# voutcn/megahit

Hardware: AMD Instinct MI355X
Metric: M (k+1)-mer edges sorted+counted/sec, sdbg_build k=21 (higher is better)
Workload: dtype u32; 1 GPU; read2sdbg (S1+S2) k=21 m=2 no mercy, 10000000 synthetic 150 bp PE reads per GPU (BASELINE configs[1]), inputs resident in HBM, outputs left in HBM; reads_per_gpu=10000000, edges_per_gpu=1290000000, k=21, min_count=2, parallelism=1 GPU, s1_items=1330000000, s2_items=117381042, sdbg_records=59857080

## Files before the change

megahit_amd/csrc/mhx_internal.h:

```cpp
#pragma once
#include <hip/hip_runtime.h>

#include <cstdint>
#include <cstdio>
#include <cstring>
#include <functional>
#include <map>
#include <stdexcept>
#include <string>
#include <vector>

#include "../../include/mhx.h"
#include "mhx_options.h"
#include "s1_handoff.h"

using mhx::Opt;

namespace mhx {

struct OnesweepLaunch;
void set_error(const char *fmt, ...);

struct Error : std::runtime_error {
  explicit Error(const std::string &s) : std::runtime_error(s) {}
// ... 56 lines not shown
  mhx::S1Handoff s1;
  uint64_t n_route = 0;
  uint32_t filter_kept = 0;
  double s1_density = 0;
  bool s1_agg_wide_agreed = false;
  std::string last_s1_plan;
  bool filter_on = false, accumulate = false;
  uint64_t filter_expected = 0, filter_batch_bytes = 0;
  bool global_marks_inverted = false;
  uint64_t s1_acc_bits = 0, mercy_acc_n = 0;
  uint32_t s1_acc_k = 0, s1_acc_m = 0;
  uint32_t count_acc_k = 0, count_acc_m = 0;
  uint64_t n_marks = 0;
  uint64_t dist_local_solid = 0;
  bool dist_s2_agg = false;
  bool ut_ready = false, ut_owner = false;
  uint64_t ut_edges = 0, ut_nv = 0;
  bool ut_text_fresh = false;
  uint64_t ub_stats[4] = {0, 0, 0, 0};
  bool lm_ready = false, lm_mapped = false;
  uint64_t lm_n_ctg = 0, lm_cap = 0, lm_n_reads = 0;
  uint32_t lm_seed = 0;
  std::map<std::string, long long> options;
  std::map<std::string, long long> tuned;
  template <mhx::Opt O>
  long long opt() const { return mhx::resolve_option<O>(options, tuned); }
  template <mhx::Opt O>
  long long opt(long long fallback) const { return mhx::resolve_option<O>(options, tuned, fallback); }
  long long opt(const char *name, long long dflt) const { return mhx::resolve_option(options, tuned, name, dflt); }
  void *pinned[2] = {nullptr, nullptr};
  hipEvent_t pinned_free[2] = {nullptr, nullptr};
  bool profiling = false;
  std::vector<mhx::PendingEvent> pending;
  std::vector<hipEvent_t> event_pool;
  std::vector<hipStream_t> side_streams;
  std::vector<hipEvent_t> side_events;
  std::map<std::string, mhx::KernelStat> stats;

  mhx::DevBuf &ws(const char *name, size_t bytes) {
    mhx::DevBuf &b = work[name];
    b.reserve(bytes);
    return b;
  }
  mhx::DevBuf &result(int which, size_t bytes) {
    mhx::DevBuf &b = results[which];
    b.reserve(bytes);
    b.used = bytes;
    return b;
  }
  void prof_begin(const char *name, double bytes);
  void prof_end();
  void prof_collect();
};

#define MHX_LAUNCH(ctx, name, bytes, ...) \
  do {                                    \
    (ctx)->prof_begin(name, bytes);       \
    __VA_ARGS__;                          \
    MHX_HIP(hipGetLastError());           \
    (ctx)->prof_end();                    \
  } while (0)

namespace mhx {

struct SortPass {
  int shift;
  int bits;
  int shift2 = 0;
  int bits2 = 0;
  int prev_lo = -1;
};
struct SortPrep {
  const void *buf = nullptr;
  uint64_t n = 0;
  int hist_passes = 0;
  uint64_t hist_sig = 0;
  const unsigned long long *hist = nullptr;
  std::function<void(const OnesweepLaunch &)> gen;
  uint64_t gen_slots = 0;
  bool gen_var = false;
  const unsigned long long *split_fill = nullptr, *split_ubase = nullptr;
  uint64_t split_range_cap = 0, split_units = 0;
  int hist_first = 0;
};
uint32_t *radix_sort(mhx_ctx *c, uint32_t *buf_a, uint32_t *buf_b, uint64_t n, int stride, int key_words,
                     const std::vector<SortPass> &passes, SortPrep *prep = nullptr);
uint32_t *sort_whole_key(mhx_ctx *c, uint32_t *buf_a, uint32_t *buf_b, uint64_t n, int stride, int key_words,
                         const std::vector<SortPass> &passes, SortPrep *prep = nullptr);
std::vector<SortPass> make_passes(int key_words, int lo_bit, int hi_bit);
bool sort_takes_generated_first_pass(const mhx_ctx *c, uint64_t n, int stride, const std::vector<SortPass> &passes);
bool sort_takes_split_first_pass(const mhx_ctx *c, const std::vector<SortPass> &passes);
constexpr uint64_t kSortSplitUnit = 4096;
uint64_t passes_signature(const std::vector<SortPass> &ps);
uint32_t *kmsort_exact(mhx_ctx *c, uint32_t *buf_a, uint32_t *buf_b, uint64_t n, int S, int key_words, SortPrep *prep = nullptr);

void exclusive_scan_u32_u64(mhx_ctx *c, const uint32_t *in, uint64_t *out, uint64_t n, uint64_t *d_total);
void exclusive_scan_u64(mhx_ctx *c, const uint64_t *in, uint64_t *out, uint64_t n, uint64_t *d_total);
void find_group_heads(mhx_ctx *c, const uint32_t *items, uint64_t n, int stride, int cmp_bits,
                      uint64_t *heads, uint64_t *d_count);
uint64_t count_group_heads(mhx_ctx *c, const uint32_t *items, uint64_t n, int stride, int cmp_bits);

struct DigitSpec;
DigitSpec spec_of_pass(const SortPass &ps, int key_words);
std::vector<SortPass> make_passes_ranges(int key_words, const std::vector<std::pair<int, int>> &ranges);
void emit_sdbg(mhx_ctx *c, const uint32_t *sorted, uint64_t n_items, int S, int kw, uint32_t k, int is_seq, mhx_sdbg_result *out, int compact_bits = 0);

void partition_by_owner(mhx_ctx *c, const uint32_t *a, uint32_t *b, uint64_t n, int stride, const uint8_t *lut, int n_parts,
                        uint64_t *counts);
uint64_t s1_extract(mhx_ctx *c, uint32_t k, bool compact, SortPrep *prep, bool defer_items = false, bool filter_in_gen = false);
bool s1_compact(const mhx_ctx *c, uint32_t k, int want_mercy);
bool s1_rank_tagged(const mhx_ctx *c, uint32_t k);
int s1_stride(uint32_t k, bool compact);
struct S1Sources {
  int n = 0;
  std::vector<const uint32_t *> ptr;
  std::vector<uint64_t> count;
  uint32_t *spare = nullptr;
  int pbits = 16;
};
constexpr int kSkmBatch = 8;
constexpr int kSkmSrcMax = 8;
struct SkmFront {
  int n_src;
  const uint4 *src[kSkmSrcMax];
  const uint64_t *src_bounds[kSkmSrcMax];
  uint32_t *spare;
  uint64_t spare_bytes;
  uint64_t n_records, n_windows;
  uint64_t n_items;
  uint32_t n_bins, max_bin;
  uint32_t bin_lo, bin_hi;
  int bin_bits;
  unsigned long long *hp;
  bool rep;
  const uint2 *giants;
  uint32_t n_giant_items, giant_limit;
  uint32_t giant_bins, giant_largest;
  const char *why;
};
bool s1_skm_applies(const mhx_ctx *c, uint32_t k, uint32_t m, int want_mercy);
bool s1_skm_dist_applies(const mhx_ctx *c, uint32_t k, uint32_t m);
int s1_skm_passes(const mhx_ctx *c, uint32_t k);
bool s1_skm_front(mhx_ctx *c, uint32_t k, SkmFront *f, int pass, int n_passes, int bin_bits_agreed = 0, bool for_count = false, bool bins_whole = false);
uint32_t s1_skm_max_m(const mhx_ctx *c);
uint64_t s1_skm_beside_below(mhx_ctx *c, const SkmFront &f, uint32_t k, uint32_t m);
void s1_skm_bounds_of(mhx_ctx *c, const uint4 *recs, uint64_t n, uint32_t n_bins, uint64_t *bounds);
void s1_skm_groups_launch(mhx_ctx *c, bool agg, unsigned grid, const SkmFront &f, uint32_t k, uint32_t m, uint8_t *solid_bytes, unsigned long long *hist,
                          uint2 *agg_raw, uint32_t agg_cap, uint32_t *agg_counts, uint32_t *err, unsigned long long *marks_raw, uint32_t marks_cap,
                          uint32_t *marks_counts);
struct DigitSpecs;
void s1_skm_hp_publish(mhx_ctx *c, const SkmFront &f, uint32_t k, uint32_t m, uint8_t *solid_bytes, unsigned long long *hist, uint2 *agg_items,
                       uint64_t *agg_cursor, bool agg, const DigitSpecs *agg_specs = nullptr, unsigned long long *agg_hist = nullptr);
uint64_t s1_skm_rep_publish(mhx_ctx *c, const SkmFront &f, uint32_t k, uint32_t m, uint8_t *solid_bytes, unsigned long long *hist, uint2 *agg_items,
                            uint64_t *agg_cursor, bool agg, const DigitSpecs *agg_specs = nullptr, unsigned long long *agg_hist = nullptr);
bool s1_skm_owner(mhx_ctx *c, uint32_t k, uint32_t m, const SkmFront &f, mhx_s1_result *out);

bool s1_presort_applies(const mhx_ctx *c, uint32_t k, uint64_t n_local_items);
uint32_t *s1_presort(mhx_ctx *c, uint32_t k, uint32_t *buf_a, uint32_t *buf_b, uint64_t n_items, int *pbits, SortPrep *prep);
bool s1_filter_in_gen_applies(const mhx_ctx *c, uint32_t k);
bool s1_bucket_histogram_fast(mhx_ctx *c, uint32_t k, unsigned long long *hist);
uint32_t s1_pos_bits(const mhx_ctx *c);
uint64_t s1_pos_stride(const mhx_ctx *c, uint32_t k);
std::string s1_plan_text(const mhx_ctx *c, uint32_t k, uint64_t n_items);
int s1_process(mhx_ctx *c, uint32_t k, uint32_t m, int want_mercy, uint32_t *buf_a, uint32_t *buf_b, uint64_t n_items, mhx_s1_result *out,
               const S1Sources *pre = nullptr, SortPrep *prep = nullptr, bool var_gen = false);
__global__ void k_add_u64(unsigned long long *__restrict__ a, const unsigned long long *__restrict__ b, int n);
void sdbg_accumulate(mhx_ctx *c, bool first);
void sdbg_publish_accumulated(mhx_ctx *c);
uint64_t s2_extract(mhx_ctx *c, uint32_t k, uint32_t m, bool filter_in_extract = false);
int s2_process(mhx_ctx *c, uint32_t k, uint32_t *buf_a, uint32_t *buf_b, uint64_t n_items, mhx_sdbg_result *out);
bool s2_use_aggregated(const mhx_ctx *c, uint32_t k, uint32_t m);
uint64_t s2_agg_extract(mhx_ctx *c, uint32_t k);
int s2_agg_process(mhx_ctx *c, uint32_t k, uint32_t *buf_a, uint32_t *buf_b, uint64_t n_items, mhx_sdbg_result *out, SortPrep *prep = nullptr);
std::vector<SortPass> s2_agg_sort_passes(uint32_t k, int count_bits);
struct StageItems {
  uint64_t n;
  int S;
  bool agg;
  bool batchable;
  SortPrep prep;
};
StageItems extract_stage(mhx_ctx *c, int stage, uint32_t k, uint32_t m, bool s1_defer_items = false);
void bucket_histogram(mhx_ctx *c, int stage, uint32_t k, uint32_t m, uint64_t *h_out);
int s2_stride(uint32_t k);
constexpr int MHX_BUF_IS_SOLID_LOCAL = 100;
constexpr int MHX_BUF_MERCY_CAND_LOCAL = 101;
uint64_t count_extract(mhx_ctx *c, uint32_t k, uint32_t m, SortPrep *prep);
int count_stride(uint32_t k);
int count_process(mhx_ctx *c, uint32_t k, uint32_t m, uint32_t *buf_a, uint32_t *buf_b, uint64_t n_items, mhx_count_result *out, SortPrep *prep = nullptr);
void count_apply_events(mhx_ctx *c, const unsigned long long *ev, uint64_t n);
uint64_t seq2sdbg_extract(mhx_ctx *c, uint32_t k);
int seq2sdbg_stride(uint32_t k);
int seq2sdbg_process(mhx_ctx *c, uint32_t k, uint32_t *buf_a, uint32_t *buf_b, uint64_t n_items, mhx_sdbg_result *out);
const uint64_t *sort_u64(mhx_ctx *c, const void *src, uint64_t n, int hi_bit);
void invert_local_marks(mhx_ctx *c, unsigned long long *words, uint64_t n_words);
DevBuf &grow_preserving(mhx_ctx *c, DevBuf &b, size_t bytes, size_t keep);
void stash_route_records(mhx_ctx *c, const void *src, uint64_t n, int hi_bit);
void mercy_adopt_routed(mhx_ctx *c, const long long *recv, uint64_t n);
void s1_apply_marks(mhx_ctx *c, const unsigned long long *recv, uint64_t n);
int sdbg_build_index(mhx_ctx *c, uint32_t k, mhx_sdbg_index_info *out);
int sdbg_remove_tips(mhx_ctx *c, const mhx_sdbg_index_info *info, int max_tip_len, uint64_t *n_removed);
int sdbg_mul_histogram(mhx_ctx *c, const mhx_sdbg_index_info *info, uint64_t *n_valid, std::vector<uint64_t> *host = nullptr);
int infer_min_depth(const uint64_t *hist, double *min_depth, int *converged);
int sdbg_unitigs(mhx_ctx *c, const mhx_sdbg_index_info *info, mhx_unitig_result *out);
int sdbg_unitig_text(mhx_ctx *c, const mhx_sdbg_index_info *info, uint64_t nv, uint64_t n_loop, mhx_unitig_result *out);
int unitig_disconnect_weak_links(mhx_ctx *c, const mhx_sdbg_index_info *info, double ratio, uint64_t *n_flagged);
int unitig_remove_tips(mhx_ctx *c, const mhx_sdbg_index_info *info, uint32_t max_tip_len, uint64_t *n_removed);
int unitig_remove_local_low_depth(mhx_ctx *c, const mhx_sdbg_index_info *info, double min_depth, uint32_t max_len, uint32_t local_width,
                                  double local_ratio, int mark_changed, uint64_t *n_removed, int *is_changed);
int unitig_iterate_local_low_depth(mhx_ctx *c, const mhx_sdbg_index_info *info, double min_depth, uint32_t max_len, uint32_t local_width,
                                   double local_ratio, int mark_changed, uint64_t *n_removed);
int unitig_finish(mhx_ctx *c, const mhx_sdbg_index_info *info, mhx_unitig_result *out);
int unitig_remove_low_depth(mhx_ctx *c, const mhx_sdbg_index_info *info, double min_depth, uint64_t *n_removed);
int unitig_pop_bubbles(mhx_ctx *c, const mhx_sdbg_index_info *info, uint32_t max_len, double similarity, double careful_threshold, int mark_changed,
                       uint64_t *n_removed, uint64_t *n_records);
int unitig_similarity(mhx_ctx *c, const char *a, uint32_t n, const char *b, uint32_t m, double sim, double *out);
int iterate_edges(mhx_ctx *c, uint32_t k, uint32_t step, const uint32_t *ctg_words, uint64_t ctg_n_words, uint64_t n_ctg, const uint64_t *ctg_start,
                  mhx_iterate_result *out);
int local_index(mhx_ctx *c, const uint32_t *ctg_words, uint64_t ctg_n_words, uint64_t n_ctg, const uint64_t *ctg_start, uint32_t seed,
                uint32_t sparsity, uint64_t *index_size);
int local_map(mhx_ctx *c, int32_t min_mapping_len, double similarity, uint64_t *n_valid);
int local_collect(mhx_ctx *c, uint32_t n_libs, const uint64_t *lib_begin, const uint64_t *lib_end, const int32_t *lib_paired,
// ... 85 lines not shown
```

megahit_amd/csrc/mhx_options.h:

```cpp
#pragma once
#include <cstddef>
#include <cstdlib>
#include <cstring>
#include <map>
#include <string>
#include <vector>

#define MHX_OPTIONS(X, D)          \
                     \
  X(edges_reserve_permille, 1000)  \
  X(fetch_pinned, 1)               \
  X(dist_marks_one_pass, 1)        \
                     \
  X(sort_unit_runs, 1)             \
  X(sort_xcd_units, 1)             \
  X(sort_loaded_ut2, 0)            \
  X(sort_rank_uniform, 1)          \
  X(sort_hybrid, 1)                \
  X(sort_hybrid_min, 1 << 16)      \
  X(sort_hybrid_margin_ps, 6)      \
  X(sort_hybrid_bits, 0)           \
                  \
  X(iterate_prefix_filter, 1)      \
                \
  X(tips_candidate_list, 1)        \
               \
  D(sdbg_hist_flush_tiles)         \
               \
  X(kmsort_emu_legacy, 0)          \
                   \
  X(s2_filter_in_extract, 1)       \
                     \
  X(dist_presort, 1)               \
  X(dist_max_items, 0)             \
  X(count_skm_dist, 0)             \
                    \
  X(count_seg, 1)                  \
  X(count_seg_bits, 0)             \
  X(count_extract_fixed, 1)        \
  X(count_seg_la, 3)               \
                       \
  X(s1_seg_bits, 0)                \
  X(s1_seg, 1)                     \
  X(s1_stream, 1)                  \
  X(s1_stream_wide, 1)             \
  X(s1_stream_max, 40000)          \
  X(s1_stream_sub_max, 1)          \
  D(s1_stream_max3)                \
  X(s1_stream_bits, 0)             \
  X(s1_stream_sub0, -1)            \
  X(s1_pos_bits, 0)                \
  X(dist_sparse_marks, 0)          \
  X(s1_seg_per, 8)                 \
  X(s1_seg_la, 3)                  \
  X(s1_stream_direct, 1)           \
  X(s1_stream_probes, 1024)        \
  D(s1_stream_fill)                \
  X(s1_giant, 1)                   \
  X(s1_giant_min, 262144)          \
  X(s1_pack_fixed, 1)              \
  X(s1_agg_wide, 0)                \
  X(count_stream, 1)               \
  X(count_event_share, 4)          \
  X(count_giant, 1)                \
                 \
  X(s1_bucket_hist_fast, 1)        \
  X(s1_digit_hist_roll, 1)         \
  X(count_stream_wide, 1)          \
  X(s1_var_fast, 1)                \
  X(s1_var_min_fill, 50)           \
  X(s1_extract_fast, 1)            \
  X(s1_filter_in_gen, 1)           \
  X(s1_fused_first_pass, 1)        \
  X(s1_digit_hist_blocked, 1)      \
  X(s1_digit_hist_plain, 1)        \
  X(s1_gen_any_order, 1)           \
  X(s1_gen_blocked, 0)             \
  X(s1_gen_roll, 1)                \
  X(s1_extract_items, 4)           \
  X(s1_digit_hist_preload, 0)      \
                  \
  X(s1_mercy_regions, 1)           \
                   \
  X(s1_skm, 1)                     \
  X(s1_skm_min_windows, 1 << 22)   \
  X(s1_skm_bin_bits, 0)            \
  X(count_skm, 1)                  \
  X(s1_skm_max_m, 2)               \
  X(dist_skm, 1)                   \
  X(s1_skm_passes, 0)              \
  X(s1_skm_cap_pct, 36)            \
  X(s1_skm_pass_gb, 48)            \
  X(s1_skm_split, 1)               \
  D(s1_skm_split_stage)            \
  X(s1_skm_make_grid, 0)           \
  X(s1_skm_hp, 1)                  \
  X(s1_skm_rep, 0)                 \
  X(s1_skm_rep_slots, 64)          \
  X(s1_skm_giant, 0)               \
  X(s1_skm_giant_max, 1 << 21)     \
  X(s1_skm_giant_keys, 4096)       \
  X(s1_skm_giant_work_pct, 25)     \
  X(s1_skm_giant_slices, 0)        \
  X(s1_skm_max_bin, 1 << 16)       \
  X(s1_skm_tags, 0)                \
  X(s1_skm_deal, 2)                \
  X(count_skm_group, 2)            \
  X(count_skm_ev_cap, 0)           \
                       \
  X(sdbg_fast, 1)                  \
  D(sdbg_fast_halo)                \
  X(sdbg_fast_tile, 2048)          \
  X(sdbg_fast_keep, 1)             \
  X(sdbg_fast_keep_max_mb, 4096)   \
  X(s2_bound_from_s1, 1)           \
  X(s2_dummy_list, 1)              \
  X(s2_dummy_list_cap, 0)          \
  X(s2_agg_from_count, 1)          \
  X(s2_count_budget_mb, 0)         \
  X(s2_count_pass_items, 0)        \
  X(s2_pre_hist, 1)                \
  X(s2_agg_in_place, 1)

namespace mhx {

#define MHX_OPT_PLAIN(name, dflt) name,
#define MHX_OPT_DERIVED(name) name,
enum class Opt : int { MHX_OPTIONS(MHX_OPT_PLAIN, MHX_OPT_DERIVED) };
#undef MHX_OPT_PLAIN
#undef MHX_OPT_DERIVED

struct OptInfo {
  const char *name;
  char env_name[48];
  long long dflt;
  bool derived;
};

constexpr void opt_env_name(const char *name, char *out, size_t cap) {
  const char pre[] = "MHX_";
  size_t n = 0;
  for (const char *p = pre; *p && n + 1 < cap; ++p) out[n++] = *p;
  for (const char *p = name; *p && n + 1 < cap; ++p) out[n++] = *p >= 'a' && *p <= 'z' ? (char)(*p - 'a' + 'A') : *p;
  out[n] = 0;
}
constexpr OptInfo make_opt_info(const char *name, long long dflt, bool derived) {
  OptInfo o{name, {}, dflt, derived};
  opt_env_name(name, o.env_name, sizeof o.env_name);
  return o;
}

#define MHX_OPT_PLAIN(name, dflt) make_opt_info(#name, dflt, false),
#define MHX_OPT_DERIVED(name) make_opt_info(#name, 0, true),
inline constexpr OptInfo kOptions[] = {MHX_OPTIONS(MHX_OPT_PLAIN, MHX_OPT_DERIVED)};
#undef MHX_OPT_PLAIN
#undef MHX_OPT_DERIVED
inline constexpr size_t kNumOptions = sizeof kOptions / sizeof kOptions[0];
constexpr const OptInfo &opt_info(Opt o) { return kOptions[(size_t)o]; }

using OptMap = std::map<std::string, long long>;

inline long long resolve_option(const OptMap &options, const OptMap &tuned, const char *name, const char *env_name, long long dflt) {
  auto it = options.find(name);
  if (it != options.end()) return it->second;
  const char *e = getenv(env_name);
  if (e && *e) return atoll(e);
  auto tu = tuned.find(name);
  return tu != tuned.end() ? tu->second : dflt;
}
inline long long resolve_option(const OptMap &options, const OptMap &tuned, const char *name, long long dflt) {
  std::string env(strlen(name) + 5, '\0');
  opt_env_name(name, &env[0], env.size());
  return resolve_option(options, tuned, name, env.c_str(), dflt);
}
template <Opt O>
long long resolve_option(const OptMap &options, const OptMap &tuned) {
  static_assert(!opt_info(O).derived, "a derived knob has no default of its own: read it as opt<Opt::name>(fallback)");
  return resolve_option(options, tuned, opt_info(O).name, opt_info(O).env_name, opt_info(O).dflt);
}
template <Opt O>
long long resolve_option(const OptMap &options, const OptMap &tuned, long long fallback) {
  static_assert(opt_info(O).derived, "this knob has its default in the table: read it as opt<Opt::name>()");
  return resolve_option(options, tuned, opt_info(O).name, opt_info(O).env_name, fallback);
}

inline void set_option(OptMap &options, Opt o, long long v) { options[opt_info(o).name] = v; }

class OptScope {
 public:
// ... 19 lines not shown
```

megahit_amd/csrc/s1.hip:

```cpp
#include "s1_shared.h"

namespace mhx {

template <bool HIST>
__global__ __launch_bounds__(256) void k_agg_compact(const uint2 *__restrict__ raw, uint32_t cap, const uint32_t *__restrict__ counts,
                                                    uint2 *__restrict__ dense, int from_back, DigitSpecs specs, unsigned long long *__restrict__ hist) {
  __shared__ uint64_t sm[256 / kWave + 1];
  __shared__ uint32_t s_hist[HIST ? kItemHistRows : 1][256];
  if (HIST)
    for (int i = threadIdx.x; i < kItemHistRows * 256; i += 256) (&s_hist[0][0])[i] = 0;
  const ItemDigits digits(specs);
  const uint32_t r = blockIdx.x;
  uint64_t part = 0;
  for (uint32_t i = threadIdx.x; i < r; i += 256) part += counts[i];
  uint64_t off;
  block_exclusive_sum<uint64_t, 256>(part, sm, &off);
  const uint32_t n = counts[r];
  const uint2 *src = raw + (size_t)r * cap;
  for (uint32_t i = blockIdx.y * 256 + threadIdx.x; i < n; i += gridDim.y * 256) {
    const uint2 v = from_back ? src[cap - 1 - i] : src[i];
    dense[off + i] = v;
    if (HIST) item_hist_add(s_hist, digits, ((uint64_t)v.x << 32) | v.y);
  }
  if (HIST) {
// ... 306 lines not shown
  const double n_eff = per_bucket * (double)MHX_NUM_BUCKETS;
  int bits = 8;
  while (bits < 32 && n_eff / 96.0 > (double)(1ull << bits)) bits += 8;
  if (force_bits) bits = force_bits;
  bits = std::max(1, std::min(bits, std::min(32, kmer_bits)));
  p.seg_bits = bits;
  p.passes = make_passes(2, 64 - bits, 64);
  return p;
}
std::string s1_plan_text(const mhx_ctx *c, uint32_t k, uint64_t n_items) {
  const S1Plan p = s1_plan(c, k, n_items, s1_compact(c, k, 0), 0);
  char buf[128];
  if (p.stream) snprintf(buf, sizeof buf, "stream p%d sub%d %zu passes (%.0f records per lv1 bucket)", p.seg_bits, p.sub0, p.passes.size(), p.per_bucket);
  else if (p.seg_bits) snprintf(buf, sizeof buf, "seg p%d %zu passes", p.seg_bits, p.passes.size());
  else snprintf(buf, sizeof buf, "full sort %zu passes", p.passes.size());
  return buf;
}
uint32_t s1_pos_bits(const mhx_ctx *c) {
  const bool force = getenv("MHX_S1_FORCE_TAGGED") != nullptr;
  const long long f = c->opt<Opt::s1_pos_bits>();
  if (f > 0) return (uint32_t)std::min<long long>(std::max<long long>(f, 4), 32);
  if (force) {
    const uint64_t n_bits = c->global_bases ? c->global_bases : c->seqs.n_bases;
    uint32_t b = 4;
    while (b < 32 && (n_bits >> b) >= 128) ++b;
    return b;
  }
  return 32;
}
bool s1_rank_tagged(const mhx_ctx *c, uint32_t k) {
  const uint64_t n_bits = c->global_bases ? c->global_bases : c->seqs.n_bases;
  const uint32_t pb = s1_pos_bits(c);
  if ((n_bits >> pb) == 0) return false;
  const int spare = 32 * s1_kw(k) - (int)(k - 1) * 2 - 6;
  return spare >= 8 && (n_bits >> pb) < 256;
}
uint64_t s1_pos_stride(const mhx_ctx *c, uint32_t k) { return s1_rank_tagged(c, k) ? 1ull << s1_pos_bits(c) : 0ull; }
bool s1_compact(const mhx_ctx *c, uint32_t k, int want_mercy) {
  if (want_mercy) return false;
  if (s1_kw(k) < 2) return false;
  const uint64_t n_bits = c->global_bases ? c->global_bases : c->seqs.n_bases;
  return (n_bits >> s1_pos_bits(c)) == 0 || s1_rank_tagged(c, k);
}
int s1_stride(uint32_t k, bool compact) {
  const int kw = s1_kw(k);
  if (!compact) return round_up2(kw + 2);
  return kw + 1 == 3 ? 3 : round_up2(kw + 1);
}


bool s1_presort_applies(const mhx_ctx *c, uint32_t k, uint64_t n_local_items) {
  return c->n_parts <= kStreamSrcMax && s1_plan(c, k, n_local_items, s1_compact(c, k, 0), 0).stream;
}
uint32_t *s1_presort(mhx_ctx *c, uint32_t k, uint32_t *buf_a, uint32_t *buf_b, uint64_t n_items, int *pbits, SortPrep *prep) {
  const S1Plan plan = s1_plan(c, k, std::max<uint64_t>(n_items, 1), true, 0);
  if (!plan.stream) throw Error("s1_presort: the bucket-streaming plan does not apply");
  *pbits = plan.seg_bits;
  return n_items ? radix_sort(c, buf_a, buf_b, n_items, 3, s1_kw(k), plan.passes, prep) : buf_a;
}

namespace {
struct S1Stage {
  mhx_ctx *c;
  uint32_t k, m;
  int want_mercy;
  uint32_t *buf_a, *buf_b;
  uint64_t n_items;
  const S1Sources *pre;
  SeqSet &s;
  hipStream_t st;
  bool compact, global, tagged_keys;
  int KWv, S, kmer_bits;
  size_t item_bytes;
  uint64_t pos_stride;
  S1Plan plan;
  uint32_t *sorted = nullptr, *spare = nullptr;
  uint64_t n_bits = 0, n_words64 = 0;
  int mark_atomic = 0;
  const char *mark_env = nullptr;
  bool sparse = false, acc = false;
  bool list_local = false;
  unsigned long long *is_solid = nullptr, *hist = nullptr, *ctr = nullptr;
  uint8_t *solid_bytes = nullptr;
  uint64_t marks_prev = 0, seg_marks = 0;
  const uint32_t *giant_ctr = nullptr;
  bool classic_ran = false;
  long long *mercy = nullptr;
  bool agg = false;
  bool agg_wide = false;
  uint2 *agg_items = nullptr;
  uint64_t *agg_cursor = nullptr;
  uint64_t agg_prev = 0, agg_bound = 0;
  unsigned long long *agg_hist = nullptr;
  DigitSpecs agg_specs = no_digits();
  uint64_t agg_sig = 0;
  uint32_t seg_grid = 0, seg_cap = 0, seg_mcap = 0;
  uint32_t *seg_err = nullptr;
  uint64_t skm_rounds = 0, skm_looks = 0;
  int mark_mode = 0, mark_mode_used = 0;

  S1Stage(mhx_ctx *c_, uint32_t k_, uint32_t m_, int wm, uint32_t *a, uint32_t *b, uint64_t n, const S1Sources *pre_)
      : c(c_), k(k_), m(m_), want_mercy(wm), buf_a(a), buf_b(b), n_items(n), pre(pre_), s(c_->seqs), st(c_->stream) {
    compact = s1_compact(c, k, want_mercy);
    KWv = s1_kw(k);
    S = s1_stride(k, compact);
    item_bytes = (size_t)S * 4;
    global = c->global_bases != 0;
    kmer_bits = (int)(k - 1) * 2;
    tagged_keys = compact && s1_rank_tagged(c, k);
    pos_stride = compact ? s1_pos_stride(c, k) : 0;
    plan = s1_plan(c, k, pre ? std::max<uint64_t>(n_items, 1) : n_items, compact, want_mercy);
    if (pre && (!plan.stream || want_mercy || !compact)) throw Error("s1_process: pre-sorted sources need the bucket-streaming plan");
    if (pre && pre->pbits != plan.seg_bits) throw Error("s1_process: the sources were sorted for another plan than the one this rank makes");
  }

  void sort_records(SortPrep *prep) {
    sorted = pre ? nullptr
             : want_mercy == 2
                 ? kmsort_exact(c, buf_a, buf_b, n_items, S, KWv, prep)
                 : (plan.seg_bits || tagged_keys ? radix_sort(c, buf_a, buf_b, n_items, S, KWv, plan.passes, prep)
                                                 : sort_whole_key(c, buf_a, buf_b, n_items, S, KWv, plan.passes, prep));
    set_spare(pre ? pre->spare : (sorted == buf_a ? buf_b : buf_a));
  }
  void set_spare(uint32_t *sp) {
    spare = sp;
    mercy = reinterpret_cast<long long *>(spare);
  }
  void ensure_byte_map() {
    if (solid_bytes) return;
    const uint64_t nw = div_ceil(n_bits, 64);
    solid_bytes = c->ws("solid_bytes", (nw + 1) * 64).as<uint8_t>();
    if (!acc || sparse) MHX_HIP(hipMemsetAsync(solid_bytes, 0, (nw + 1) * 64, st));
  }
  void open_outputs() {
    n_bits = global ? c->global_bases : s.n_bases;
    mark_env = getenv("MHX_S1_MARK");
    mark_atomic = mark_env && !strcmp(mark_env, "atomic") ? 1 : 0;
    sparse = global && !mark_atomic && c->opt<Opt::dist_sparse_marks>() != 0;
    n_words64 = sparse ? 0 : div_ceil(n_bits, 64);
    is_solid = c->result(MHX_BUF_IS_SOLID, (n_words64 + 1) * 8).as<unsigned long long>();
    c->results[MHX_BUF_IS_SOLID].used = n_words64 * 8;
    hist = c->result(MHX_BUF_MUL_HIST, (MHX_MAX_MUL + 1) * 8).as<unsigned long long>();
    acc = c->accumulate && c->s1_acc_bits == n_bits && c->s1_acc_k == k && c->s1_acc_m == m;
    marks_prev = sparse && acc ? c->n_marks : 0;
    if (!sparse || !acc) c->n_marks = 0;
    if (mark_atomic) {
      if (!acc) MHX_HIP(hipMemsetAsync(is_solid, 0, (n_words64 + 1) * 8, st));
    } else {
      if (!sparse) ensure_byte_map();
      MHX_HIP(hipMemsetAsync(is_solid + n_words64, 0, 8, st));
    }
    if (!acc) MHX_HIP(hipMemsetAsync(hist, 0, (MHX_MAX_MUL + 1) * 8, st));
    c->s1_acc_bits = n_bits;
    c->s1_acc_k = k;
    c->s1_acc_m = m;
    ctr = c->ws("s1_counters", 64).as<unsigned long long>();
    MHX_HIP(hipMemsetAsync(ctr, 0, 64, st));
    const bool agg_off = getenv("MHX_S2_PER_OCCURRENCE") != nullptr;
    agg = !agg_off && k <= 22 && m >= 2 && KWv == 2;
    agg_wide = !agg_off && k >= 23 && k <= 27 && m >= 2 && KWv == 2 && !want_mercy && plan.stream && c->opt<Opt::s1_agg_wide>() != 0;
    if (global && !c->s1_agg_wide_agreed) agg_wide = false;
    const S1Handoff::Opened opened = c->s1.open_items(k, m, acc);
    if (agg_wide && acc && !opened.continues) agg_wide = false;
    agg = agg || agg_wide;
    agg_cursor = c->ws("s2_agg_cursor", 64).as<uint64_t>();
    if (!opened.in_flight.empty()) MHX_HIP(hipStreamSynchronize(st));
    agg_prev = opened.continues ? c->s1.agg_n : 0;
    agg_bound = (n_items / m + 16) * 2;
    if (agg_wide) agg_bound += n_items / ((1ull << s2_agg_compact_bits(k)) - 1) * 2;
    agg_hist = nullptr;
    if (agg && !global && !c->filter_on && !c->accumulate && agg_prev == 0 && c->opt<Opt::s2_pre_hist>() != 0) {
      const std::vector<SortPass> ps = s2_agg_sort_passes(k, s2_agg_count_bits(k));
      if (!ps.empty() && ps.size() <= (size_t)kItemHistRows) {
        agg_specs.n = (int)ps.size();
        for (size_t p = 0; p < ps.size(); ++p) agg_specs.d[p] = spec_of_pass(ps[p], 2);
        agg_sig = passes_signature(ps);
        agg_hist = c->ws("s2_pre_hist", (size_t)kItemHistRows * 256 * 8).as<unsigned long long>();
        MHX_HIP(hipMemsetAsync(agg_hist, 0, (size_t)kItemHistRows * 256 * 8, st));
      }
    }
    seg_err = c->ws("s1_seg_err", 64).as<uint32_t>();
  }
  void agg_wide_off() {
    if (!agg_wide) return;
    agg = agg_wide = false;
    agg_hist = nullptr;
  }
  void agg_prepare_classic() {
    agg_wide_off();
    agg_hist = nullptr;
    if (!agg) return;
    agg_items = grow_preserving(c, c->work["s2_agg_items"], (agg_prev + agg_bound) * 8, agg_prev * 8).as<uint2>();
    MHX_HIP(hipMemsetAsync(agg_cursor, 0, 24, st));
    if (agg_prev) MHX_HIP(hipMemcpyAsync(agg_cursor, &agg_prev, 8, hipMemcpyHostToDevice, st));
  }

  void launch_partial(int mode) {
    const int per = (int)c->opt<Opt::s1_seg_per>();
    const int la = (int)std::min<long long>(std::max<long long>(c->opt<Opt::s1_seg_la>(), 0), 200);
    const int T = 256 * (per == 4 ? 4 : 8);
    const uint64_t n_tiles = div_ceil(n_items, (uint64_t)T);
    const uint32_t stride = mode == 2 ? 64u : 1u;
    const uint64_t n_buckets = plan.stream ? 1ull << plan.seg_bits : 0;
    const uint64_t n_work = plan.stream ? div_ceil(n_buckets, stride) : div_ceil(n_tiles, stride);
    const uint32_t pfx_mask = plan.seg_bits >= 32 ? 0xFFFFFFFFu : ~(0xFFFFFFFFu >> plan.seg_bits);
    const uint32_t eq_mask1 = (kmer_bits > 32 ? ~(0xFFFFFFFFu >> (kmer_bits - 32)) : 0u) | 63u;
    const bool agg_on = agg && mode != 2;
    const bool half = false;
    const uint64_t cus = c->n_cus > 0 ? (uint64_t)c->n_cus : 256;
    unsigned grid = (unsigned)std::min<uint64_t>(n_work, plan.stream ? (half ? 2 * cus : cus) : (per == 4 ? 256 * 6 : 256 * 3));
    if (agg_on && agg_wide) {
      const uint64_t min_region = 16 * ((uint64_t)MHX_MAX_MUL / ((1ull << s2_agg_compact_bits(k)) - 1) + 1);
      grid = (unsigned)std::min<uint64_t>(grid, std::max<uint64_t>(1, n_items * (uint64_t)S * 4 / 8 / min_region));
    }
    const uint32_t region = (uint32_t)std::min<uint64_t>(n_items * (uint64_t)S * 4 / 8 / grid, 0xFFFFFFF0u);
// ... 538 lines not shown
    g.fl_cap = kGiantFlagged;
    g.fl_cnt = c->ws("cs_giant_fl_cnt", (size_t)g.gcap * 4 + 64).as<uint32_t>();
    g.fl_key = c->ws("cs_giant_fl_key", (size_t)g.gcap * g.fl_cap * 8 + 64).as<unsigned long long>();
    MHX_HIP(hipMemsetAsync(g.fl_cnt, 0, (size_t)g.gcap * 4 + 64, st));
    if (global) {
      g.ev_cap = (uint32_t)std::min<uint64_t>(std::max<uint64_t>(n_items / 8, 1u << 20), 0xFFFFFFF0u);
      g.ev = c->ws("cs_giant_events", (size_t)g.ev_cap * 8 + 64).as<unsigned long long>();
      g.ev_cur = g.fl_cnt + g.gcap;
    }
    MHX_HIP(hipMemsetAsync(g.flag, 0, n_buckets, st));
    MHX_HIP(hipMemsetAsync(lists, 0, 64, st));
    s1_giant_launch(c, items0, srcs, bounds, n_src, n_buckets, plan.seg_bits, (int)k, g, key64, true);
  }
  S1StreamLaunch sl{true, false, pos_stride != 0, false, true, grid, items0, bounds, a, geo, 1u, ticket, srcs, n_src};
  sl.key64 = key64;
  s1_stream_launch(c, "count_groups", bytes, sl);
  if (giant_on) {
    S1StreamLaunch gl{true, false, pos_stride != 0, true, true, grid, items0, bounds, a, geo, 1u, ticket2, srcs, n_src};
    gl.key64 = key64;
    s1_stream_launch(c, "count_giant_groups", 0.0, gl);
    count_giant_look_launch(c, items0, srcs, bounds, n_src, n_buckets, plan.seg_bits, a);
  }
  uint32_t e = 0;
  unsigned long long h_ctr[8] = {0};
  std::vector<uint32_t> h_ec(global ? grid : 0);
  MHX_HIP(hipMemcpyAsync(&e, seg_err, 4, hipMemcpyDeviceToHost, st));
  MHX_HIP(hipMemcpyAsync(h_ctr, ctr, 64, hipMemcpyDeviceToHost, st));
  if (global) MHX_HIP(hipMemcpyAsync(h_ec.data(), ecounts, (size_t)grid * 4, hipMemcpyDeviceToHost, st));
  MHX_HIP(hipStreamSynchronize(st));
  o->grid = grid;
  o->cap = region;
  o->counts = counts;
  o->spare = spare;
  o->sorted = sorted;
  o->n_items = n_items;
  o->n_distinct = h_ctr[4];
  o->plan = s1_plan_text(c, k, std::max<uint64_t>(count_plan_items(c, k), 1));
  if (giant_ctr) {
    uint32_t h_giant[4] = {0, 0, 0, 0};
    MHX_HIP(hipMemcpy(h_giant, giant_ctr, 16, hipMemcpyDeviceToHost));
    if (h_giant[0]) o->plan += " [" + std::to_string(h_giant[0]) + " giant buckets in slices]";
  }
  o->events = nullptr;
  o->n_events = 0;
  if (e == 0 && global) {
    for (uint32_t v : h_ec) o->n_events += v;
    uint32_t n_look = 0;
    if (giant_on) {
      MHX_HIP(hipMemcpy(&n_look, a.giant.ev_cur, 4, hipMemcpyDeviceToHost));
      n_look = std::min(n_look, a.giant.ev_cap);
    }
    unsigned long long *dense = c->ws("cs_events_dense", (o->n_events + n_look) * 8 + 64).as<unsigned long long>();
    if (o->n_events)
      MHX_LAUNCH(c, "events_compact", (double)o->n_events * 16,
                 agg_compact_launch(st, dim3(grid, 8), reinterpret_cast<const uint2 *>(a.marks_raw), ecap, ecounts,
                                    reinterpret_cast<uint2 *>(dense), 0, no_digits(), nullptr));
    if (n_look) MHX_HIP(hipMemcpyAsync(dense + o->n_events, a.giant.ev, (size_t)n_look * 8, hipMemcpyDeviceToDevice, st));
    o->n_events += n_look;
    o->events = dense;
  }
  return e == 0;
}

static bool s1_skm_try(mhx_ctx *c, uint32_t k, uint32_t m, mhx_s1_result *out, std::string *why) {
  const int n_passes = s1_skm_passes(c, k);
  SkmFront f{};
  S1Stage stage(c, k, m, 0, nullptr, nullptr, 0, nullptr);
  stage.sorted = nullptr;
  uint64_t n_records = 0;
  uint32_t max_bin = 0, giant_bins = 0, giant_slices = 0, giant_largest = 0;
  for (int p = 0; p < n_passes; ++p) {
    if (!s1_skm_front(c, k, &f, p, n_passes, 0, false, m >= 3)) {
      *why = f.n_records ? "a bin of " + std::to_string(f.max_bin) + " records" : "more records than the array holds";
      if (f.why) *why += std::string(", ") + f.why;
      return false;
    }
    if (p == 0 && m >= 3) {
      if (const uint64_t n_below = s1_skm_beside_below(c, f, k, m)) {
        *why = "a key beside the records has " + std::to_string(n_below) + " windows, below the min count";
        return false;
      }
    }
    stage.set_spare(f.spare);
    if (p == 0) stage.open_outputs();
    if (!stage.run_skm(f)) {
      *why = "an output region overflowed";
      return false;
    }
    n_records += f.n_records;
    max_bin = std::max(max_bin, f.max_bin);
    giant_bins += f.giant_bins;
    giant_slices += f.n_giant_items;
    giant_largest = std::max(giant_largest, f.giant_largest);
  }
  stage.publish_skm_hp(f);
  const uint64_t n_rep = stage.publish_skm_rep(f);
  stage.n_items = f.n_items;
  stage.mark_mode_used = 1;
  char txt[320];
  snprintf(txt, sizeof txt, "super-k-mers m%u, 2^%d bins (%llu records for %llu windows: %.2f per record; largest bin %u)%s", k + 1 - 9, f.bin_bits,
           (unsigned long long)n_records, (unsigned long long)f.n_windows, n_records ? (double)f.n_windows / (double)n_records : 0.0, max_bin,
           c->seqs.fixed_len ? "" : " [reads of several lengths]");
  c->last_s1_plan = txt;
  if (n_passes > 1) c->last_s1_plan += " [" + std::to_string(n_passes) + " passes over ranges of bins]";
  if (f.rep) c->last_s1_plan += " [" + std::to_string(n_rep) + " windows of period <= 4 beside the records]";
  if (giant_bins)
    c->last_s1_plan += " [" + std::to_string(giant_bins) + " giant bins in " + std::to_string(giant_slices) + " slices, largest " + std::to_string(giant_largest) + " records]";
  if (m >= 3) c->last_s1_plan += " [a second look in " + std::to_string(stage.skm_looks) + " of " + std::to_string(stage.skm_rounds) + " rounds]";
  stage.publish(out);
  return true;
}

bool s1_skm_owner(mhx_ctx *c, uint32_t k, uint32_t m, const SkmFront &f, mhx_s1_result *out) {
  S1Stage stage(c, k, m, 0, nullptr, nullptr, f.n_items, nullptr);
  stage.sorted = nullptr;
  stage.set_spare(f.spare);
  stage.open_outputs();
  if (!stage.sparse) throw Error("s1_skm_owner: the marks of a global layout leave as a list (dist_sparse_marks)");
  if (!stage.run_skm(f)) return false;
  stage.mark_mode_used = 1;
  char txt[320];
  snprintf(txt, sizeof txt, "super-k-mers m%u, 2^%d bins (%llu records at this owner, bins %u..%u) [records exchanged by bin]", k + 1 - 9, f.bin_bits,
           (unsigned long long)f.n_records, f.bin_lo, f.bin_hi);
  c->last_s1_plan = txt;
  stage.publish(out);
  return true;
}

int run_s1(mhx_ctx *c, uint32_t k, uint32_t m, int want_mercy, mhx_s1_result *out) {
  if (c->global_bases) throw Error("read2sdbg_s1: a global layout is set; use the mhx_dist_* entry points");
  std::string skm_why;
  if (s1_skm_applies(c, k, m, want_mercy)) {
    if (s1_skm_try(c, k, m, out, &skm_why)) return 0;
    if (c->opt<Opt::s1_skm>() == 3) throw Error("read2sdbg_s1: super-k-mer records given up (" + skm_why + ")");
  }
  StageItems it = extract_stage(c, want_mercy ? MHX_STAGE_S1_MERCY : MHX_STAGE_S1, k, m, !want_mercy);
  uint32_t *buf_a = c->work["items_a"].as<uint32_t>();
  uint32_t *buf_b = c->ws("items_b", it.n * (size_t)it.S * 4 + 64).as<uint32_t>();
  const int rc = s1_process(c, k, m, want_mercy, buf_a, buf_b, it.n, out, nullptr, &it.prep, it.prep.gen_var);
  if (!skm_why.empty()) c->last_s1_plan += " [super-k-mer records given up: " + skm_why + "]";
  return rc;
}

}
```

megahit_amd/csrc/s1_skm.hip:

```cpp
#include <cstring>

#include "s1_shared.h"
#include "skm_deal.h"
#include "skm_giant.h"

namespace mhx {

constexpr int kSkmC = 8;
constexpr int kSkmW = 10;
constexpr int kSkmNM = kSkmC + kSkmW - 1;
constexpr int kSkmMinBinBits = 16, kSkmMaxBinBits = 20;

__device__ __forceinline__ uint32_t skm_mix(uint32_t c) {
  uint32_t h = c * 0x9E3779B1u;
  return h ^ (h >> 15);
}
__device__ __forceinline__ uint32_t skm_mix2(uint32_t c) {
  uint32_t h = c * 0x9E3779B1u;
  h ^= h >> 15;
  return h * 0x85EBCA6Bu;
}
__device__ __forceinline__ uint32_t skm_bin_of(uint32_t minh) {
  return (minh ^ (minh >> 16)) * 0x7FEB352Du;
}

constexpr int kSkmStage = 2560;
constexpr int kSkmRepN = 320, kSkmRepAt = 64;
constexpr int kSkmRepSlotsS1 = 48, kSkmRepSlotsCount = 16, kSkmRepProbes = 8;
template <int NT, int J, bool VAR, bool COUNT = false, bool SPLIT = false, bool REP = false>
__global__ __launch_bounds__(NT) void k_skm_make(const uint32_t *__restrict__ seq, const uint64_t *__restrict__ start, uint32_t L, uint32_t bpr, uint64_t n_blocks,
                                                 int k, int bin_bits, uint32_t bin_lo, uint32_t bin_hi, int count_items, uint64_t pos_base,
                                                 unsigned long long *__restrict__ hp, uint4 *__restrict__ out, unsigned long long cap,
                                                 unsigned long long *__restrict__ cursor, uint32_t *__restrict__ err, unsigned long long *__restrict__ digit_hist,
                                                 unsigned long long range_cap, unsigned long long *__restrict__ split_cur, uint32_t stage_n) {
  constexpr long long kNoRoom = -0x7FFFFFFFFFFFFFFFll - 1;
  __shared__ uint32_t sm_scan[NT / kWave + 1];
  __shared__ uint4 stage[SPLIT ? kSkmStage : 1];
  __shared__ uint32_t dcnt[SPLIT ? 256 : 1], dpos[SPLIT ? 256 : 1];
  __shared__ long long goff[SPLIT ? 256 : 1];
  __shared__ unsigned long long s_base;
  __shared__ uint32_t dh[3][256];
  __shared__ uint32_t lbin[J * kSkmC][NT];
  __shared__ uint32_t hpl[2][12];
  constexpr int kSkmRepSlots = COUNT ? kSkmRepSlotsCount : kSkmRepSlotsS1;
  __shared__ uint32_t rid[REP ? kSkmRepSlots : 1];
  __shared__ uint32_t rtl[REP ? kSkmRepSlots : 1][COUNT ? 9 : 1];
  __shared__ unsigned long long rps[REP && !COUNT ? kSkmRepSlots : 1];
  const int tid = threadIdx.x;
  if constexpr (REP) {
    if (tid < kSkmRepSlots) {
      rid[tid] = (uint32_t)kSkmRepN;
      if constexpr (!COUNT) rps[tid] = ~0ull;
    }
    if (tid < kSkmRepSlots * (COUNT ? 9 : 1)) rtl[tid / (COUNT ? 9 : 1)][tid % (COUNT ? 9 : 1)] = 0;
  }
  if (tid < 24) hpl[tid / 12][tid % 12] = 0;
  for (int i = tid; i < 768; i += NT) dh[i >> 8][i & 255] = 0;
  if (SPLIT && tid < 256) dcnt[tid] = 0;
  __syncthreads();
  const bool third_digit = bin_bits > 16;
  const int M = k + 1 - (kSkmW - 1);
  const uint32_t mmask = (1u << (2 * M)) - 1u;
  const int K1 = k + 1;
  const unsigned bin_sh = 32u - (unsigned)bin_bits;
  unsigned long long items = 0;
  uint32_t hp_n[2] = {0, 0};
  unsigned long long hp_p[2] = {~0ull, ~0ull};
  const uint64_t step_trip = (uint64_t)gridDim.x * (uint64_t)(NT * J);
  const uint64_t trip_r = step_trip / bpr;
  const uint32_t trip_q = (uint32_t)(step_trip - trip_r * bpr), next_r = (uint32_t)NT / bpr, next_q = (uint32_t)NT % bpr;
  uint64_t blk_r = ((uint64_t)blockIdx.x * (uint64_t)(NT * J) + tid) / bpr;
  uint32_t blk_q = (uint32_t)((uint64_t)blockIdx.x * (uint64_t)(NT * J) + tid - blk_r * bpr);
  uint64_t fa[J];
  uint32_t fq0[J], fnwin[J], fc[J][COUNT ? 4 : 3];
  [[maybe_unused]] auto rep_tally = [&](uint32_t e, unsigned pv, unsigned nx, uint64_t p) {
    if constexpr (REP) {
      unsigned long long *const tab = hp + kSkmRepAt;
      const uint32_t n_slots = min((uint32_t)hp[kSkmRepAt - 1], (uint32_t)kSkmRepSlots);
      uint32_t h = n_slots ? (e ^ (e >> 4) ^ (e >> 6)) % n_slots : 0u;
      int slot = -1;
      for (int n = 0; n < kSkmRepProbes && n_slots; ++n) {
        const uint32_t old = atomicCAS(&rid[h], (uint32_t)kSkmRepN, e);
        if (old == (uint32_t)kSkmRepN || old == e) {
          slot = (int)h;
          break;
        }
        h = h + 1 == n_slots ? 0u : h + 1;
      }
      if (slot >= 0) {
        atomicAdd(&rtl[slot][0], 1u);
        if constexpr (COUNT) {
          if (pv < 4) atomicAdd(&rtl[slot][1 + pv], 1u);
          if (nx < 4) atomicAdd(&rtl[slot][5 + nx], 1u);
        } else {
          atomicMin(&rps[slot], (unsigned long long)p);
        }
      } else {
        const uint32_t sig = COUNT ? e | ((uint32_t)pv << 9) | ((uint32_t)nx << 12) : e;
        for (;;) {
          const uint32_t s0 = (uint32_t)__builtin_amdgcn_readfirstlane((int)sig);
          const unsigned long long together = __ballot(sig == s0);
          if (sig == s0) {
            if ((tid & (kWave - 1)) == __builtin_ctzll(together)) {
              const unsigned long long n = (unsigned long long)__builtin_popcountll(together);
              if constexpr (COUNT) {
                atomicAdd(tab + 9 * e, n);
                if (pv < 4) atomicAdd(tab + 9 * e + 1 + pv, n);
                if (nx < 4) atomicAdd(tab + 9 * e + 5 + nx, n);
              } else {
                atomicAdd(tab + e, n);
              }
            }
            break;
          }
        }
        if constexpr (!COUNT) {
          unsigned long long *const at = tab + kSkmRepN + e;
          if ((unsigned long long)p < __hip_atomic_load(at, __ATOMIC_RELAXED, __HIP_MEMORY_SCOPE_AGENT)) atomicMin(at, (unsigned long long)p);
        }
      }
    }
  };
  auto fetch = [&](uint64_t it2) {
    uint64_t r = blk_r;
    uint32_t q = blk_q;
#pragma unroll
    for (int j = 0; j < J; ++j) {
      const uint64_t b = it2 * (uint64_t)(NT * J) + (uint64_t)j * NT + tid;
      fa[j] = 0;
      fq0[j] = 0;
      fnwin[j] = 0;
      if (j > 0) {
        r += next_r;
        q += next_q;
        if (q >= bpr) {
          q -= bpr;
          ++r;
        }
      }
      if (b < n_blocks) {
        const uint32_t q0 = q * kSkmC;
        uint64_t base;
        uint32_t nwin;
        if constexpr (VAR) {
          base = start[r];
          const uint64_t len_r = start[r + 1] - base;
          nwin = len_r >= (uint64_t)K1 ? (uint32_t)(len_r - k) : 0u;
          if (q0 == 0 && nwin && count_items) items += nwin + (COUNT ? 0 : 4);
        } else {
          base = r * L;
          nwin = L - k;
        }
        if (q0 < nwin) {
          fa[j] = base + q0;
          fq0[j] = q0;
          fnwin[j] = nwin;
        }
      }
      const uint64_t wi = fa[j] >> 4;
      fc[j][0] = seq[wi];
      fc[j][1] = seq[wi + 1];
      fc[j][2] = seq[wi + 2];
      if constexpr (COUNT) fc[j][3] = seq[(fa[j] > 0 ? fa[j] - 1 : 0) >> 4];
    }
    blk_r += trip_r;
    blk_q += trip_q;
    if (blk_q >= bpr) {
      blk_q -= bpr;
      ++blk_r;
    }
  };
  for (uint64_t it = blockIdx.x; it * (uint64_t)(NT * J) < n_blocks; it += gridDim.x) {
    uint64_t Wv[J], pos0[J];
    uint32_t smask[J], emask[J];
    uint32_t bflag[J];
    fetch(it);
#pragma unroll
    for (int j = 0; j < J; ++j) {
      smask[j] = 0;
      emask[j] = 0;
      bflag[j] = 0;
      Wv[j] = 0;
      pos0[j] = 0;
      {
        const uint32_t q0 = fq0[j], nwin = fnwin[j];
        if (q0 < nwin) {
          const uint64_t a = fa[j];
          const unsigned sh = (unsigned)(a & 15) * 2;
          const uint32_t c0 = fc[j][0], c1 = fc[j][1], c2 = fc[j][2];
          const uint64_t W = ((uint64_t)funnel_l(c0, c1, sh) << 32) | funnel_l(c1, c2, sh);
          const uint64_t R = rc64(W, 32);
          uint32_t h[kSkmNM];
#pragma unroll
          for (int i = 0; i < kSkmNM; ++i) {
            const uint32_t f = (uint32_t)(W >> (64 - 2 * (i + M))) & mmask;
            const uint32_t rv = (uint32_t)(R >> (2 * i)) & mmask;
            h[i] = skm_mix(min(f, rv));
          }
          uint32_t sfx[kSkmW];
          sfx[kSkmW - 1] = h[kSkmW - 1];
#pragma unroll
          for (int i = kSkmW - 2; i >= 0; --i) sfx[i] = min(h[i], sfx[i + 1]);
          uint32_t pfx = 0xFFFFFFFFu;
          uint32_t bins[kSkmC];
          bins[0] = skm_bin_of(sfx[0]) >> bin_sh;
#pragma unroll
          for (int w = 1; w < kSkmC; ++w) {
            pfx = min(pfx, h[kSkmW - 1 + w]);
            bins[w] = skm_bin_of(min(sfx[w], pfx)) >> bin_sh;
          }
#pragma unroll
          for (int w = 0; w < kSkmC; ++w) lbin[j * kSkmC + w][tid] = bins[w];
          const uint32_t n_here = min((uint32_t)kSkmC, nwin - q0);
          uint32_t km = 0, sm = 0, hm = 0;
          if constexpr (REP) {
            const uint64_t d4 = W ^ (W << 8), d3 = W ^ (W << 6);
            uint32_t m4 = 0, m3 = 0;
            if ((d4 & ((~0ull >> (2 * (kSkmC - 1))) & (~0ull << (64 - 2 * (K1 - 4))))) == 0) {
#pragma unroll
              for (int w = 0; w < kSkmC; ++w)
                if ((uint32_t)w < n_here && ((d4 << (2 * w)) >> (64 - 2 * (K1 - 4))) == 0) m4 |= 1u << w;
            }
            if ((d3 & ((~0ull >> (2 * (kSkmC - 1))) & (~0ull << (64 - 2 * (K1 - 3))))) == 0) {
#pragma unroll
              for (int w = 0; w < kSkmC; ++w)
                if ((uint32_t)w < n_here && ((d3 << (2 * w)) >> (64 - 2 * (K1 - 3))) == 0) m3 |= 1u << w;
            }
            hm = m4 | m3;
            if (hm && count_items) {
#pragma unroll
              for (int w = 0; w < kSkmC; ++w)
                if ((hm >> w) & 1u) {
                  const uint32_t e = (m4 >> w) & 1u ? (uint32_t)(W >> (56 - 2 * w)) & 255u : 256u + ((uint32_t)(W >> (58 - 2 * w)) & 63u);
                  unsigned prev_raw = 4, next_raw = 4;
                  if constexpr (COUNT) {
                    prev_raw = q0 + w == 0 ? kSentinel
                                           : (w == 0 ? (unsigned)((fc[j][COUNT ? 3 : 0] >> (30 - 2 * (unsigned)((a - 1) & 15))) & 3u) : (unsigned)(W >> (64 - 2 * w)) & 3u);
                    next_raw = q0 + w + 1 == nwin ? kSentinel : (unsigned)(W >> (62 - 2 * (w + K1))) & 3u;
                  }
                  rep_tally(e, prev_raw, next_raw, pos_base + a + (uint64_t)w);
                }
            }
          } else if (hp) {
            const uint64_t dx = W ^ (W << 2);
            if ((dx & ((~0ull >> (2 * (kSkmC - 1))) & (~0ull << (64 - 2 * (K1 - 1))))) == 0) {
#pragma unroll
              for (int w = 0; w < kSkmC; ++w)
                if ((uint32_t)w < n_here && ((dx << (2 * w)) >> (64 - 2 * (K1 - 1))) == 0) hm |= 1u << w;
            }
            if (hm && count_items) {
#pragma unroll
              for (int w = 0; w < kSkmC; ++w)
                if ((hm >> w) & 1u) {
                  const unsigned b = (unsigned)(W >> (62 - 2 * w)) & 3u;
                  const unsigned cls = b == 0 || b == 3 ? 0u : 1u;
                  if constexpr (COUNT) {
                    const bool strand = b >= 2;
                    const unsigned prev_raw = q0 + w == 0 ? kSentinel
                                              : (w == 0 ? (unsigned)((fc[j][COUNT ? 3 : 0] >> (30 - 2 * (unsigned)((a - 1) & 15))) & 3u) : (unsigned)(W >> (64 - 2 * w)) & 3u);
                    const unsigned next_raw = q0 + w + 1 == nwin ? kSentinel : (unsigned)(W >> (62 - 2 * (w + K1))) & 3u;
                    const unsigned pv = strand ? comp_or_sentinel(next_raw) : prev_raw, nx = strand ? comp_or_sentinel(prev_raw) : next_raw;
                    atomicAdd(&hpl[cls][0], 1u);
                    if (pv < 4) atomicAdd(&hpl[cls][1 + pv], 1u);
                    if (nx < 4) atomicAdd(&hpl[cls][5 + nx], 1u);
                  } else {
                    ++hp_n[cls];
                    hp_p[cls] = min(hp_p[cls], pos_base + a + (uint64_t)w);
                  }
                }
            }
          }
#pragma unroll
          for (int w = 0; w < kSkmC; ++w)
            if ((uint32_t)w < n_here && !((hm >> w) & 1u) && bins[w] >= bin_lo && bins[w] < bin_hi) km |= 1u << w;
#pragma unroll
          for (int w = 0; w < kSkmC; ++w)
            if (((km >> w) & 1u) && (w == 0 || !((km >> (w - 1)) & 1u) || bins[w] != bins[w > 0 ? w - 1 : 0])) sm |= 1u << w;
          smask[j] = sm;
          emask[j] = km & ((sm >> 1) | ~(km >> 1));
          if constexpr (COUNT) {
            const uint64_t pb = a > 0 ? (uint64_t)((fc[j][COUNT ? 3 : 0] >> (30 - 2 * (unsigned)((a - 1) & 15))) & 3u) : 0ull;
            Wv[j] = (W >> 2) | (pb << 62);
            bflag[j] = (q0 == 0 ? 1u : 0u) | (q0 + n_here == nwin ? 2u : 0u) | (n_here << 2);
          } else {
            Wv[j] = W;
          }
          pos0[j] = pos_base + a;
        }
      }
    }
    auto rec_of = [&](int j, int rs, int re, uint32_t run_bin) -> uint4 {
      const int len = re - rs + 1;
      const uint64_t p = pos0[j] + (uint64_t)rs;
// ... 228 lines not shown
  for (int o = 0; o < kSkmRepN; ++o)
    if (s_t[o][0] && s_key[o] == s_key[e]) {
      if (o < e) lead = false;
      for (int c = 0; c < 9; ++c) t[c] += s_t[o][c];
    }
  if (lead && t[0]) {
    atomicAdd(&s_res[1], 1ull);
    atomicAdd(&s_res[3], t[0]);
    const unsigned long long hb = t[0] > MHX_MAX_MUL ? (unsigned long long)MHX_MAX_MUL : t[0];
    atomicAdd(&hist[hb], 1ull);
    if (t[0] >= m) {
      bool has_in = false, has_out = false;
      for (int c = 0; c < 4; ++c) {
        has_in = has_in || t[1 + c] >= m;
        has_out = has_out || t[5 + c] >= m;
      }
      if (!has_in || !has_out) s_res[2] = 1;
      edges_at[atomicAdd(&s_res[0], 1ull)] = s_key[e] | hb;
    }
  }
  __syncthreads();
  if (e < 4) res[e] = s_res[e];
}

__global__ void k_skm_hp_publish(const unsigned long long *__restrict__ hp, int k, uint32_t m, uint8_t *__restrict__ solid_bytes,
                                 unsigned long long *__restrict__ hist, uint2 *__restrict__ agg_items, uint64_t *__restrict__ agg_cursor, int agg,
                                 DigitSpecs agg_specs, unsigned long long *__restrict__ agg_hist) {
  if (threadIdx.x || blockIdx.x) return;
  for (int x = 0; x < 2; ++x) {
    const unsigned long long cnt = hp[x];
    if (!cnt) continue;
    const unsigned long long hb = cnt > MHX_MAX_MUL ? (unsigned long long)MHX_MAX_MUL : cnt;
    hist[hb] += 1;
    if (cnt < m) {
      solid_bytes[hp[2 + x]] = 1;
    } else if (agg) {
      const uint64_t e0 = x == 0 ? 0ull : 0x5555555555555555ull;
      const uint64_t keep = ~0ull << (64 - 2 * (k + 1));
      const uint64_t xs[2] = {e0 & keep, ~e0 & keep};
      const uint64_t mask_k = ~0ull << (64 - 2 * k);
      uint64_t at = *agg_cursor;
      for (int y = 0; y < 2; ++y) {
        const uint64_t v = xs[y];
        const uint64_t f = ((v << 2) & mask_k) | (1ull << 19) | ((v >> 62) << 16) | hb;
        agg_items[at++] = make_uint2((uint32_t)(f >> 32), (uint32_t)f);
        if (agg_hist) {
          const uint32_t w[2] = {(uint32_t)(f >> 32), (uint32_t)f};
          for (int p = 0; p < agg_specs.n; ++p) atomicAdd(&agg_hist[p * 256 + words_digit2<2>(w, agg_specs.d[p])], 1ull);
        }
      }
      *agg_cursor = at;
    }
  }
}

__global__ __launch_bounds__(kSkmRepN) void k_skm_beside_check(const unsigned long long *__restrict__ hp, int rep, int k, uint32_t m, unsigned long long *__restrict__ res) {
  __shared__ unsigned long long s_key[kSkmRepN], s_cnt[kSkmRepN];
  __shared__ unsigned long long s_worst;
  const int e = threadIdx.x, K1 = k + 1;
  const uint64_t kmask = ~0ull << (64 - 2 * (k - 1));
  if (e == 0) s_worst = 0;
  {
    const uint64_t win = skm_rep_window((uint32_t)e, K1);
    const uint64_t f = (win << 2) & kmask, rc = (rc64(win, 32) << (2 * (32 - k))) & kmask;
    const unsigned head = (unsigned)(win >> 62), tail = (unsigned)(win >> (62 - 2 * k)) & 3u;
    s_key[e] = skm_s1_key(f, rc, head, tail);
    s_cnt[e] = rep ? hp[kSkmRepAt + e] : 0ull;
  }
  __syncthreads();
  unsigned long long cnt = 0;
  bool lead = s_cnt[e] != 0;
  for (int o = 0; o < kSkmRepN; ++o)
    if (s_cnt[o] && s_key[o] == s_key[e]) {
      if (o < e) lead = false;
      cnt += s_cnt[o];
    }
  if (!lead) cnt = 0;
  if (e < 2 && !rep) cnt = hp[e];
  if (cnt > 1 && cnt < m) atomicMax(&s_worst, cnt);
  __syncthreads();
  if (e == 0) *res = s_worst;
}

__global__ __launch_bounds__(256) void k_skm_bounds(const uint4 *__restrict__ recs, uint64_t n, uint32_t n_bins, uint64_t *__restrict__ bounds,
                                                    uint32_t *__restrict__ max_bin) {
  const uint32_t b = blockIdx.x * 256 + threadIdx.x;
  if (b > n_bins) return;
  auto lower = [&](uint32_t v) -> uint64_t {
    uint64_t lo = 0, hi = n;
    while (lo < hi) {
      const uint64_t mid = (lo + hi) >> 1;
      const uint32_t bin = (reinterpret_cast<const uint32_t *>(recs + mid)[0] >> 8) & 0xFFFFFu;
      if (bin < v) lo = mid + 1;
      else hi = mid;
    }
    return lo;
  };
  const uint64_t at = b == n_bins ? n : lower(b);
  bounds[b] = at;
  if (b < n_bins) {
    const uint64_t nx = b + 1 == n_bins ? n : lower(b + 1);
    const uint64_t d = nx - at;
    atomicMax(max_bin, d > 0xFFFFFFFFull ? 0xFFFFFFFFu : (uint32_t)d);
  }
}

__global__ __launch_bounds__(256) void k_skm_giants(const uint64_t *__restrict__ bounds, uint32_t bin_lo, uint32_t bin_hi, uint64_t limit, uint2 *__restrict__ out,
                                                    uint32_t list_cap) {
  const uint64_t b = (uint64_t)bin_lo + (uint64_t)blockIdx.x * 256 + threadIdx.x;
  if (b >= bin_hi) return;
  const uint64_t d = bounds[b + 1] - bounds[b];
  if (d > limit) {
    const uint32_t at = atomicAdd(reinterpret_cast<uint32_t *>(out), 1u);
    if (at < list_cap) out[1 + at] = make_uint2((uint32_t)b, d > 0xFFFFFFFFull ? 0xFFFFFFFFu : (uint32_t)d);
  }
}

struct SkmArgs {
  int k;
  uint32_t m;
  uint8_t *solid_bytes;
  unsigned long long *hist;
  uint2 *agg_raw;
  uint32_t agg_cap;
  uint32_t *agg_counts;
  uint32_t *err;
  uint32_t max_fill;
  int probe_limit;
  uint32_t bin_lo, bin_hi;
  unsigned long long *marks_raw;
  uint32_t marks_cap;
  uint32_t *marks_counts;
  const uint2 *giants;
  uint32_t n_giant, giant_limit;
};
struct SkmSrcs {
  const uint4 *ptr[kSkmSrcMax];
  const uint64_t *bounds[kSkmSrcMax];
  int n;
};

constexpr int kSkmThreads = 1024, kSkmLogSlots = 13;

__device__ __forceinline__ uint32_t wave_exclusive_sum_4bit(uint32_t v, uint32_t *total) {
  uint32_t ex = 0, tot = 0;
#pragma unroll
  for (int b = 0; b < 4; ++b) {
    const unsigned long long has = __ballot((v >> b) & 1u);
    ex += __builtin_amdgcn_mbcnt_hi((uint32_t)(has >> 32), __builtin_amdgcn_mbcnt_lo((uint32_t)has, 0u)) << b;
    tot += (uint32_t)__builtin_popcountll(has) << b;
  }
  *total = tot;
  return ex;
}

template <bool AGG, bool TAGS, int DEAL, bool GIANT = false, bool LOOK = false>
__global__ __launch_bounds__(kSkmThreads) void k_s1_skm(SkmSrcs srcs, SkmArgs a, uint32_t *__restrict__ ticket) {
  static_assert(!LOOK || (DEAL == 2 && !GIANT), "the second look is built on the three-shuffle deal, bins whole");
  constexpr int NT = kSkmThreads, NSLOT = 1 << kSkmLogSlots, W = NSLOT / NT;
  constexpr unsigned long long kEmpty = ~0ull;
  constexpr int NLIST = 1024;
  __shared__ unsigned long long keys[NSLOT];
  __shared__ uint32_t cnts[NSLOT];
  __shared__ uint32_t fpos[NSLOT];
  __shared__ uint8_t ftag[TAGS ? NSLOT : 4];
  __shared__ uint32_t lhist[kSegHist];
  __shared__ unsigned long long slist_k[AGG ? NLIST : 1];
  __shared__ uint32_t slist_c[AGG ? NLIST : 1];
  __shared__ unsigned long long heads[DEAL ? kSkmThreads / kWave : 1][8];
  __shared__ uint32_t s_bad2[2], s_nclaimed2[2], s_list_n2[2];
  __shared__ uint32_t s_agg_cur, s_mark_cur, s_tk;
  __shared__ uint32_t s_look;
  __shared__ uint64_t s_lo[kSkmSrcMax][kSkmBatch + 1];
  const int tid = threadIdx.x, lane = tid & (kWave - 1), wv = DEAL ? tid / kWave : 0;
  const uint32_t le_lo = lane >= 31 ? 0xFFFFFFFFu : (2u << lane) - 1u, le_hi = lane < 32 ? 0u : (lane == 63 ? 0xFFFFFFFFu : (2u << (lane - 32)) - 1u);
  const int k = a.k, K1 = k + 1;
  const uint32_t m = a.m;
  const uint64_t kmask = ~0ull << (64 - 2 * (k - 1));
  uint2 *const agg_end = AGG ? a.agg_raw + (size_t)(blockIdx.x + 1) * a.agg_cap : nullptr;
  for (int i = tid; i < NSLOT; i += NT) {
    keys[i] = kEmpty;
    cnts[i] = 0;
  }
  for (int i = tid; i < kSegHist; i += NT) lhist[i] = 0;
  if (tid == 0) {
    s_bad2[0] = s_bad2[1] = 0;
    s_nclaimed2[0] = s_nclaimed2[1] = 0;
    s_list_n2[0] = s_list_n2[1] = 0;
    s_agg_cur = 0;
    s_mark_cur = 0;
    if constexpr (LOOK) s_look = 0;
  }
  const int n_src = srcs.n;
  unsigned long long *const marks_out = a.marks_raw ? a.marks_raw + (size_t)blockIdx.x * a.marks_cap : nullptr;
  int rp = 0;
  __syncthreads();

  auto emit_items = [&](unsigned long long key, uint32_t cnt, bool dense, bool valid) {
    uint64_t x = 0, xr = 0;
    uint32_t n_out = 0;
    if (valid) {
      x = skm_s1_key_kmer(key, k, kmask);
      xr = rc64(x, K1);
      n_out = x == xr ? 1u : 2u;
    }
    uint32_t at;
    bool ok;
    if (dense) {
      const uint32_t incl = wave_inclusive_sum(n_out);
      const uint32_t tot = __shfl(incl, kWave - 1, kWave);
      if (!tot) return;
      uint32_t wbase = 0;
      if (lane == 0) wbase = atomicAdd(&s_agg_cur, tot);
      wbase = __shfl(wbase, 0, kWave);
      ok = wbase + tot <= a.agg_cap;
      at = wbase + incl - n_out;
    } else {
      at = atomicAdd(&s_agg_cur, n_out);
      ok = at + n_out <= a.agg_cap;
    }
    if (!ok) {
      atomicOr(a.err, 1u);
      return;
    }
    if (n_out) {
      const uint64_t mul = cnt > MHX_MAX_MUL ? (uint64_t)MHX_MAX_MUL : cnt;
      const uint64_t f = skm_s2_item(x, k, mul);
      agg_end[-1 - (long)at] = make_uint2((uint32_t)(f >> 32), (uint32_t)f);
      if (n_out == 2) {
        const uint64_t b = skm_s2_item(xr, k, mul);
        agg_end[-2 - (long)at] = make_uint2((uint32_t)(b >> 32), (uint32_t)b);
      }
    }
  };

  uint4 pre = make_uint4(0u, 0u, 0u, 0u);
  uint64_t pre_at = 0;
  bool pre_ok = false;
  for (;;) {
    if (tid == 0) s_tk = atomicAdd(ticket, 1u);
    __syncthreads();
    uint32_t sub0 = 0, rj0 = 0;
    bool slice = false;
    if constexpr (GIANT) slice = s_tk < a.n_giant;
    if (slice) {
      const uint2 item = a.giants[(uint32_t)__builtin_amdgcn_readfirstlane((int)s_tk)];
      const uint32_t depth_at = (uint32_t)__builtin_amdgcn_readfirstlane((int)item.y);
      sub0 = depth_at >> 16;
      rj0 = depth_at & 0xFFFFu;
      if (tid <= kSkmBatch) s_lo[0][tid] = srcs.bounds[0][item.x + (tid ? 1u : 0u)];
    } else {
      const uint64_t bin0 = (uint64_t)a.bin_lo + (uint64_t)(s_tk - (GIANT ? a.n_giant : 0u)) * kSkmBatch;
      if (bin0 >= a.bin_hi) break;
      if (tid < n_src * (kSkmBatch + 1)) {
        const int q = tid / (kSkmBatch + 1), x = tid - q * (kSkmBatch + 1);
        s_lo[q][x] = srcs.bounds[q][min(bin0 + x, (uint64_t)a.bin_hi)];
      }
    }
    __syncthreads();
    for (int bb = 0; bb < kSkmBatch; ++bb) {
      bool any = false;
      for (int q = 0; q < n_src; ++q) any = any || s_lo[q][bb] != s_lo[q][bb + 1];
      if (!any) continue;
      const uint64_t lo0 = s_lo[0][bb], hi0 = s_lo[0][bb + 1];
      if constexpr (GIANT)
        if (!slice && hi0 - lo0 > (uint64_t)a.giant_limit) continue;
      uint32_t sub = sub0, rj = rj0;
      for (;;) {
        uint32_t seen = 0;
        for (int q = 0; q < n_src; ++q) {
        const uint64_t lo = s_lo[q][bb], hi = s_lo[q][bb + 1];
        if (lo == hi) continue;
        const uint4 *__restrict__ recs = srcs.ptr[q];
        uint4 nxt = q == 0 && pre_ok && pre_at == lo ? pre : (lo + tid < hi ? recs[lo + tid] : make_uint4(0u, 0u, 0u, 0u));
        if (q == 0) pre_ok = false;
        for (uint64_t base = lo; base < hi; base += NT) {
          const uint4 r = nxt;
          const bool in = base + tid < hi;
          if (base + NT + tid < hi) nxt = recs[base + NT + tid];
          if (seen > a.max_fill) continue;
          const uint32_t len = in ? (r.z & 7u) + 1u : 0u;
          const uint8_t tag = TAGS ? (uint8_t)(r.x >> 28) : (uint8_t)0;
          uint32_t claims = 0;
          auto settle = [&](unsigned long long old, unsigned long long key, uint32_t hh, uint32_t pos, uint8_t tg) -> bool {
            if (old != kEmpty && old != key) return false;
            atomicAdd(&cnts[hh], 1u);
            if (old == kEmpty) {
              fpos[hh] = pos;
              if constexpr (TAGS) ftag[hh] = tg;
              ++claims;
            }
            return true;
          };
          const uint64_t rec_b = ((uint64_t)r.y << 32) | r.z;
          if constexpr (DEAL != 0) {
            uint32_t start, T;
            if constexpr (DEAL == 2) {
              start = wave_exclusive_sum_4bit(len, &T);
            } else {
              const uint32_t incl = wave_inclusive_sum(len);
              T = (uint32_t)__builtin_amdgcn_readlane((int)incl, kWave - 1);
              start = incl - len;
            }
            if (lane < 8) heads[wv][lane] = 0ull;
            __builtin_amdgcn_fence(__ATOMIC_RELEASE, "wavefront");
            __builtin_amdgcn_wave_barrier();
            if (len) atomicOr(&heads[wv][start >> 6], 1ull << (start & 63u));
            __builtin_amdgcn_fence(__ATOMIC_ACQ_REL, "wavefront");
            __builtin_amdgcn_wave_barrier();
            const unsigned long long hv = __hip_atomic_load(&heads[wv][lane & 7], __ATOMIC_RELAXED, __HIP_MEMORY_SCOPE_WORKGROUP);
            const uint32_t hv_lo = (uint32_t)hv, hv_hi = (uint32_t)(hv >> 32);
            const uint32_t bh = r.y, bl = r.z;
            [[maybe_unused]] uint32_t qh = 0, ql = 0, pd = 0, cbase_m1 = 0xFFFFFFFFu;
            [[maybe_unused]] SkmDealCarry dc;
            if constexpr (DEAL == 1) {
              const uint64_t rec_r = rc64(rec_b, 32);
              qh = (uint32_t)(rec_r >> 32), ql = (uint32_t)rec_r;
              pd = r.w - start;
            }
#pragma unroll
            for (int grp = 0; grp < 2; ++grp) {
              if ((uint32_t)(grp * 4 * kWave) >= T) break;
              unsigned long long key[4], old1[4];
              uint32_t h1[4], pos[4], mine = 0;
              uint8_t tg[4];
#pragma unroll
              for (int u = 0; u < 4; ++u) {
                const int c = grp * 4 + u;
                const uint32_t w_lo = (uint32_t)__builtin_amdgcn_readlane((int)hv_lo, c), w_hi = (uint32_t)__builtin_amdgcn_readlane((int)hv_hi, c);
                uint32_t o, j, xbh, xbl, p0;
                uint64_t win, rc;
                bool mn;
                if constexpr (DEAL == 2) {
                  const SkmDealAt d = skm_deal_at(((uint64_t)w_hi << 32) | w_lo, (uint32_t)lane, dc);
                  o = d.o;
                  j = d.j & 7u;
                  xbh = __shfl(bh, (int)o, kWave), xbl = __shfl(bl, (int)o, kWave);
                  p0 = __shfl(r.w, (int)o, kWave);
                  win = (((uint64_t)xbh << 32) | xbl) << (2 * j);
                  rc = skm_win_rc(win, k, kmask);
                  pos[u] = p0 + j;
                  mn = lane < (int)T - c * kWave;
                } else {
                  const uint32_t g = (uint32_t)(c * kWave) + (uint32_t)lane;
                  o = cbase_m1 + (uint32_t)__builtin_popcount(w_lo & le_lo) + (uint32_t)__builtin_popcount(w_hi & le_hi);
                  cbase_m1 += (uint32_t)__builtin_popcount(w_lo) + (uint32_t)__builtin_popcount(w_hi);
                  xbh = __shfl(bh, (int)o, kWave), xbl = __shfl(bl, (int)o, kWave);
                  const uint32_t xqh = __shfl(qh, (int)o, kWave), xql = __shfl(ql, (int)o, kWave);
                  const uint32_t so = __shfl(start, (int)o, kWave), pdo = __shfl(pd, (int)o, kWave);
                  j = g - so;
                  win = (((uint64_t)xbh << 32) | xbl) << (2 * j);
                  rc = ((((uint64_t)xqh << 32) | xql) << (2 * (32 - k - j))) & kmask;
                  pos[u] = pdo + g;
                  p0 = pdo + so;
                  mn = g < T;
                }
                const uint64_t f = (win << 2) & kmask;
                const unsigned head = (unsigned)(win >> 62), tail = ((uint32_t)win >> (62 - 2 * k)) & 3u;
                key[u] = skm_s1_key(f, rc, head, tail);
                const uint32_t klo = (uint32_t)key[u], khi = (uint32_t)(key[u] >> 32);
                if (sub) mn = mn && skm_in_round(skm_mix2((klo * 0xC2B2AE35u) ^ (khi * 0x27D4EB2Fu)), sub, rj);
                mine |= mn ? 1u << u : 0u;
// ... 73 lines not shown
              }
              if (a.probe_limit <= 0) {
                if (mine) s_bad2[rp] = 1;
                mine = 0;
              }
  #pragma unroll
              for (int u = 0; u < 4; ++u) {
                old1[u] = kEmpty;
                if ((mine >> u) & 1u) old1[u] = atomicCAS(&keys[h1[u]], kEmpty, key[u]);
              }
              bool has = false;
              unsigned long long pk = 0;
              uint32_t ph = 0, pp = 0;
              uint8_t pt = 0;
  #pragma unroll
              for (int u = 0; u < 4; ++u) {
                if ((mine >> u) & 1u) {
                  const uint32_t pos = r.w + (uint32_t)(half * 4 + u);
                  const uint8_t ptag = TAGS ? (uint8_t)(tag + (pos < r.w ? 1 : 0)) : (uint8_t)0;
                  if (!settle(old1[u], key[u], h1[u], pos, ptag)) {
                    uint32_t hh = (h1[u] + 1) & (NSLOT - 1);
                    if (!has) {
                      has = true;
                      pk = key[u], ph = hh, pp = pos, pt = ptag;
                    } else {
                      int n = 0;
                      while (!settle(atomicCAS(&keys[hh], kEmpty, key[u]), key[u], hh, pos, ptag)) {
                        hh = (hh + 1) & (NSLOT - 1);
                        if (++n >= a.probe_limit) {
                          s_bad2[rp] = 1;
                          break;
                        }
                      }
                    }
                  }
                }
              }
              int turns = 0;
              while (__ballot(has)) {
                if (has) {
                  if (settle(atomicCAS(&keys[ph], kEmpty, pk), pk, ph, pp, pt)) has = false;
                  else ph = (ph + 1) & (NSLOT - 1);
                }
                if (++turns > a.probe_limit) {
                  if (has) s_bad2[rp] = 1;
                  break;
                }
              }
            }
          }
          {
            uint32_t c;
            if constexpr (DEAL == 2) wave_exclusive_sum_4bit(claims, &c);
            else c = wave_sum(claims);
            if (lane == 0 && c) atomicAdd(&s_nclaimed2[rp], c);
            seen = __hip_atomic_load(&s_nclaimed2[rp], __ATOMIC_RELAXED, __HIP_MEMORY_SCOPE_WORKGROUP);
            seen = (uint32_t)__builtin_amdgcn_readfirstlane((int)seen);
          }
        }
        }
        __syncthreads();
        const bool bad = s_bad2[rp] != 0 || s_nclaimed2[rp] > a.max_fill;
        if (tid == 0) {
          s_bad2[rp ^ 1] = 0;
          s_nclaimed2[rp ^ 1] = 0;
          s_list_n2[rp ^ 1] = 0;
        }
        uint32_t nsub, nrj;
        bool done, give_up;
        skm_next_round(sub, rj, bad, sub0, rj0, &nsub, &nrj, &done, &give_up);
        if (give_up && tid == 0) atomicOr(a.err, 1u);
        {
          uint64_t nlo = lo0, nhi = hi0;
          if (done) {
            nlo = nhi = 0;
            for (int nb = bb + 1; nb < kSkmBatch; ++nb)
              if (s_lo[0][nb] != s_lo[0][nb + 1] && !(GIANT && !slice && s_lo[0][nb + 1] - s_lo[0][nb] > (uint64_t)a.giant_limit)) {
                nlo = s_lo[0][nb];
                nhi = s_lo[0][nb + 1];
                break;
              }
          }
          if (nlo != nhi) {
            pre = nlo + tid < nhi ? srcs.ptr[0][nlo + tid] : make_uint4(0u, 0u, 0u, 0u);
            pre_at = nlo;
            pre_ok = true;
          }
        }
        unsigned long long wk[W];
        uint32_t wc[W], wp[W];
        uint8_t wt[W];
#pragma unroll
        for (int it = 0; it < W; ++it) {
          const int sl = it * NT + tid;
          wk[it] = keys[sl];
          wc[it] = cnts[sl];
          wp[it] = fpos[sl];
          wt[it] = TAGS ? ftag[sl] : (uint8_t)0;
        }
        if constexpr (!LOOK) {
#pragma unroll
        for (int it = 0; it < W; ++it) {
          const int sl = it * NT + tid;
          keys[sl] = kEmpty;
          cnts[sl] = 0;
        }
        }
        uint32_t want_bits = 0, mark_bits = 0;
        [[maybe_unused]] bool look_mine = false;
#pragma unroll
        for (int it = 0; it < W; ++it) {
          if (wk[it] != kEmpty && !bad) {
            const uint32_t cnt = wc[it];
            const uint32_t hb = cnt > MHX_MAX_MUL ? (uint32_t)MHX_MAX_MUL : cnt;
            if (hb < kSegHist) atomicAdd(&lhist[hb], 1u);
            else atomicAdd(&a.hist[hb], 1ull);
            if (cnt < m) mark_bits |= 1u << it;
            else if (AGG) want_bits |= 1u << it;
            if constexpr (LOOK) look_mine = look_mine || (cnt > 1u && cnt < m);
          }
        }
        if constexpr (LOOK) {
          if (__ballot(look_mine) && lane == 0) s_look = 1;
        }
        if (!marks_out) {
#pragma unroll
          for (int it = 0; it < W; ++it)
            if ((mark_bits >> it) & 1u) a.solid_bytes[((uint64_t)wt[it] << 32) | wp[it]] = 1;
        } else {
          const uint32_t n_mk = (uint32_t)__builtin_popcount(mark_bits);
          const uint32_t incl = wave_inclusive_sum(n_mk);
          const uint32_t tot = __shfl(incl, kWave - 1, kWave);
          if (tot) {
            uint32_t mbase = 0;
            if (lane == 0) mbase = atomicAdd(&s_mark_cur, tot);
            mbase = __shfl(mbase, 0, kWave);
            uint32_t at = mbase + incl - n_mk;
#pragma unroll
            for (int it = 0; it < W; ++it)
              if ((mark_bits >> it) & 1u) {
                if (at < a.marks_cap) marks_out[at] = ((unsigned long long)wt[it] << 32) | wp[it];
                else atomicOr(a.err, 2u);
                ++at;
              }
          }
        }
        if constexpr (AGG) {
          const uint32_t n_w = (uint32_t)__builtin_popcount(want_bits);
          const uint32_t incl = wave_inclusive_sum(n_w);
          const uint32_t tot = __shfl(incl, kWave - 1, kWave);
          if (tot) {
            uint32_t lbase = 0;
            if (lane == 0) lbase = atomicAdd(&s_list_n2[rp], tot);
            lbase = __shfl(lbase, 0, kWave);
            uint32_t at = lbase + incl - n_w;
#pragma unroll
            for (int it = 0; it < W; ++it)
              if ((want_bits >> it) & 1u) {
                if (at < (uint32_t)NLIST) {
                  slist_k[at] = wk[it];
                  slist_c[at] = wc[it];
                } else {
                  emit_items(wk[it], wc[it], false, true);
                }
                ++at;
              }
          }
        }
        __syncthreads();
        if constexpr (AGG) {
          const uint32_t n_list = min(s_list_n2[rp], (uint32_t)NLIST);
          for (uint32_t base = 0; base < n_list; base += NT) {
            const uint32_t i = base + tid;
            const bool v = i < n_list;
            emit_items(v ? slist_k[i] : 0ull, v ? slist_c[i] : 0u, true, v);
          }
        }
        if constexpr (LOOK) {
          if (tid == 0 && !bad) {
            atomicAdd(a.err + 1, 1u);
            if (s_look) atomicAdd(a.err + 2, 1u);
          }
          if (s_look && !bad) {
            for (int q = 0; q < n_src; ++q) {
              const uint64_t lo = s_lo[q][bb], hi = s_lo[q][bb + 1];
              const uint4 *__restrict__ recs = srcs.ptr[q];
              for (uint64_t base = lo; base < hi; base += NT) {
                const bool in = base + tid < hi;
                const uint4 r = in ? recs[base + tid] : make_uint4(0u, 0u, 0u, 0u);
                const uint32_t len = in ? (r.z & 7u) + 1u : 0u;
                const uint8_t tag = TAGS ? (uint8_t)(r.x >> 28) : (uint8_t)0;
                uint32_t T;
                const uint32_t start = wave_exclusive_sum_4bit(len, &T);
                if (lane < 8) heads[wv][lane] = 0ull;
                __builtin_amdgcn_fence(__ATOMIC_RELEASE, "wavefront");
                __builtin_amdgcn_wave_barrier();
                if (len) atomicOr(&heads[wv][start >> 6], 1ull << (start & 63u));
                __builtin_amdgcn_fence(__ATOMIC_ACQ_REL, "wavefront");
                __builtin_amdgcn_wave_barrier();
                const unsigned long long hv = __hip_atomic_load(&heads[wv][lane & 7], __ATOMIC_RELAXED, __HIP_MEMORY_SCOPE_WORKGROUP);
                const uint32_t hv_lo = (uint32_t)hv, hv_hi = (uint32_t)(hv >> 32);
                SkmDealCarry dc;
                for (uint32_t c = 0; c * kWave < T; ++c) {
                  const uint32_t w_lo = (uint32_t)__builtin_amdgcn_readlane((int)hv_lo, (int)c), w_hi = (uint32_t)__builtin_amdgcn_readlane((int)hv_hi, (int)c);
                  const SkmDealAt d = skm_deal_at(((uint64_t)w_hi << 32) | w_lo, (uint32_t)lane, dc);
                  const uint32_t o = d.o, j = d.j & 7u;
                  const uint32_t xbh = __shfl(r.y, (int)o, kWave), xbl = __shfl(r.z, (int)o, kWave), p0 = __shfl(r.w, (int)o, kWave);
                  const uint64_t win = (((uint64_t)xbh << 32) | xbl) << (2 * j);
                  const uint64_t rc = skm_win_rc(win, k, kmask), f = (win << 2) & kmask;
                  const unsigned head = (unsigned)(win >> 62), tail = ((uint32_t)win >> (62 - 2 * k)) & 3u;
                  const unsigned long long key = skm_s1_key(f, rc, head, tail);
                  const uint32_t klo = (uint32_t)key, khi = (uint32_t)(key >> 32), pos = p0 + j;
                  [[maybe_unused]] uint32_t tg = 0;
                  if constexpr (TAGS) tg = (uint8_t)(__shfl((uint32_t)tag, (int)o, kWave) + (pos < p0 ? 1u : 0u));
                  bool mn = c * kWave + (uint32_t)lane < T;
                  if (sub) mn = mn && skm_in_round(skm_mix2((klo * 0xC2B2AE35u) ^ (khi * 0x27D4EB2Fu)), sub, rj);
                  if (mn) {
                    uint32_t h = ((klo * 0x9E3779B1u) ^ (khi * 0x85EBCA6Bu)) >> (32 - kSkmLogSlots);
                    int n = 0;
                    while (keys[h] != key && n < NSLOT) {
                      h = (h + 1) & (NSLOT - 1);
                      ++n;
                    }
                    if (n >= NSLOT) atomicOr(a.err, 4u);
                    else if (cnts[h] < m) a.solid_bytes[((uint64_t)tg << 32) | pos] = 1;
                  }
                }
              }
            }
          }
          __syncthreads();
#pragma unroll
          for (int it = 0; it < W; ++it) {
            const int sl = it * NT + tid;
            keys[sl] = kEmpty;
            cnts[sl] = 0;
          }
          if (tid == 0) s_look = 0;
          __syncthreads();
        }
        rp ^= 1;
        sub = nsub;
        rj = nrj;
        if (done) break;
      }
    }
  }
  __syncthreads();
  for (int i = tid; i < kSegHist; i += NT)
    if (lhist[i]) atomicAdd(&a.hist[i], (unsigned long long)lhist[i]);
  if (AGG && tid == 0) a.agg_counts[blockIdx.x] = s_agg_cur < a.agg_cap ? s_agg_cur : a.agg_cap;
  if (marks_out && tid == 0) a.marks_counts[blockIdx.x] = s_mark_cur < a.marks_cap ? s_mark_cur : a.marks_cap;
}

__global__ void k_count_hp_publish(const unsigned long long *__restrict__ hp, int k, uint32_t m, unsigned long long *__restrict__ hist,
                                   unsigned long long *__restrict__ edges_at, unsigned long long *__restrict__ res) {
  if (threadIdx.x || blockIdx.x) return;
  unsigned long long n_edges = 0, n_keys = 0, flagged = 0;
  for (int x = 0; x < 2; ++x) {
    const unsigned long long *t = hp + 8 + x * 16;
    const unsigned long long cnt = t[0];
    if (!cnt) continue;
    ++n_keys;
    const unsigned long long hb = cnt > MHX_MAX_MUL ? (unsigned long long)MHX_MAX_MUL : cnt;
    hist[hb] += 1;
    if (cnt >= m) {
      bool has_in = false, has_out = false;
      for (int c = 0; c < 4; ++c) {
        has_in = has_in || t[1 + c] >= m;
        has_out = has_out || t[5 + c] >= m;
      }
      if (!has_in || !has_out) flagged = 1;
// ... 399 lines not shown
      }
    }
  }
  n_dist_all = wave_sum(n_dist_all);
  if (lane == 0 && n_dist_all) atomicAdd(a.ctr + 4, n_dist_all);
  __syncthreads();
  for (int i = tid; i < kSegHist; i += NT)
    if (lhist[i]) atomicAdd(&a.hist[i], (unsigned long long)lhist[i]);
  if (tid == 0) a.edges_counts[blockIdx.x] = s_edge_cur < a.edges_cap ? s_edge_cur : a.edges_cap;
}

uint32_t s1_skm_max_m(const mhx_ctx *c) { return (uint32_t)std::min<long long>(std::max<long long>(c->opt<Opt::s1_skm_max_m>(), 2), 4); }

bool s1_skm_applies(const mhx_ctx *c, uint32_t k, uint32_t m, int want_mercy) {
  const SeqSet &s = c->seqs;
  const long long knob = c->opt<Opt::s1_skm>();
  if (!knob || want_mercy || c->global_bases || c->n_parts > 1 || c->filter_on || c->accumulate || c->pos_base) return false;
  if (k < 19 || k > 22 || m < 1 || m > s1_skm_max_m(c)) return false;
  if (!s.n_seqs || s.max_len < k + 1 || (s.n_bases >> 36)) return false;
  if (!s.fixed_len && (double)s.n_bases * 100.0 < (double)c->opt<Opt::s1_var_min_fill>() * (double)s.n_seqs * s.max_len) return false;
  const char *e = getenv("MHX_S1_MARK");
  if (e && strcmp(e, "nonsolid")) return false;
  const uint64_t n_win = s.n_bases > s.n_seqs * (uint64_t)k ? s.n_bases - s.n_seqs * (uint64_t)k : 0;
  return knob >= 2 || n_win >= (uint64_t)c->opt<Opt::s1_skm_min_windows>();
}

bool s1_skm_dist_applies(const mhx_ctx *c, uint32_t k, uint32_t m) {
  const SeqSet &s = c->seqs;
  if (!c->opt<Opt::s1_skm>() || !c->opt<Opt::dist_skm>() || !c->global_bases || c->n_parts > kSkmSrcMax || c->filter_on || c->accumulate) return false;
  if (k < 19 || k > 22 || m < 1 || m > 2 || (c->global_bases >> 36)) return false;
  if (!s.n_seqs || s.max_len < k + 1) return false;
  if (!s.fixed_len && (double)s.n_bases * 100.0 < (double)c->opt<Opt::s1_var_min_fill>() * (double)s.n_seqs * s.max_len) return false;
  if (getenv("MHX_S1_MARK") || !c->opt<Opt::dist_sparse_marks>()) return false;
  return s1_skm_passes(c, k) == 1;
}

int s1_skm_passes(const mhx_ctx *c, uint32_t k) {
  const SeqSet &s = c->seqs;
  if (const long long f = c->opt<Opt::s1_skm_passes>()) return (int)std::min<long long>(64, std::max<long long>(1, f));
  const uint64_t n_win = s.n_bases > s.n_seqs * (uint64_t)k ? s.n_bases - s.n_seqs * (uint64_t)k : 0;
  const double need = (double)n_win * (double)std::max<long long>(c->opt<Opt::s1_skm_cap_pct>(), 1) / 100.0 * 32.0;
  const double budget = (double)std::max<long long>(c->opt<Opt::s1_skm_pass_gb>(), 1) * 1e9;
  return (int)std::min(64.0, std::max(1.0, std::ceil(need / budget)));
}

bool s1_skm_front(mhx_ctx *c, uint32_t k, SkmFront *f, int pass, int n_passes, int bin_bits_agreed, bool for_count, bool bins_whole) {
  SeqSet &s = c->seqs;
  hipStream_t st = c->stream;
  const bool var = s.fixed_len == 0;
  const uint32_t L = var ? s.max_len : s.fixed_len, bpr = (L - k + kSkmC - 1) / kSkmC;
  const uint64_t n_blocks = s.n_seqs * (uint64_t)bpr;
  const uint64_t n_win = var ? (s.n_bases > s.n_seqs * (uint64_t)k ? s.n_bases - s.n_seqs * (uint64_t)k : 0) : s.n_seqs * (uint64_t)(L - k);
  const uint64_t cap_all = n_win * (uint64_t)std::max<long long>(c->opt<Opt::s1_skm_cap_pct>(), 1) / 100;
  const uint64_t cap = std::max<uint64_t>(n_passes > 1 ? cap_all / n_passes + cap_all / n_passes * 15 / 100 : cap_all, 1u << 16);
  int bin_bits = kSkmMinBinBits;
  while (bin_bits < kSkmMaxBinBits && (double)n_win * 0.29 / (double)(1ull << bin_bits) > 8192.0) ++bin_bits;
  if (const long long fb = c->opt<Opt::s1_skm_bin_bits>()) bin_bits = (int)std::min<long long>(kSkmMaxBinBits, std::max<long long>(8, fb));
  if (bin_bits_agreed > 0) bin_bits = bin_bits_agreed;
  std::vector<SortPass> passes;
  for (int lo = 0; lo < bin_bits; lo += 8) passes.push_back(SortPass{8 + lo, std::min(8, bin_bits - lo), 0, 0, 0});
  const std::vector<SortPass> passes_rest(passes.begin() + (passes.empty() ? 0 : 1), passes.end());
  bool split = c->opt<Opt::s1_skm_split>() != 0 && passes.size() >= 2 && sort_takes_split_first_pass(c, passes_rest);
  const uint64_t cap_split = std::max<uint64_t>(cap, 1u << 20), range_cap = cap_split / 256 / kSortSplitUnit * kSortSplitUnit;
  const uint64_t cap_alloc = split ? cap_split : cap;
  uint4 *buf_a = c->ws("items_a", cap_alloc * 16 + 64).as<uint4>();
  uint4 *buf_b = c->ws("items_b", cap_alloc * 16 + 64).as<uint4>();
  unsigned long long *cursor = c->ws("skm_cursor", 64).as<unsigned long long>();
  uint32_t *err = reinterpret_cast<uint32_t *>(cursor + 1);
  uint32_t *max_bin = err + 1;
  unsigned long long *split_cur = split ? c->ws("skm_split_cursors", (256 + 257) * 8).as<unsigned long long>() : nullptr;
  const uint32_t stage_n = (uint32_t)std::min<long long>(std::max<long long>(c->opt<Opt::s1_skm_split_stage>(kSkmStage), 0), kSkmStage);
  unsigned long long *pre_hist = c->ws("sort_pre_hist", (size_t)kMaxFusedPasses * 256 * 8).as<unsigned long long>();
  constexpr int NT = 512, J = 2;
  const uint64_t cus = c->n_cus > 0 ? (uint64_t)c->n_cus : 256;
  const long long grid_knob = c->opt<Opt::s1_skm_make_grid>();
  const unsigned grid = (unsigned)std::min<uint64_t>(div_ceil(n_blocks, (uint64_t)NT * J), grid_knob > 0 ? (uint64_t)grid_knob : cus * 8);
  const uint32_t n_bins = 1u << bin_bits;
  const uint32_t bin_lo = (uint32_t)((uint64_t)n_bins * pass / n_passes), bin_hi = (uint32_t)((uint64_t)n_bins * (pass + 1) / n_passes);
  unsigned long long *hp = nullptr;
  if ((!c->global_bases || for_count) && c->opt<Opt::s1_skm_hp>()) hp = c->ws("skm_hp", 512).as<unsigned long long>();
  const bool rep = hp && !c->global_bases && c->n_parts <= 1 && c->opt<Opt::s1_skm_rep>() != 0;
  if (rep) hp = c->ws("skm_hp", (size_t)(kSkmRepAt + kSkmRepN * 9) * 8).as<unsigned long long>();
  const unsigned long long rep_slots = (unsigned long long)std::min<long long>(std::max<long long>(c->opt<Opt::s1_skm_rep_slots>(), 0), 64);
  unsigned long long hp_init[48] = {0};
  hp_init[2] = hp_init[3] = ~0ull;
  unsigned long long h[4] = {0, 0, 0, 0};
  std::vector<unsigned long long> h_dh(passes.size() * 256), h_fill(256);
#define MHX_MAKE(VARV, COUNTV, SPLITV) MHX_MAKE_R(VARV, COUNTV, SPLITV, false)
#define MHX_MAKE_R(VARV, COUNTV, SPLITV, REPV)                                                                                                                           \
  hipLaunchKernelGGL((k_skm_make<NT, J, VARV, COUNTV, SPLITV, REPV>), dim3(grid), dim3(NT), 0, st, s.words.as<uint32_t>(), s.start.as<uint64_t>(), L, bpr, n_blocks, (int)k, \
                     bin_bits, bin_lo, bin_hi, pass == 0 ? 1 : 0, c->pos_base, hp, buf_a, (unsigned long long)cap, cursor, err, pre_hist,                            \
                     (unsigned long long)range_cap, split_cur, stage_n)
  auto make = [&](bool split_now) {
    MHX_HIP(hipMemsetAsync(cursor, 0, 64, st));
    MHX_HIP(hipMemsetAsync(pre_hist, 0, (size_t)3 * 256 * 8, st));
    if (split_now) MHX_HIP(hipMemsetAsync(split_cur, 0, 256 * 8, st));
    if (hp && pass == 0) MHX_HIP(hipMemcpyAsync(hp, hp_init, sizeof hp_init, hipMemcpyHostToDevice, st));
    if (rep && pass == 0) {
      MHX_HIP(hipMemsetAsync(hp + kSkmRepAt, 0, (size_t)kSkmRepN * 9 * 8, st));
      MHX_HIP(hipMemcpyAsync(hp + kSkmRepAt - 1, &rep_slots, 8, hipMemcpyHostToDevice, st));
      if (!for_count) MHX_HIP(hipMemsetAsync(hp + kSkmRepAt + kSkmRepN, 0xFF, (size_t)kSkmRepN * 8, st));
    }
    MHX_LAUNCH(c, for_count ? "count_skm_make" : "s1_skm_make", (double)s.n_bases / 4 + (double)n_win * 16 / 3.5, {
      if (rep && split_now) {
        if (var && for_count) MHX_MAKE_R(true, true, true, true);
        else if (var) MHX_MAKE_R(true, false, true, true);
        else if (for_count) MHX_MAKE_R(false, true, true, true);
        else MHX_MAKE_R(false, false, true, true);
      } else if (rep) {
        if (var && for_count) MHX_MAKE_R(true, true, false, true);
        else if (var) MHX_MAKE_R(true, false, false, true);
        else if (for_count) MHX_MAKE_R(false, true, false, true);
        else MHX_MAKE_R(false, false, false, true);
      } else if (split_now) {
        if (var && for_count) MHX_MAKE(true, true, true);
        else if (var) MHX_MAKE(true, false, true);
        else if (for_count) MHX_MAKE(false, true, true);
        else MHX_MAKE(false, false, true);
      } else {
        if (var && for_count) MHX_MAKE(true, true, false);
        else if (var) MHX_MAKE(true, false, false);
        else if (for_count) MHX_MAKE(false, true, false);
        else MHX_MAKE(false, false, false);
      }
    });
    MHX_HIP(hipMemcpyAsync(h, cursor, 32, hipMemcpyDeviceToHost, st));
    MHX_HIP(hipMemcpyAsync(h_dh.data(), pre_hist, h_dh.size() * 8, hipMemcpyDeviceToHost, st));
    if (split_now) MHX_HIP(hipMemcpyAsync(h_fill.data(), split_cur, 256 * 8, hipMemcpyDeviceToHost, st));
    MHX_HIP(hipStreamSynchronize(st));
  };
  make(split);
  if (split && ((uint32_t)h[1] & 2u)) {
    split = false;
    make(false);
  }
#undef MHX_MAKE
#undef MHX_MAKE_R
  if (split) {
    h[0] = 0;
    for (int d = 0; d < 256; ++d) h[0] += h_fill[d];
  }
  f->n_records = 0;
  f->hp = hp;
  f->rep = rep;
  f->giants = nullptr;
  f->n_giant_items = f->giant_limit = f->giant_bins = f->giant_largest = 0;
  f->why = nullptr;
  if ((uint32_t)h[1] != 0 || h[0] > cap) return false;
  const uint64_t n = h[0];
  const bool giant = !bins_whole && !c->global_bases && c->n_parts <= 1 && c->opt<Opt::s1_skm_giant>() != 0;
  SkmGiantKnobs gk;
  gk.max_records = (uint64_t)std::max<long long>(c->opt<Opt::s1_skm_giant_max>(), 1);
  gk.keys = (uint64_t)std::max<long long>(c->opt<Opt::s1_skm_giant_keys>(), 1);
  gk.work_pct = (uint64_t)std::max<long long>(c->opt<Opt::s1_skm_giant_work_pct>(), 0);
  gk.slices = (uint64_t)std::min<long long>(std::max<long long>(c->opt<Opt::s1_skm_giant_slices>(), 0), 1 << kSkmGiantMaxDepth);
  {
    const uint64_t n_bins_pass = std::max<uint64_t>(1, ((1ull << bin_bits) + n_passes - 1) / n_passes);
    const uint64_t limit = giant ? gk.max_records : std::max<uint64_t>((uint64_t)c->opt<Opt::s1_skm_max_bin>(), 16 * (n / n_bins_pass + 1));
    bool all = n > 0;
    uint64_t smallest_excess = ~0ull;
    for (size_t p = 0; p < passes.size() && all; ++p) {
      const uint64_t vals = 1ull << passes[p].bits;
      uint64_t mx = 0;
      for (uint64_t d = 0; d < vals; ++d) mx = std::max<uint64_t>(mx, h_dh[p * 256 + d]);
      const uint64_t mean = n / std::max<uint64_t>(1, (p + 1 == passes.size() && n_passes > 1) ? std::max<uint64_t>(1, vals / n_passes) : vals);
      const uint64_t excess = mx > mean ? mx - mean : 0;
      smallest_excess = std::min(smallest_excess, excess);
      all = excess >= limit + limit / 2;
    }
    if (all) {
      f->n_records = n;
      f->max_bin = (uint32_t)std::min<uint64_t>(smallest_excess, 0xFFFFFFFFu);
      if (giant) f->why = "beyond s1_skm_giant_max";
      return false;
    }
  }
  const std::vector<SortPass> &sort_passes = split ? passes_rest : passes;
  SortPrep prep;
  prep.buf = buf_a;
  prep.n = n;
  prep.hist_passes = (int)sort_passes.size();
  prep.hist_sig = passes_signature(sort_passes);
  std::vector<unsigned long long> h_ubase(257, 0);
  if (split) {
    for (int d = 0; d < 256; ++d) h_ubase[d + 1] = h_ubase[d] + div_ceil((uint64_t)h_fill[d], kSortSplitUnit);
    unsigned long long *ubase = split_cur + 256;
    MHX_HIP(hipMemcpyAsync(ubase, h_ubase.data(), 257 * 8, hipMemcpyHostToDevice, st));
    prep.split_fill = split_cur;
    prep.split_ubase = ubase;
    prep.split_units = h_ubase[256];
    prep.split_range_cap = range_cap;
    prep.hist_first = 1;
  }
  uint32_t *sorted = radix_sort(c, reinterpret_cast<uint32_t *>(buf_a), reinterpret_cast<uint32_t *>(buf_b), n, 4, 1, sort_passes, &prep);
  uint64_t *bounds = c->ws("s1_bucket_bounds", ((size_t)n_bins + 1) * 8 + 64).as<uint64_t>();
  MHX_LAUNCH(c, "s1_skm_bounds", (double)n_bins * 8 * 30,
             hipLaunchKernelGGL(k_skm_bounds, dim3((n_bins + 1 + 255) / 256), dim3(256), 0, st, reinterpret_cast<const uint4 *>(sorted), n, n_bins, bounds, max_bin));
  const uint64_t limit = std::max<uint64_t>((uint64_t)c->opt<Opt::s1_skm_max_bin>(), 16 * (n / (bin_hi - bin_lo) + 1));
  constexpr uint32_t kListCap = (uint32_t)kSkmGiantMaxBins + 1;
  uint2 *giant_list = nullptr;
  if (giant && bin_hi > bin_lo) {
    giant_list = c->ws("skm_giant_list", (size_t)(1 + kListCap) * 8).as<uint2>();
    MHX_HIP(hipMemsetAsync(giant_list, 0, 8, st));
    MHX_LAUNCH(c, "s1_skm_giants", (double)(bin_hi - bin_lo) * 8,
               hipLaunchKernelGGL(k_skm_giants, dim3((bin_hi - bin_lo + 255) / 256), dim3(256), 0, st, bounds, bin_lo, bin_hi, limit, giant_list, kListCap));
  }
  uint32_t h_max = 0;
  MHX_HIP(hipMemcpyAsync(&h_max, max_bin, 4, hipMemcpyDeviceToHost, st));
  MHX_HIP(hipStreamSynchronize(st));
  f->n_src = 1;
  f->src[0] = reinterpret_cast<const uint4 *>(sorted);
  f->src_bounds[0] = bounds;
  f->spare = sorted == reinterpret_cast<uint32_t *>(buf_a) ? reinterpret_cast<uint32_t *>(buf_b) : reinterpret_cast<uint32_t *>(buf_a);
  f->spare_bytes = cap_alloc * 16;
  f->n_records = n;
  f->n_windows = n_win;
  if (pass == 0) f->n_items = var ? h[3] : s.n_seqs * (uint64_t)(L - k + (for_count ? 0 : 4));
  f->n_bins = n_bins;
  f->bin_lo = bin_lo;
  f->bin_hi = bin_hi;
  f->bin_bits = bin_bits;
  f->max_bin = h_max;
  if (h_max <= limit) return true;
  if (!giant_list) return false;
  std::vector<uint2> h_list(1 + kListCap);
  MHX_HIP(hipMemcpyAsync(h_list.data(), giant_list, h_list.size() * 8, hipMemcpyDeviceToHost, st));
  MHX_HIP(hipStreamSynchronize(st));
  const uint32_t n_listed = h_list[0].x;
  std::vector<uint2> bins(h_list.begin() + 1, h_list.begin() + 1 + std::min(n_listed, kListCap));
  std::sort(bins.begin(), bins.end(), [](const uint2 &x, const uint2 &y) { return x.y != y.y ? x.y > y.y : x.x < y.x; });
  std::vector<uint64_t> recs(bins.size());
  for (size_t g = 0; g < bins.size(); ++g) recs[g] = bins[g].y;
  std::vector<uint8_t> depth(bins.size() + 1, 0);
  const double win_per_rec = n ? (double)n_win / (double)n_passes / (double)n : 1.0;
  switch (skm_giant_plan(recs.data(), (int)recs.size(), n, win_per_rec, gk, depth.data())) {
    case kSkmGiantServed: break;
    case kSkmGiantCap: f->why = "beyond s1_skm_giant_max"; return false;
    case kSkmGiantBudget: f->why = "its slices beyond s1_skm_giant_work_pct"; return false;
    default: f->why = "more than 1024 such bins"; return false;
  }
  std::vector<uint2> items;
  for (size_t g = 0; g < bins.size(); ++g)
    for (uint32_t rj0 = 0; rj0 < (1u << depth[g]); ++rj0) items.push_back(make_uint2(bins[g].x, ((uint32_t)depth[g] << 16) | rj0));
  uint2 *d_items = c->ws("skm_giant_items", items.size() * 8 + 64).as<uint2>();
  MHX_HIP(hipMemcpyAsync(d_items, items.data(), items.size() * 8, hipMemcpyHostToDevice, st));
  MHX_HIP(hipStreamSynchronize(st));
  f->giants = d_items;
  f->n_giant_items = (uint32_t)items.size();
  f->giant_limit = (uint32_t)std::min<uint64_t>(limit, 0xFFFFFFFFu);
  f->giant_bins = (uint32_t)bins.size();
  f->giant_largest = bins.empty() ? 0u : bins[0].y;
  return true;
}

void s1_skm_groups_launch(mhx_ctx *c, bool agg, unsigned grid, const SkmFront &f, uint32_t k, uint32_t m, uint8_t *solid_bytes, unsigned long long *hist,
                          uint2 *agg_raw, uint32_t agg_cap, uint32_t *agg_counts, uint32_t *err, unsigned long long *marks_raw, uint32_t marks_cap,
                          uint32_t *marks_counts) {
  hipStream_t st = c->stream;
  uint32_t *ticket = c->ws("s1_stream_ticket", 64).as<uint32_t>();
  MHX_HIP(hipMemsetAsync(ticket, 0, 4, st));
  const uint32_t nslot = 1u << kSkmLogSlots;
  SkmArgs a{(int)k, m, solid_bytes, hist, agg_raw, agg_cap, agg_counts, err,
            (uint32_t)std::min<long long>(std::max<long long>(c->opt<Opt::s1_stream_fill>(nslot * 7 / 8), 1), nslot), (int)std::min<long long>(c->opt<Opt::s1_stream_probes>(), 1024),
            f.bin_lo, f.bin_hi, marks_raw, marks_cap, marks_counts, f.giants, f.n_giant_items, f.giant_limit};
  const bool giant = f.n_giant_items != 0 && f.n_src == 1;
  SkmSrcs srcs{};
  srcs.n = f.n_src;
  for (int q = 0; q < f.n_src; ++q) {
    srcs.ptr[q] = f.src[q];
    srcs.bounds[q] = f.src_bounds[q];
  }
  const uint64_t n_bits = c->global_bases ? c->global_bases : c->seqs.n_bases;
  const bool tags = (n_bits >> 32) != 0 || c->opt<Opt::s1_skm_tags>() != 0;
  const long long deal = std::min<long long>(std::max<long long>(c->opt<Opt::s1_skm_deal>(), 0), 2);
#define MHX_SKM_G(AGGV, TAGV, GV)                                                                                                \
  do {                                                                                                                           \
    if (deal == 2) hipLaunchKernelGGL((k_s1_skm<AGGV, TAGV, 2, GV>), dim3(grid), dim3(kSkmThreads), 0, st, srcs, a, ticket);      \
    else if (deal == 1) hipLaunchKernelGGL((k_s1_skm<AGGV, TAGV, 1, GV>), dim3(grid), dim3(kSkmThreads), 0, st, srcs, a, ticket); \
    else hipLaunchKernelGGL((k_s1_skm<AGGV, TAGV, 0, GV>), dim3(grid), dim3(kSkmThreads), 0, st, srcs, a, ticket);                \
  } while (0)
#define MHX_SKM(AGGV, TAGV)                  \
  do {                                       \
    if (giant) MHX_SKM_G(AGGV, TAGV, true);  \
    else MHX_SKM_G(AGGV, TAGV, false);       \
  } while (0)
  const bool look = m >= 3;
  if (look && (marks_raw || giant)) throw Error("s1_skm_groups: min count 3 and 4 are served on one GPU, bins whole");
#define MHX_SKM_LOOK(AGGV, TAGV) hipLaunchKernelGGL((k_s1_skm<AGGV, TAGV, 2, false, true>), dim3(grid), dim3(kSkmThreads), 0, st, srcs, a, ticket)
  MHX_LAUNCH(c, "s1_skm_groups", (double)f.n_records * 16, {
    if (look && agg && tags) MHX_SKM_LOOK(true, true);
    else if (look && agg) MHX_SKM_LOOK(true, false);
    else if (look && tags) MHX_SKM_LOOK(false, true);
    else if (look) MHX_SKM_LOOK(false, false);
    else if (agg && tags) MHX_SKM(true, true);
    else if (agg) MHX_SKM(true, false);
    else if (tags) MHX_SKM(false, true);
    else MHX_SKM(false, false);
  });
#undef MHX_SKM_LOOK
#undef MHX_SKM
#undef MHX_SKM_G
}

bool count_skm_applies(const mhx_ctx *c, uint32_t k, uint32_t m) {
  const SeqSet &s = c->seqs;
  const long long knob = c->opt<Opt::count_skm>();
  if (!knob || !c->opt<Opt::s1_skm>() || c->global_bases || c->n_parts > 1 || c->filter_on || c->accumulate || c->pos_base) return false;
  if (k < 19 || k > 21 || m < 1 || m > s1_skm_max_m(c)) return false;
  if (!s.n_seqs || s.max_len < k + 1 || (s.n_bases >> 36)) return false;
  if (!s.fixed_len && (double)s.n_bases * 100.0 < (double)c->opt<Opt::s1_var_min_fill>() * (double)s.n_seqs * s.max_len) return false;
  const uint64_t n_win = s.n_bases > s.n_seqs * (uint64_t)k ? s.n_bases - s.n_seqs * (uint64_t)k : 0;
  return knob >= 2 || c->opt<Opt::s1_skm>() >= 2 || n_win >= (uint64_t)c->opt<Opt::s1_skm_min_windows>();
}
static uint32_t count_skm_launch(mhx_ctx *c, uint32_t k, uint32_t m, const SkmFront &f, unsigned grid, unsigned long long *edges_raw, uint32_t region, uint32_t *counts,
                                 uint32_t *first_0_out, uint32_t *last_0_in_p1, unsigned long long *hist, unsigned long long *ev_raw, uint32_t ev_cap,
                                 uint32_t *ev_counts, uint64_t *n_distinct) {
  SeqSet &s = c->seqs;
  hipStream_t st = c->stream;
  unsigned long long *ctr = c->ws("s1_counters", 64).as<unsigned long long>();
  uint32_t *seg_err = c->ws("s1_seg_err", 64).as<uint32_t>();
  uint32_t *ticket = c->ws("s1_stream_ticket", 64).as<uint32_t>();
  MHX_HIP(hipMemsetAsync(ctr, 0, 64, st));
  MHX_HIP(hipMemsetAsync(seg_err, 0, 4, st));
  MHX_HIP(hipMemsetAsync(ticket, 0, 4, st));
  if (ev_raw) MHX_HIP(hipMemsetAsync(ev_counts, 0, (size_t)grid * 4, st));
  const uint32_t nslot = 1u << kSkmLogSlots;
  CountSkmArgs a{(int)k, m, hist, ctr, edges_raw, region, counts, seg_err,
                 (uint32_t)std::min<long long>(std::max<long long>(c->opt<Opt::s1_stream_fill>(nslot * 7 / 8), 1), nslot), (int)std::min<long long>(c->opt<Opt::s1_stream_probes>(), 1024),
                 f.bin_lo, f.bin_hi, s.start.as<uint64_t>(), s.n_seqs, s.fixed_len, first_0_out, last_0_in_p1, ev_raw, ev_cap, ev_counts,
                 f.giants, f.n_giant_items, f.giant_limit};
  const bool giant = f.n_giant_items != 0 && f.n_src == 1 && !ev_raw;
  SkmSrcs srcs{};
  srcs.n = f.n_src;
  for (int q = 0; q < f.n_src; ++q) {
    srcs.ptr[q] = f.src[q];
    srcs.bounds[q] = f.src_bounds[q];
  }
  const uint64_t n_bits = c->global_bases ? c->global_bases : s.n_bases;
  const bool tags = (n_bits >> 32) != 0 || c->opt<Opt::s1_skm_tags>() != 0;
  const bool g2 = c->opt<Opt::count_skm_group>() == 2;
#define MHX_CSKM(EV, GV)                                                                                                                 \
  do {                                                                                                                                   \
    if (tags && g2) hipLaunchKernelGGL((k_count_skm<true, 2, EV, GV>), dim3(grid), dim3(kSkmThreads), 0, st, srcs, a, ticket);            \
    else if (tags) hipLaunchKernelGGL((k_count_skm<true, 4, EV, GV>), dim3(grid), dim3(kSkmThreads), 0, st, srcs, a, ticket);             \
    else if (g2) hipLaunchKernelGGL((k_count_skm<false, 2, EV, GV>), dim3(grid), dim3(kSkmThreads), 0, st, srcs, a, ticket);              \
    else hipLaunchKernelGGL((k_count_skm<false, 4, EV, GV>), dim3(grid), dim3(kSkmThreads), 0, st, srcs, a, ticket);                      \
  } while (0)
  const bool lv4 = m >= 3;
  if (lv4 && (ev_raw || giant)) throw Error("count_skm_groups: min count 3 and 4 are served on one GPU, bins whole");
  MHX_LAUNCH(c, "count_skm_groups", (double)f.n_records * 16, {
    if (lv4 && tags) hipLaunchKernelGGL((k_count_skm<true, 2, false, false, 4>), dim3(grid), dim3(kSkmThreads), 0, st, srcs, a, ticket);
    else if (lv4) hipLaunchKernelGGL((k_count_skm<false, 2, false, false, 4>), dim3(grid), dim3(kSkmThreads), 0, st, srcs, a, ticket);
    else if (ev_raw) MHX_CSKM(true, false);
    else if (giant) MHX_CSKM(false, true);
    else MHX_CSKM(false, false);
  });
#undef MHX_CSKM
  uint32_t e = 0;
  unsigned long long h_ctr[8] = {0};
  MHX_HIP(hipMemcpyAsync(&e, seg_err, 4, hipMemcpyDeviceToHost, st));
  MHX_HIP(hipMemcpyAsync(h_ctr, ctr, 64, hipMemcpyDeviceToHost, st));
  MHX_HIP(hipStreamSynchronize(st));
  *n_distinct = h_ctr[4];
  return e;
}

bool count_skm_groups(mhx_ctx *c, uint32_t k, uint32_t m, uint32_t *first_0_out, uint32_t *last_0_in_p1, unsigned long long *hist, CountStreamOut *o, bool *touched,
                      int pass, int n_passes) {
  SkmFront f{};
  if (!s1_skm_front(c, k, &f, pass, n_passes, 0, true, m >= 3)) {
    if (f.why) o->skm_why = "a bin of " + std::to_string(f.max_bin) + " records, " + f.why;
    return false;
// ... 66 lines not shown
  o->grid = grid;
  o->cap = region;
  o->counts = counts;
  o->spare = reinterpret_cast<uint32_t *>(edges_raw);
  o->sorted = nullptr;
  o->n_items = 0;
  o->n_distinct = n_distinct;
  o->events = ev_raw;
  o->n_events = n_events;
  o->ev_cap = ev_cap;
  o->ev_counts = ev_counts;
  o->skm_hp = nullptr;
  o->skm_records = f.n_records;
  o->skm_windows = 0;
  o->skm_max_bin = f.max_bin;
  o->skm_bin_bits = f.bin_bits;
  return true;
}

void count_skm_hp_publish(mhx_ctx *c, const unsigned long long *hp, uint32_t k, uint32_t m, unsigned long long *hist, unsigned long long *edges_at,
                          uint64_t *n_edges, uint64_t *n_keys, bool *flagged) {
  unsigned long long *res = c->ws("skm_hp_res", 64).as<unsigned long long>();
  hipLaunchKernelGGL(k_count_hp_publish, dim3(1), dim3(64), 0, c->stream, hp, (int)k, m, hist, edges_at, res);
  unsigned long long h[3] = {0, 0, 0};
  MHX_HIP(hipMemcpyAsync(h, res, 24, hipMemcpyDeviceToHost, c->stream));
  MHX_HIP(hipStreamSynchronize(c->stream));
  *n_edges = h[0];
  *n_keys = h[1];
  *flagged = h[2] != 0;
}

void s1_skm_hp_publish(mhx_ctx *c, const SkmFront &f, uint32_t k, uint32_t m, uint8_t *solid_bytes, unsigned long long *hist, uint2 *agg_items,
                       uint64_t *agg_cursor, bool agg, const DigitSpecs *agg_specs, unsigned long long *agg_hist) {
  if (!f.hp) return;
  DigitSpecs specs;
  specs.n = 0;
  if (agg_specs && agg_hist) specs = *agg_specs;
  MHX_LAUNCH(c, "s1_skm_hp", 64.0, hipLaunchKernelGGL(k_skm_hp_publish, dim3(1), dim3(64), 0, c->stream, f.hp, (int)k, m, solid_bytes, hist, agg_items, agg_cursor,
                                                       agg ? 1 : 0, specs, agg_specs ? agg_hist : nullptr));
}

uint64_t s1_skm_beside_below(mhx_ctx *c, const SkmFront &f, uint32_t k, uint32_t m) {
  if (!f.hp || m < 3) return 0;
  unsigned long long *res = c->ws("skm_hp_res", 64).as<unsigned long long>();
  hipLaunchKernelGGL(k_skm_beside_check, dim3(1), dim3(kSkmRepN), 0, c->stream, f.hp, f.rep ? 1 : 0, (int)k, m, res);
  unsigned long long h = 0;
  MHX_HIP(hipMemcpyAsync(&h, res, 8, hipMemcpyDeviceToHost, c->stream));
  MHX_HIP(hipStreamSynchronize(c->stream));
  return h;
}

uint64_t s1_skm_rep_publish(mhx_ctx *c, const SkmFront &f, uint32_t k, uint32_t m, uint8_t *solid_bytes, unsigned long long *hist, uint2 *agg_items,
                            uint64_t *agg_cursor, bool agg, const DigitSpecs *agg_specs, unsigned long long *agg_hist) {
  if (!f.hp || !f.rep) return 0;
  DigitSpecs specs;
  specs.n = 0;
  if (agg_specs && agg_hist) specs = *agg_specs;
  unsigned long long *res = c->ws("skm_hp_res", 64).as<unsigned long long>();
  MHX_LAUNCH(c, "s1_skm_rep", (double)kSkmRepN * 16,
             hipLaunchKernelGGL(k_skm_rep_publish, dim3(1), dim3(kSkmRepN), 0, c->stream, f.hp + kSkmRepAt, (int)k, m, solid_bytes, hist, agg_items,
                                reinterpret_cast<unsigned long long *>(agg_cursor), agg ? 1 : 0, specs, agg_specs ? agg_hist : nullptr, res));
  unsigned long long h[2] = {0, 0};
  MHX_HIP(hipMemcpyAsync(h, res, 16, hipMemcpyDeviceToHost, c->stream));
  MHX_HIP(hipStreamSynchronize(c->stream));
  return h[0];
}

void count_skm_rep_publish(mhx_ctx *c, const unsigned long long *hp, uint32_t k, uint32_t m, unsigned long long *hist, unsigned long long *edges_at,
                           uint64_t *n_edges, uint64_t *n_keys, bool *flagged, uint64_t *n_windows) {
  unsigned long long *res = c->ws("skm_hp_res", 64).as<unsigned long long>();
  MHX_LAUNCH(c, "count_skm_rep", (double)kSkmRepN * 72,
             hipLaunchKernelGGL(k_count_rep_publish, dim3(1), dim3(kSkmRepN), 0, c->stream, hp + kSkmRepAt, (int)k, m, hist, edges_at, res));
  unsigned long long h[4] = {0, 0, 0, 0};
  MHX_HIP(hipMemcpyAsync(h, res, 32, hipMemcpyDeviceToHost, c->stream));
  MHX_HIP(hipStreamSynchronize(c->stream));
  *n_edges = h[0];
  *n_keys = h[1];
  *flagged = h[2] != 0;
  *n_windows = h[3];
}

void s1_skm_bounds_of(mhx_ctx *c, const uint4 *recs, uint64_t n, uint32_t n_bins, uint64_t *bounds) {
  uint32_t *scratch = c->ws("skm_cursor", 64).as<uint32_t>() + 8;
  hipLaunchKernelGGL(k_skm_bounds, dim3((n_bins + 1 + 255) / 256), dim3(256), 0, c->stream, recs, n, n_bins, bounds, scratch);
}

}
```

megahit_amd/csrc/sort.hip:

```cpp
#include "dev_prims.h"
#include <cstdlib>
#include <cstring>
#include <string>

#include "mhx_internal.h"
#include "sort_digits.h"
#include "sort_kernels.h"

namespace mhx {

template <int S, int NI>
__global__ __launch_bounds__(kSortThreads) void k_radix_hist(const uint32_t *__restrict__ items, uint64_t n, DigitSpec ds,
                                                             uint32_t *__restrict__ hist, uint64_t n_chunks,
                                                             const uint8_t *__restrict__ lut) {
  __shared__ uint32_t h[kSortWaves][256];
  for (int i = threadIdx.x; i < kSortWaves * 256; i += kSortThreads) (&h[0][0])[i] = 0;
  __syncthreads();
  const int w = threadIdx.x / kWave;
  const uint64_t base = (uint64_t)blockIdx.x * SortCfg<S, NI>::kChunk;
  for (int j = 0; j < SortCfg<S, NI>::kChunk / kSortThreads; ++j) {
    uint64_t idx = base + (uint64_t)j * kSortThreads + threadIdx.x;
    if (idx < n) {
      const uint32_t *p = items + idx * S;
      unsigned d;
// ... 197 lines not shown
}

DigitSpec spec_of_pass(const SortPass &ps, int key_words) {
  DigitSpec ds{key_words - 1 - ps.shift / 32, (unsigned)(ps.shift % 32), (1u << ps.bits) - 1, 0, 0u, 0u, 0u};
  if (ps.bits2) {
    ds.wi2 = key_words - 1 - ps.shift2 / 32;
    ds.bit2 = (unsigned)(ps.shift2 % 32);
    ds.mask2 = (1u << ps.bits2) - 1;
    ds.sh2 = (unsigned)ps.bits;
  }
  if (ps.prev_lo >= 0 && ps.prev_lo < ps.shift && !ps.bits2 && ps.prev_lo / 32 == (ps.shift + ps.bits - 1) / 32) {
    const unsigned hi = (unsigned)(ps.shift % 32), lo = (unsigned)(ps.prev_lo % 32);
    ds.prev_mask = ((1u << hi) - 1u) & ~((1u << lo) - 1u);
  }
  return ds;
}

struct SortEnv {
  bool classic;
  std::string shape;
  int items;
};
static SortEnv sort_env() {
  const char *e = getenv("MHX_SORT"), *sh = getenv("MHX_SORT_SHAPE"), *it = getenv("MHX_SORT_ITEMS");
  return SortEnv{e && !strcmp(e, "classic"), sh ? sh : "", it ? atoi(it) : 0};
}
static void refuse_unconsumed_generator(const SortPrep &prep, const char *who) {
  if (prep.gen) throw Error(std::string(who) + ": the records of this buffer are to be made by a generated first pass, which this sort path cannot run");
  if (prep.split_fill) throw Error(std::string(who) + ": the records of this buffer lie in ranges split by an earlier digit, which this sort path cannot read");
}

template <int S, int NI, int UT>
static uint32_t *radix_sort_onesweep(mhx_ctx *c, uint32_t *a, uint32_t *b, uint64_t n, int key_words, const std::vector<SortPass> &passes,
                                     const SortPrep &prep) {
  const int P = (int)passes.size();
  const bool prep_fits = prep.buf == (const void *)a && prep.n == n;
  const bool gen = prep.gen && prep_fits && S == 3 && NI == 8 && UT == 3;
  constexpr bool kCanSplit = S == 4 && NI == 8 && UT == 2;
  static_assert(!kCanSplit || (uint64_t)kSortThreads * NI * UT == kSortSplitUnit, "a unit of the split pass");
  const bool split = kCanSplit && !prep.gen && prep.split_fill && prep.split_ubase && prep_fits && c->opt<Opt::sort_unit_runs>() != 0 &&
                     prep.split_range_cap > 0 && prep.split_range_cap % kSortSplitUnit == 0;
  if (!gen && !split) refuse_unconsumed_generator(prep, "radix sort (chained scan)");
  const uint64_t gen_slots = gen ? std::max<uint64_t>(prep.gen_slots, n) : (split ? prep.split_units * kSortSplitUnit : n);
  const int xcd_units = c->opt<Opt::sort_xcd_units>() != 0 && c->n_cus >= 192;
  const uint64_t unit = (uint64_t)kSortThreads * NI * UT;
  auto units_of = [&](uint64_t items) { return xcd_units ? (div_ceil(items, unit) + 127) / 128 * 128 : div_ceil(items, unit); };
  const uint64_t n_units = units_of(n), n_units_gen = units_of(gen_slots);
  hipStream_t st = c->stream;
  constexpr bool kCanUt2 = S == 3 && NI == 8 && UT == 3;
  const bool loaded_ut2 = kCanUt2 && c->opt<Opt::sort_loaded_ut2>() != 0;
  const uint64_t unit2 = (uint64_t)kSortThreads * NI * 2;
  const uint64_t n_units2 = xcd_units ? (div_ceil(n, unit2) + 127) / 128 * 128 : div_ceil(n, unit2);
  const uint64_t n_status = std::max(n_units_gen, loaded_ut2 ? n_units2 : 0);
  unsigned long long *status = c->ws("sort_status", n_status * 256 * 8).as<unsigned long long>();
  unsigned long long *gh = c->ws("sort_ghist", (size_t)2 * kMaxChainedPasses * 256 * 8).as<unsigned long long>();
  unsigned long long *starts = gh + kMaxChainedPasses * 256;
  constexpr int kErrSlot = kMaxChainedPasses * 8;
  uint32_t *tickets = c->ws("sort_tickets", (kErrSlot + 8) * 4).as<uint32_t>();
  MHX_HIP(hipMemsetAsync(status, 0, n_status * 256 * 8, st));
  MHX_HIP(hipMemsetAsync(gh, 0, (size_t)kMaxChainedPasses * 256 * 8, st));
  MHX_HIP(hipMemsetAsync(tickets, 0, (kErrSlot + 8) * 4, st));
  const double bytes = (double)n * S * 4;
  static const std::string nm_hist = "radix_hist_all_" + std::to_string(S * 4) + "B", nm_scat = "radix_scatter_" + std::to_string(S * 4) + "B";
  const unsigned hgrid = (unsigned)std::min<uint64_t>(div_ceil(n, (uint64_t)kSortThreads * 16), 4096);
  std::vector<DigitSpec> all(P);
  for (int p = 0; p < P; ++p) all[p] = spec_of_pass(passes[p], key_words);
  const bool pre = prep_fits && prep.hist_passes == P && P > 0 && P <= kMaxFusedPasses && prep.hist_sig == passes_signature(passes);
  if (gen && !pre) throw Error("radix sort: a generated first pass needs the digit histograms of the plan (pre-hist)");
  if (split && !pre) throw Error("radix sort: a split first pass needs the digit histograms of the plan (pre-hist)");
  if (pre)
    MHX_HIP(hipMemcpyAsync(gh, (prep.hist ? prep.hist : static_cast<const unsigned long long *>(c->work["sort_pre_hist"].p)) + (size_t)prep.hist_first * 256,
                           (size_t)P * 256 * 8, hipMemcpyDeviceToDevice, st));
  for (int p0 = 0; p0 < P && !pre; p0 += kMaxFusedPasses) {
    DigitSpecs specs;
    specs.n = std::min(kMaxFusedPasses, P - p0);
    for (int p = 0; p < specs.n; ++p) specs.d[p] = all[p0 + p];
    MHX_LAUNCH(c, nm_hist.c_str(), bytes,
               hipLaunchKernelGGL((k_radix_hist_all<S>), dim3(hgrid), dim3(kSortThreads), 0, st, a, n, specs, gh + (size_t)p0 * 256));
  }
  hipLaunchKernelGGL(k_bin_starts, dim3(P), dim3(256), 0, st, gh, starts);
  constexpr bool kHasUnitRuns = (S <= 3 && NI == 8 && (UT == 3 || UT == 2)) || (S == 4 && NI == 8 && UT == 2) || (S > 4 && NI == 4 && UT == 2);
  const bool unit_runs = kHasUnitRuns && c->opt<Opt::sort_unit_runs>() != 0;
  const bool rank_uniform = unit_runs && c->opt<Opt::sort_rank_uniform>() != 0;
  for (int p = 0; p < P; ++p) {
    const int nb = passes[p].bits + passes[p].bits2;
    const int wi = digit_word_of(all[p], nb, 1);
    if (p == 0 && gen) {
      static const std::string nm_gen = nm_scat + "_gen";
      MHX_LAUNCH(c, nm_gen.c_str(), bytes,
                 prep.gen(OnesweepLaunch{(unsigned)n_units_gen, st, b, gen_slots, all[p], nb, starts + p * 256, status, tickets + p * 8,
                                    tickets + kErrSlot, (unsigned long long)(p + 1), xcd_units, unit_runs ? 1 : 0, wi}));
    } else if (p == 0 && split) {
      if constexpr (kCanSplit) {
#define MHX_US(RANKV, WIV)                                                                                                                        \
  hipLaunchKernelGGL((k_radix_onesweep_u<S, NI, UT, SrcSplit<S>, RANKV, WIV>), dim3((unsigned)n_units_gen), dim3(kSortThreads), 0, st,            \
                     SrcSplit<S>{a, prep.split_fill, prep.split_ubase, prep.split_range_cap}, b, gen_slots, all[p], nb, starts + p * 256, status, tickets + p * 8, \
                     tickets + kErrSlot, (unsigned long long)(p + 1), xcd_units)
        MHX_LAUNCH(c, nm_scat.c_str(), 2 * bytes, {
          if (wi == 0 && rank_uniform && all[p].prev_mask) MHX_US(2, 0);
          else if (wi == 0) MHX_US(0, 0);
          else MHX_US(0, -1);
        });
#undef MHX_US
      }
    } else if (unit_runs) {
      if constexpr (kHasUnitRuns) {
#define MHX_U(RANKV, WIV)                                                                                                                      \
  hipLaunchKernelGGL((k_radix_onesweep_u<S, NI, UT, SrcArray<S>, RANKV, WIV>), dim3((unsigned)n_units), dim3(kSortThreads), 0, st, SrcArray<S>{a}, b, \
                     n, all[p], nb, starts + p * 256, status, tickets + p * 8, tickets + kErrSlot, (unsigned long long)(p + 1), xcd_units)
#define MHX_U2(RANKV, WIV)                                                                                                                     \
  hipLaunchKernelGGL((k_radix_onesweep_u<S, NI, 2, SrcArray<S>, RANKV, WIV>), dim3((unsigned)n_units2), dim3(kSortThreads), 0, st, SrcArray<S>{a}, b, \
                     n, all[p], nb, starts + p * 256, status, tickets + p * 8, tickets + kErrSlot, (unsigned long long)(p + 1), xcd_units)
        if constexpr (kCanUt2) {
          if (loaded_ut2 && wi == 0) {
            MHX_LAUNCH(c, nm_scat.c_str(), 2 * bytes, {
              if (rank_uniform && all[p].prev_mask) MHX_U2(2, 0);
              else MHX_U2(0, 0);
            });
            std::swap(a, b);
            continue;
          }
        }
#undef MHX_U2
        MHX_LAUNCH(c, nm_scat.c_str(), 2 * bytes, {
          if (wi == 0 && rank_uniform && all[p].prev_mask) MHX_U(2, 0);
          else if (wi == 0) MHX_U(0, 0);
          else if (wi == 1) MHX_U(0, 1);
          else MHX_U(0, -1);
        });
#undef MHX_U
      }
    } else {
      MHX_LAUNCH(c, nm_scat.c_str(), 2 * bytes,
                 hipLaunchKernelGGL((k_radix_onesweep<S, NI, UT, SrcArray<S>>), dim3((unsigned)n_units), dim3(kSortThreads), 0, st, SrcArray<S>{a}, b, n,
                                    all[p], nb, starts + p * 256, status, tickets + p * 8, tickets + kErrSlot,
                                    (unsigned long long)(p + 1), xcd_units));
    }
    std::swap(a, b);
  }
  uint32_t e = 0;
  MHX_HIP(hipMemcpyAsync(&e, tickets + kErrSlot, 4, hipMemcpyDeviceToHost, st));
  MHX_HIP(hipStreamSynchronize(st));
  if (e) throw Error("radix sort: chained scan timed out waiting for a predecessor unit (set MHX_SORT=classic)");
  return a;
}

template <int S, int NI>
static uint32_t *radix_sort_impl2(mhx_ctx *c, uint32_t *a, uint32_t *b, uint64_t n, int key_words,
                                  const std::vector<SortPass> &passes, const SortPrep &prep) {
  if (n == 0) return a;
  const SortEnv env = sort_env();
  if constexpr (S <= 8 && NI == default_items<S>()) {
    const bool classic = env.classic;
    if (!classic && passes.size() <= (size_t)kMaxChainedPasses && div_ceil(n, (uint64_t)kSortThreads * 8) < (1ull << 31)) {
      if constexpr (S <= 4) {
        const std::string shape = !env.shape.empty() ? env.shape : (S <= 3 ? "8x3" : "8x2");
        if (shape == "8x2") return radix_sort_onesweep<S, 8, 2>(c, a, b, n, key_words, passes, prep);
        if (shape == "4x4") return radix_sort_onesweep<S, 4, 4>(c, a, b, n, key_words, passes, prep);
        if (shape == "16x1") return radix_sort_onesweep<S, 16, 1>(c, a, b, n, key_words, passes, prep);
        if (shape == "8x4" && S <= 3) return radix_sort_onesweep<S, 8, 4>(c, a, b, n, key_words, passes, prep);
        if (shape == "8x3" || S <= 3) return radix_sort_onesweep<S, 8, 3>(c, a, b, n, key_words, passes, prep);
        return radix_sort_onesweep<S, 8, 2>(c, a, b, n, key_words, passes, prep);
      } else {
        return radix_sort_onesweep<S, 4, 2>(c, a, b, n, key_words, passes, prep);
      }
    }
  }
  refuse_unconsumed_generator(prep, "radix sort (classic passes)");
  const uint64_t n_chunks = div_ceil(n, SortCfg<S, NI>::kChunk);
  uint32_t *hist = c->ws("sort_hist", n_chunks * 256 * 4).as<uint32_t>();
  uint64_t *offs = c->ws("sort_offs", n_chunks * 256 * 8).as<uint64_t>();
  const double bytes = (double)n * S * 4;
  static const std::string nm_hist = "radix_hist_" + std::to_string(S * 4) + "B", nm_scat = "radix_scatter_" + std::to_string(S * 4) + "B";
  auto spec_of = [&](const SortPass &ps) {
    DigitSpec ds{key_words - 1 - ps.shift / 32, (unsigned)(ps.shift % 32), (1u << ps.bits) - 1, 0, 0u, 0u, 0u};
    if (ps.bits2) {
      ds.wi2 = key_words - 1 - ps.shift2 / 32;
      ds.bit2 = (unsigned)(ps.shift2 % 32);
      ds.mask2 = (1u << ps.bits2) - 1;
      ds.sh2 = (unsigned)ps.bits;
    }
    return ds;
  };
#ifdef MHX_TILE_TIMING
  const bool use_side = getenv("MHX_SORT_SIDE_DIGITS") != nullptr;
#else
  constexpr bool use_side = false;
#endif
  uint8_t *dnext = use_side && passes.size() > 1 ? c->ws("sort_digits", n + 64).as<uint8_t>() : nullptr;
  static const std::string nm_histb = "radix_hist_bytes";
  for (size_t pi = 0; pi < passes.size(); ++pi) {
    const SortPass &ps = passes[pi];
    const DigitSpec ds = spec_of(ps);
    const bool last = pi + 1 == passes.size();
    const DigitSpec ds_next = last ? ds : spec_of(passes[pi + 1]);
#ifdef MHX_TILE_TIMING
    const bool dbg_identity = getenv("MHX_DEBUG_IDENTITY_SCATTER") != nullptr;
#else
    constexpr bool dbg_identity = false;
#endif
    const int nbits = dbg_identity ? -(ps.bits + ps.bits2) : ps.bits + ps.bits2;
    if (pi == 0 || !dnext)
      MHX_LAUNCH(c, nm_hist.c_str(), bytes,
                 hipLaunchKernelGGL((k_radix_hist<S, NI>), dim3((unsigned)n_chunks), dim3(kSortThreads), 0, c->stream, a, n, ds, hist,
                                    n_chunks, (const uint8_t *)nullptr));
    else
      MHX_LAUNCH(c, nm_histb.c_str(), (double)n,
                 hipLaunchKernelGGL((k_radix_hist_bytes<SortCfg<S, NI>::kChunk>), dim3((unsigned)n_chunks), dim3(kSortThreads), 0,
                                    c->stream, dnext, n, hist, n_chunks));
    exclusive_scan_u32_u64(c, hist, offs, n_chunks * 256, nullptr);
    uint8_t *dn = last ? nullptr : dnext;
#ifdef MHX_TILE_TIMING
    const unsigned lds_pad = getenv("MHX_SORT_LDS_PAD") ? (unsigned)atoi(getenv("MHX_SORT_LDS_PAD")) : 0u;
#else
    constexpr unsigned lds_pad = 0u;
#endif
    MHX_LAUNCH(c, nm_scat.c_str(), 2 * bytes + (dn ? (double)n : 0.0),
               hipLaunchKernelGGL((k_radix_scatter<S, NI>), dim3((unsigned)n_chunks), dim3(kSortThreads), lds_pad, c->stream, a, b, n, ds,
                                  nbits, offs, n_chunks, (const uint8_t *)nullptr, ds_next, dn));
    std::swap(a, b);
  }
  return a;
}

template <int S>
static uint32_t *radix_sort_impl(mhx_ctx *c, uint32_t *a, uint32_t *b, uint64_t n, int key_words,
                                 const std::vector<SortPass> &passes, const SortPrep &prep) {
  if constexpr (S <= 4) {
    const SortEnv env = sort_env();
    const int items = env.items ? env.items : default_items<S>();
    if (items == 2) return radix_sort_impl2<S, 2>(c, a, b, n, key_words, passes, prep);
    if (items == 3) return radix_sort_impl2<S, 3>(c, a, b, n, key_words, passes, prep);
    if (items == 6) return radix_sort_impl2<S, 6>(c, a, b, n, key_words, passes, prep);
    if (items == 16) return radix_sort_impl2<S, 16>(c, a, b, n, key_words, passes, prep);
    if (items == 8) return radix_sort_impl2<S, 8>(c, a, b, n, key_words, passes, prep);
    if (items == 12) return radix_sort_impl2<S, 12>(c, a, b, n, key_words, passes, prep);
  }
  return radix_sort_impl2<S, default_items<S>()>(c, a, b, n, key_words, passes, prep);
}

constexpr int kSegWalkLimit = 4096;

template <int S>
__global__ __launch_bounds__(256) void k_seg_finish(const uint32_t *__restrict__ in, uint32_t *__restrict__ out, uint64_t n, int kw,
                                                    uint32_t pfx_mask, uint32_t *__restrict__ err) {
  const uint64_t stride = (uint64_t)gridDim.x * 256;
  for (uint64_t gi = (uint64_t)blockIdx.x * 256 + threadIdx.x; gi < n; gi += stride) {
    Rec<S> me;
    load_rec<S>(in + gi * S, me);
    const uint32_t r0 = me.w[0];
    auto cmp = [&](uint64_t x) -> int {
// ... 72 lines not shown
    const double avg = pbits >= 40 ? 0.0 : (double)n / (double)(1ull << pbits);
    return (14.0 + 4.5 * stride) + std::max(0.0, avg - 1.0) * (2.0 + 0.8 * stride);
  };
  int best_bits = 0;
  double best = (double)passes.size() * pass_ps;
  for (int pbits = 8; pbits <= 32; pbits += 8) {
    const double t = (pbits / 8) * pass_ps + finish_ps(pbits) + (double)c->opt<Opt::sort_hybrid_margin_ps>();
    if ((double)n / (double)(1ull << pbits) <= 64.0 && t < best) {
      best = t;
      best_bits = pbits;
    }
  }
  if (mode == 2 && !best_bits) {
    best_bits = 8;
    while (best_bits < 32 && (double)n / 4.0 > (double)(1ull << best_bits)) best_bits += 8;
  }
  if (const long long f = c->opt<Opt::sort_hybrid_bits>()) best_bits = (int)std::min<long long>(32, std::max<long long>(1, f));
  if (!best_bits) return radix_sort(c, a, b, n, stride, key_words, passes, prep);
  uint32_t *sorted = radix_sort(c, a, b, n, stride, key_words, make_passes(key_words, key_words * 32 - best_bits, key_words * 32), prep);
  uint32_t *other = sorted == a ? b : a;
  if (seg_finish(c, sorted, other, n, stride, key_words, best_bits)) return other;
  return radix_sort(c, sorted, other, n, stride, key_words, passes);
}

template <int S>
static void partition_impl(mhx_ctx *c, const uint32_t *a, uint32_t *b, uint64_t n, const uint8_t *lut, int n_parts, uint64_t *counts) {
  for (int p = 0; p < n_parts; ++p) counts[p] = 0;
  if (n == 0) return;
  const uint64_t n_chunks = div_ceil(n, SortCfg<S, default_items<S>()>::kChunk);
  uint32_t *hist = c->ws("sort_hist", n_chunks * 256 * 4).as<uint32_t>();
  uint64_t *offs = c->ws("sort_offs", (n_chunks * 256 + 1) * 8).as<uint64_t>();
  const double bytes = (double)n * S * 4;
  int nbits = 1;
  while ((1 << nbits) < n_parts) ++nbits;
  MHX_LAUNCH(c, "owner_hist", bytes,
             hipLaunchKernelGGL((k_radix_hist<S, default_items<S>()>), dim3((unsigned)n_chunks), dim3(kSortThreads), 0, c->stream, a, n, DigitSpec{0, 0u, 0xFFu, 0, 0u, 0u, 0u}, hist,
                                n_chunks, lut));
  exclusive_scan_u32_u64(c, hist, offs, n_chunks * 256, offs + n_chunks * 256);
  MHX_LAUNCH(c, "owner_scatter", 2 * bytes,
             hipLaunchKernelGGL((k_radix_scatter<S, default_items<S>()>), dim3((unsigned)n_chunks), dim3(kSortThreads), 0, c->stream, a, b, n, DigitSpec{0, 0u, 0xFFu, 0, 0u, 0u, 0u},
                                nbits, offs, n_chunks, lut, DigitSpec{0, 0u, 0xFFu, 0, 0u, 0u, 0u}, (uint8_t *)nullptr));
  std::vector<uint64_t> starts(n_parts + 1);
  for (int p = 0; p <= n_parts; ++p)
    MHX_HIP(hipMemcpyAsync(&starts[p], offs + (uint64_t)p * n_chunks, 8, hipMemcpyDeviceToHost, c->stream));
  MHX_HIP(hipStreamSynchronize(c->stream));
  for (int p = 0; p < n_parts; ++p) counts[p] = starts[p + 1] - starts[p];
}

void partition_by_owner(mhx_ctx *c, const uint32_t *a, uint32_t *b, uint64_t n, int stride, const uint8_t *lut, int n_parts,
                        uint64_t *counts) {
  if (n_parts > 256) throw Error("partition_by_owner: at most 256 owners");
  switch (stride) {
    case 2: return partition_impl<2>(c, a, b, n, lut, n_parts, counts);
    case 3: return partition_impl<3>(c, a, b, n, lut, n_parts, counts);
    case 4: return partition_impl<4>(c, a, b, n, lut, n_parts, counts);
    case 6: return partition_impl<6>(c, a, b, n, lut, n_parts, counts);
    case 8: return partition_impl<8>(c, a, b, n, lut, n_parts, counts);
    case 10: return partition_impl<10>(c, a, b, n, lut, n_parts, counts);
    case 12: return partition_impl<12>(c, a, b, n, lut, n_parts, counts);
    case 14: return partition_impl<14>(c, a, b, n, lut, n_parts, counts);
    case 16: return partition_impl<16>(c, a, b, n, lut, n_parts, counts);
    case 18: return partition_impl<18>(c, a, b, n, lut, n_parts, counts);
    case 20: return partition_impl<20>(c, a, b, n, lut, n_parts, counts);
    default: throw Error("partition_by_owner: unsupported record stride");
  }
}

bool sort_takes_generated_first_pass(const mhx_ctx *c, uint64_t n, int stride, const std::vector<SortPass> &passes) {
  (void)c;
  const SortEnv env = sort_env();
  if (env.classic) return false;
  if ((!env.shape.empty() && env.shape != "8x3") || (env.items && env.items != default_items<3>())) return false;
  return stride == 3 && n > 0 && passes.size() <= (size_t)kMaxChainedPasses && passes.size() <= (size_t)kMaxFusedPasses &&
         div_ceil(n, (uint64_t)kSortThreads * 8) < (1ull << 31);
}

bool sort_takes_split_first_pass(const mhx_ctx *c, const std::vector<SortPass> &passes) {
  const SortEnv env = sort_env();
  if (env.classic || c->opt<Opt::sort_unit_runs>() == 0) return false;
  if ((!env.shape.empty() && env.shape != "8x2") || (env.items && env.items != default_items<4>())) return false;
  return !passes.empty() && passes.size() <= (size_t)kMaxChainedPasses && passes.size() <= (size_t)kMaxFusedPasses;
}

uint32_t *radix_sort(mhx_ctx *c, uint32_t *a, uint32_t *b, uint64_t n, int stride, int key_words,
                     const std::vector<SortPass> &passes, SortPrep *prep_io) {
  SortPrep prep;
  if (prep_io) std::swap(prep, *prep_io);
  switch (stride) {
    case 2: return radix_sort_impl<2>(c, a, b, n, key_words, passes, prep);
    case 3: return radix_sort_impl<3>(c, a, b, n, key_words, passes, prep);
    case 4: return radix_sort_impl<4>(c, a, b, n, key_words, passes, prep);
    case 6: return radix_sort_impl<6>(c, a, b, n, key_words, passes, prep);
    case 8: return radix_sort_impl<8>(c, a, b, n, key_words, passes, prep);
    case 10: return radix_sort_impl<10>(c, a, b, n, key_words, passes, prep);
    case 12: return radix_sort_impl<12>(c, a, b, n, key_words, passes, prep);
    case 14: return radix_sort_impl<14>(c, a, b, n, key_words, passes, prep);
    case 16: return radix_sort_impl<16>(c, a, b, n, key_words, passes, prep);
    case 18: return radix_sort_impl<18>(c, a, b, n, key_words, passes, prep);
    case 20: return radix_sort_impl<20>(c, a, b, n, key_words, passes, prep);
    default: throw Error("radix_sort: unsupported record stride");
  }
}

}
```

megahit_amd/csrc/sort_kernels.h:

```cpp
#pragma once
#include "dev_prims.h"
#include "sort_digits.h"

namespace mhx {

constexpr int kSortThreads = 256;
constexpr int kSortWaves = kSortThreads / kWave;

template <int S>
constexpr int default_items() {
  return (S <= 4) ? 4 : (S <= 8 ? 8 : (S <= 12 ? 5 : (S <= 16 ? 4 : 3)));
}
template <int S, int ITEMS>
struct SortCfg {
  static constexpr int kItems = ITEMS;
  static constexpr int kTile = kSortThreads * kItems;
  static constexpr int kTilesPerChunk = (16384 / kTile) > 4 ? (16384 / kTile) : 4;
  static constexpr int kChunk = kTile * kTilesPerChunk;
};

template <int S>
struct Rec {
  uint32_t w[S];
};
// ... 199 lines not shown
          const uint64_t m = __ballot(bitset);
          peers &= bitset ? m : ~m;
        }
        const uint32_t before = wave_cnt[w][d];
        rank[j] = before + __builtin_popcountll(peers & lanemask_lt);
        __builtin_amdgcn_wave_barrier();
        if (valid && (peers & lanemask_lt) == 0) wave_cnt[w][d] = before + __builtin_popcountll(peers);
        __builtin_amdgcn_wave_barrier();
      }
    }
    __syncthreads();
    {
      uint32_t c[kSortWaves], tot = 0;
#pragma unroll
      for (int i = 0; i < kSortWaves; ++i) {
        c[i] = wave_cnt[i][tid];
        tot += c[i];
      }
      const uint32_t start = block_exclusive_sum<uint32_t, kSortThreads>(tot, sm_scan, nullptr);
      uint32_t run = start;
#pragma unroll
      for (int i = 0; i < kSortWaves; ++i) {
        wave_cnt[i][tid] = run;
        run += c[i];
      }
      if (t == 0) {
        unsigned long long excl = 0;
        if (unit > 0) {
          for (uint64_t p = unit; p-- > 0;) {
            unsigned long long v;
            uint32_t polls = 0;
            for (;;) {
              v = __hip_atomic_load(status + p * 256 + tid, __ATOMIC_RELAXED, __HIP_MEMORY_SCOPE_AGENT);
              if ((v >> 58) == tag && ((v >> 56) & 3ull)) break;
              if (++polls > (1u << 27)) {
                atomicOr(err, 1u);
                v = 2ull << 56;
                break;
              }
              if (polls < 64) __builtin_amdgcn_s_sleep(1);
              else __builtin_amdgcn_s_sleep(8);
            }
            excl += v & kStValMask;
            if (((v >> 56) & 3ull) == 2ull) break;
          }
          __hip_atomic_store(st, tagbits | (2ull << 56) | (excl + unit_tot), __ATOMIC_RELAXED, __HIP_MEMORY_SCOPE_AGENT);
        }
        g_base[tid] = bin_start[tid] + excl;
      }
      g_off[tid] = (long long)g_base[tid] - (long long)start;
      g_base[tid] += tot;
    }
    __syncthreads();
#pragma unroll
    for (int j = 0; j < NI; ++j) {
      const int li = w * (kWave * NI) + j * kWave + lane;
      if (li < tile_n) store_rec<S>(stage + (size_t)(wave_cnt[w][dig[j]] + rank[j]) * S, rec[t][j]);
    }
    __syncthreads();
#pragma unroll
    for (int j = 0; j < NI; ++j) {
      const int li = j * kSortThreads + tid;
      if (li < tile_n) {
        Rec<S> r;
        load_rec<S>(stage + (size_t)li * S, r);
        const unsigned d = rec_digit2<S>(r, ds);
        store_rec<S>(out + (uint64_t)(g_off[d] + li) * S, r);
      }
    }
    __syncthreads();
  }
}


template <int S, int WI>
__device__ __forceinline__ unsigned rec_digit_w(const Rec<S> &r, const DigitSpec &ds) {
  if constexpr (WI >= 0) return (r.w[WI] >> ds.bit1) & ds.mask1;
  else return rec_digit2<S>(r, ds);
}
inline int digit_word_of(const DigitSpec &ds, int nbits, int max_word) {
  return (ds.mask2 == 0 && ds.wi1 >= 0 && ds.wi1 <= max_word && (int)ds.bit1 + nbits <= 32) ? ds.wi1 : -1;
}

template <int S, int NI, int UT, class Src, int RANK, int WI>
__global__ __launch_bounds__(kSortThreads) void k_radix_onesweep_u(Src src, uint32_t *__restrict__ out, uint64_t n, DigitSpec ds, int nbits,
                                                                   const unsigned long long *__restrict__ bin_start,
                                                                   unsigned long long *__restrict__ status, uint32_t *__restrict__ ticket,
                                                                   uint32_t *__restrict__ err, unsigned long long tag, int xcd_units) {
  constexpr int kTile = kSortThreads * NI;
  static_assert(kTile * (UT + 1) < 0xFFFF, "16-bit ranks and positions");
  __shared__ __attribute__((aligned(16))) uint32_t stage[kTile * S];
  __shared__ uint32_t cnt[UT][kSortWaves][256];
  __shared__ long long g_off[256];
  __shared__ uint32_t sm_scan[kSortThreads / kWave + 1];
  __shared__ uint32_t s_unit;

  const int tid = threadIdx.x, w = tid / kWave, lane = tid & (kWave - 1);
  const uint64_t lanemask_lt = (1ull << lane) - 1;
  if (tid == 0) {
    if (xcd_units) {
      const uint32_t cls = blockIdx.x & 7u, tk = atomicAdd(ticket + cls, 1u);
      s_unit = ((tk >> 4) * 8 + cls) * 16 + (tk & 15u);
    } else {
      s_unit = atomicAdd(ticket, 1u);
    }
  }
#pragma unroll
  for (int t = 0; t < UT; ++t)
#pragma unroll
    for (int i = 0; i < kSortWaves; ++i) cnt[t][i][tid] = 0;
  __syncthreads();
  const uint64_t unit = s_unit;
  const uint64_t unit_base = unit * (uint64_t)(kTile * UT);

  Rec<S> rec[UT][NI];
  src.template get_unit<NI, UT>(unit_base, w, lane, n, rec);

  uint32_t pk[UT][(NI + 1) / 2];
#pragma unroll
  for (int t = 0; t < UT; ++t) {
#pragma unroll
    for (int h = 0; h < (NI + 1) / 2; ++h) pk[t][h] = 0xFFFFFFFFu;
#pragma unroll
    for (int j = 0; j < NI; ++j) {
      const uint64_t gi = src.template index<NI>(unit_base + (uint64_t)t * kTile, w, lane, j);
      bool valid = gi < n;
      if constexpr (Src::kMayDrop) valid = valid && src.is_record(rec[t][j]);
      const unsigned d = valid ? rec_digit_w<S, WI>(rec[t][j], ds) : 0u;
      uint32_t rk;
      bool by_atomic = RANK == 1;
      if constexpr (RANK == 2) {
        static_assert(WI >= 0, "RANK 2 needs the digit and the bits sorted before it in one word");
        const uint64_t vm = __ballot(valid);
        const uint32_t pv = valid ? (rec[t][j].w[WI >= 0 ? WI : 0] & ds.prev_mask) : 0u;
        const uint32_t p0 = __shfl(pv, vm ? __builtin_ctzll(vm) : 0, kWave);
        by_atomic = __ballot(valid && pv != p0) == 0;
      }
      if (by_atomic) {
        rk = valid ? atomicAdd(&cnt[t][w][d], 1u) : 0xFFFFu;
      } else {
        uint64_t peers = __ballot(valid);
        for (int b = 0; b < nbits; ++b) {
          const bool bitset = (d >> b) & 1u;
          const uint64_t m = __ballot(bitset);
          peers &= bitset ? m : ~m;
        }
        const uint32_t before = cnt[t][w][d];
        rk = valid ? before + __builtin_popcountll(peers & lanemask_lt) : 0xFFFFu;
        __builtin_amdgcn_wave_barrier();
        if (valid && (peers & lanemask_lt) == 0) cnt[t][w][d] = before + __builtin_popcountll(peers);
        __builtin_amdgcn_wave_barrier();
      }
      pk[t][j >> 1] = (j & 1) ? ((pk[t][j >> 1] & 0xFFFFu) | (rk << 16)) : ((pk[t][j >> 1] & 0xFFFF0000u) | rk);
      asm volatile("" : "+v"(pk[t][j >> 1]));
    }
  }
  __syncthreads();

  uint32_t unit_records = 0;
  {
    uint32_t c[UT][kSortWaves], tot = 0;
#pragma unroll
    for (int t = 0; t < UT; ++t)
#pragma unroll
      for (int i = 0; i < kSortWaves; ++i) {
        c[t][i] = cnt[t][i][tid];
        tot += c[t][i];
      }
    unsigned long long *const st = status + unit * 256 + tid;
    const unsigned long long tagbits = tag << 58;
    __hip_atomic_store(st, tagbits | ((unit == 0 ? 2ull : 1ull) << 56) | (unsigned long long)tot, __ATOMIC_RELAXED, __HIP_MEMORY_SCOPE_AGENT);
    const uint32_t start = block_exclusive_sum<uint32_t, kSortThreads>(tot, sm_scan, &unit_records);
    uint32_t run = start;
#pragma unroll
    for (int t = 0; t < UT; ++t)
#pragma unroll
      for (int i = 0; i < kSortWaves; ++i) {
        cnt[t][i][tid] = run;
        run += c[t][i];
      }
    unsigned long long excl = 0;
    if (unit > 0 && unit_base < n) {
      for (uint64_t p = unit; p-- > 0;) {
        unsigned long long v;
        uint32_t polls = 0;
        for (;;) {
          v = __hip_atomic_load(status + p * 256 + tid, __ATOMIC_RELAXED, __HIP_MEMORY_SCOPE_AGENT);
          if ((v >> 58) == tag && ((v >> 56) & 3ull)) break;
          if (++polls > (1u << 27)) {
            atomicOr(err, 1u);
            v = 2ull << 56;
            break;
          }
          if (polls < 64) __builtin_amdgcn_s_sleep(1);
          else __builtin_amdgcn_s_sleep(8);
        }
        excl += v & kStValMask;
        if (((v >> 56) & 3ull) == 2ull) break;
      }
      __hip_atomic_store(st, tagbits | (2ull << 56) | (excl + (unsigned long long)tot), __ATOMIC_RELAXED, __HIP_MEMORY_SCOPE_AGENT);
    }
    g_off[tid] = (long long)(bin_start[tid] + excl) - (long long)start;
  }
  __syncthreads();

#pragma unroll
  for (int t = 0; t < UT; ++t)
#pragma unroll
    for (int j = 0; j < NI; ++j) {
      const uint32_t rk = (pk[t][j >> 1] >> ((j & 1) * 16)) & 0xFFFFu;
      if (rk != 0xFFFFu) {
        const uint32_t p = cnt[t][w][rec_digit_w<S, WI>(rec[t][j], ds)] + rk;
        pk[t][j >> 1] = (j & 1) ? ((pk[t][j >> 1] & 0xFFFFu) | (p << 16)) : ((pk[t][j >> 1] & 0xFFFF0000u) | p);
      }
    }
  const uint64_t rem = n > unit_base ? n - unit_base : 0;
  const uint32_t unit_n = Src::kMayDrop ? unit_records : (rem < (uint64_t)(kTile * UT) ? (uint32_t)rem : (uint32_t)(kTile * UT));
#pragma unroll
  for (int r = 0; r < UT; ++r) {
    const uint32_t lo = (uint32_t)r * kTile;
    if (lo >= unit_n) break;
#pragma unroll
    for (int t = 0; t < UT; ++t)
#pragma unroll
      for (int j = 0; j < NI; ++j) {
        const uint32_t rel = ((pk[t][j >> 1] >> ((j & 1) * 16)) & 0xFFFFu) - lo;
        if (rel < (uint32_t)kTile) store_rec<S>(stage + (size_t)rel * S, rec[t][j]);
      }
    __syncthreads();
#pragma unroll
    for (int j = 0; j < NI; ++j) {
      const uint32_t li = (uint32_t)(j * kSortThreads + tid);
      if (lo + li < unit_n) {
        Rec<S> rr;
        load_rec<S>(stage + (size_t)li * S, rr);
        const unsigned d = rec_digit_w<S, WI>(rr, ds);
        store_rec<S>(out + (uint64_t)(g_off[d] + (long long)(lo + li)) * S, rr);
      }
    }
    __syncthreads();
  }
}

struct OnesweepLaunch {
  unsigned grid;
  hipStream_t stream;
  uint32_t *out;
  uint64_t n;
  DigitSpec ds;
  int nbits;
  const unsigned long long *bin_start;
  unsigned long long *status;
  uint32_t *ticket, *err;
  unsigned long long tag;
  int xcd_units;
  int unit_runs;
  int wi;
};

}
```

Measured before the change: 57350 M edges/s.

## Write 12-byte records from last sort pass and recompute bins from bases

The final radix pass of the super-k-mer sort now drops the first word of each 16-byte record and writes 12-byte records. The bin is recomputed from the packed bases wherever it is needed, in the bounds search and in the group kernel loads. This is meant to cut global memory traffic in the last scatter and in the grouping kernel. It also adds an optional path, off by default, that zeroes the solid byte map on a side stream overlapping the make kernel. The cost is extra hash recomputation in the binary search and unaligned 12-byte loads.

```diff
diff --git a/megahit_amd/csrc/mhx_internal.h b/megahit_amd/csrc/mhx_internal.h
--- a/megahit_amd/csrc/mhx_internal.h
+++ b/megahit_amd/csrc/mhx_internal.h
@@ -162,6 +162,7 @@
   const unsigned long long *split_fill = nullptr, *split_ubase = nullptr;
   uint64_t split_range_cap = 0, split_units = 0;
   int hist_first = 0;
+  int last_words = 0;
 };
 uint32_t *radix_sort(mhx_ctx *c, uint32_t *buf_a, uint32_t *buf_b, uint64_t n, int stride, int key_words,
                      const std::vector<SortPass> &passes, SortPrep *prep = nullptr);
@@ -170,6 +171,7 @@
 std::vector<SortPass> make_passes(int key_words, int lo_bit, int hi_bit);
 bool sort_takes_generated_first_pass(const mhx_ctx *c, uint64_t n, int stride, const std::vector<SortPass> &passes);
 bool sort_takes_split_first_pass(const mhx_ctx *c, const std::vector<SortPass> &passes);
+bool sort_takes_narrow_last_pass(const mhx_ctx *c, const std::vector<SortPass> &passes, int key_words);
 constexpr uint64_t kSortSplitUnit = 4096;
 uint64_t passes_signature(const std::vector<SortPass> &ps);
 uint32_t *kmsort_exact(mhx_ctx *c, uint32_t *buf_a, uint32_t *buf_b, uint64_t n, int S, int key_words, SortPrep *prep = nullptr);
@@ -203,6 +205,7 @@
 struct SkmFront {
   int n_src;
   const uint4 *src[kSkmSrcMax];
+  int rec_words;
   const uint64_t *src_bounds[kSkmSrcMax];
   uint32_t *spare;
   uint64_t spare_bytes;
@@ -217,7 +220,9 @@
   uint32_t n_giant_items, giant_limit;
   uint32_t giant_bins, giant_largest;
   const char *why;
-};
+  uint64_t zeroed_bits;
+};
+inline size_t s1_byte_map_bytes(uint64_t n_bits) { return (size_t)((n_bits + 63) / 64 + 1) * 64; }
 bool s1_skm_applies(const mhx_ctx *c, uint32_t k, uint32_t m, int want_mercy);
 bool s1_skm_dist_applies(const mhx_ctx *c, uint32_t k, uint32_t m);
 int s1_skm_passes(const mhx_ctx *c, uint32_t k);
diff --git a/megahit_amd/csrc/mhx_options.h b/megahit_amd/csrc/mhx_options.h
--- a/megahit_amd/csrc/mhx_options.h
+++ b/megahit_amd/csrc/mhx_options.h
@@ -105,6 +105,8 @@
   X(s1_skm_max_bin, 1 << 16)       \
   X(s1_skm_tags, 0)                \
   X(s1_skm_deal, 2)                \
+  X(s1_skm_zero_in_make, 0)        \
+  X(s1_skm_narrow, 1)              \
   X(count_skm_group, 2)            \
   X(count_skm_ev_cap, 0)           \
                        \
diff --git a/megahit_amd/csrc/s1.hip b/megahit_amd/csrc/s1.hip
--- a/megahit_amd/csrc/s1.hip
+++ b/megahit_amd/csrc/s1.hip
@@ -412,6 +412,7 @@
   bool list_local = false;
   unsigned long long *is_solid = nullptr, *hist = nullptr, *ctr = nullptr;
   uint8_t *solid_bytes = nullptr;
+  uint64_t front_zeroed_bits = 0;
   uint64_t marks_prev = 0, seg_marks = 0;
   const uint32_t *giant_ctr = nullptr;
   bool classic_ran = false;
@@ -458,9 +459,11 @@
   }
   void ensure_byte_map() {
     if (solid_bytes) return;
-    const uint64_t nw = div_ceil(n_bits, 64);
-    solid_bytes = c->ws("solid_bytes", (nw + 1) * 64).as<uint8_t>();
-    if (!acc || sparse) MHX_HIP(hipMemsetAsync(solid_bytes, 0, (nw + 1) * 64, st));
+    const size_t bytes = s1_byte_map_bytes(n_bits);
+    solid_bytes = c->ws("solid_bytes", bytes).as<uint8_t>();
+    if (acc && !sparse) return;
+    const uint64_t done = front_zeroed_bits == n_bits ? n_bits : 0;
+    MHX_LAUNCH(c, "s1_byte_map_zero", (double)(bytes - done), MHX_HIP(hipMemsetAsync(solid_bytes + done, 0, bytes - done, st)));
   }
   void open_outputs() {
     n_bits = global ? c->global_bases : s.n_bases;
@@ -1165,7 +1168,10 @@
       }
     }
     stage.set_spare(f.spare);
-    if (p == 0) stage.open_outputs();
+    if (p == 0) {
+      stage.front_zeroed_bits = f.zeroed_bits;
+      stage.open_outputs();
+    }
     if (!stage.run_skm(f)) {
       *why = "an output region overflowed";
       return false;
@@ -1185,6 +1191,7 @@
            (unsigned long long)n_records, (unsigned long long)f.n_windows, n_records ? (double)f.n_windows / (double)n_records : 0.0, max_bin,
            c->seqs.fixed_len ? "" : " [reads of several lengths]");
   c->last_s1_plan = txt;
+  if (f.rec_words == 3) c->last_s1_plan += " [12-byte sorted records]";
   if (n_passes > 1) c->last_s1_plan += " [" + std::to_string(n_passes) + " passes over ranges of bins]";
   if (f.rep) c->last_s1_plan += " [" + std::to_string(n_rep) + " windows of period <= 4 beside the records]";
   if (giant_bins)
diff --git a/megahit_amd/csrc/s1_skm.hip b/megahit_amd/csrc/s1_skm.hip
--- a/megahit_amd/csrc/s1_skm.hip
+++ b/megahit_amd/csrc/s1_skm.hip
@@ -1,27 +1,18 @@
 #include <cstring>
 
 #include "s1_shared.h"
+#include "skm_bins.h"
 #include "skm_deal.h"
 #include "skm_giant.h"
 
 namespace mhx {
 
-constexpr int kSkmC = 8;
-constexpr int kSkmW = 10;
-constexpr int kSkmNM = kSkmC + kSkmW - 1;
 constexpr int kSkmMinBinBits = 16, kSkmMaxBinBits = 20;
 
-__device__ __forceinline__ uint32_t skm_mix(uint32_t c) {
-  uint32_t h = c * 0x9E3779B1u;
-  return h ^ (h >> 15);
-}
 __device__ __forceinline__ uint32_t skm_mix2(uint32_t c) {
   uint32_t h = c * 0x9E3779B1u;
   h ^= h >> 15;
   return h * 0x85EBCA6Bu;
-}
-__device__ __forceinline__ uint32_t skm_bin_of(uint32_t minh) {
-  return (minh ^ (minh >> 16)) * 0x7FEB352Du;
 }
 
 constexpr int kSkmStage = 2560;
@@ -59,8 +50,6 @@
   if (SPLIT && tid < 256) dcnt[tid] = 0;
   __syncthreads();
   const bool third_digit = bin_bits > 16;
-  const int M = k + 1 - (kSkmW - 1);
-  const uint32_t mmask = (1u << (2 * M)) - 1u;
   const int K1 = k + 1;
   const unsigned bin_sh = 32u - (unsigned)bin_bits;
   unsigned long long items = 0;
@@ -190,25 +179,8 @@
           const uint32_t c0 = fc[j][0], c1 = fc[j][1], c2 = fc[j][2];
           const uint64_t W = ((uint64_t)funnel_l(c0, c1, sh) << 32) | funnel_l(c1, c2, sh);
           const uint64_t R = rc64(W, 32);
-          uint32_t h[kSkmNM];
-#pragma unroll
-          for (int i = 0; i < kSkmNM; ++i) {
-            const uint32_t f = (uint32_t)(W >> (64 - 2 * (i + M))) & mmask;
-            const uint32_t rv = (uint32_t)(R >> (2 * i)) & mmask;
-            h[i] = skm_mix(min(f, rv));
-          }
-          uint32_t sfx[kSkmW];
-          sfx[kSkmW - 1] = h[kSkmW - 1];
-#pragma unroll
-          for (int i = kSkmW - 2; i >= 0; --i) sfx[i] = min(h[i], sfx[i + 1]);
-          uint32_t pfx = 0xFFFFFFFFu;
           uint32_t bins[kSkmC];
-          bins[0] = skm_bin_of(sfx[0]) >> bin_sh;
-#pragma unroll
-          for (int w = 1; w < kSkmC; ++w) {
-            pfx = min(pfx, h[kSkmW - 1 + w]);
-            bins[w] = skm_bin_of(min(sfx[w], pfx)) >> bin_sh;
-          }
+          skm_block_bins(W, R, k, bin_sh, bins);
 #pragma unroll
           for (int w = 0; w < kSkmC; ++w) lbin[j * kSkmC + w][tid] = bins[w];
           const uint32_t n_here = min((uint32_t)kSkmC, nwin - q0);
@@ -603,15 +575,17 @@
   if (e == 0) *res = s_worst;
 }
 
-__global__ __launch_bounds__(256) void k_skm_bounds(const uint4 *__restrict__ recs, uint64_t n, uint32_t n_bins, uint64_t *__restrict__ bounds,
-                                                    uint32_t *__restrict__ max_bin) {
+__global__ __launch_bounds__(256) void k_skm_bounds(const uint32_t *__restrict__ recs, int words, uint64_t n, uint32_t n_bins, uint64_t *__restrict__ bounds,
+                                                    uint32_t *__restrict__ max_bin, int k, unsigned bin_sh) {
   const uint32_t b = blockIdx.x * 256 + threadIdx.x;
   if (b > n_bins) return;
   auto lower = [&](uint32_t v) -> uint64_t {
     uint64_t lo = 0, hi = n;
     while (lo < hi) {
       const uint64_t mid = (lo + hi) >> 1;
-      const uint32_t bin = (reinterpret_cast<const uint32_t *>(recs + mid)[0] >> 8) & 0xFFFFFu;
+      uint32_t bin;
+      if (words == 3) bin = skm_first_bin(((uint64_t)recs[mid * 3] << 32) | recs[mid * 3 + 1], k, bin_sh);
+      else bin = (recs[mid * 4] >> 8) & 0xFFFFFu;
       if (bin < v) lo = mid + 1;
       else hi = mid;
     }
@@ -659,7 +633,21 @@
   const uint4 *ptr[kSkmSrcMax];
   const uint64_t *bounds[kSkmSrcMax];
   int n;
+  int narrow;
 };
+struct SkmRec3 {
+  uint32_t y, z, w;
+};
+template <bool TAGS>
+__device__ __forceinline__ uint4 skm_load_rec(const uint4 *__restrict__ recs, uint64_t i, bool narrow) {
+  if constexpr (TAGS) {
+    return recs[i];
+  } else {
+    const uint32_t stride = narrow ? 12u : 16u, first = narrow ? 0u : 4u;
+    const SkmRec3 r = *reinterpret_cast<const SkmRec3 *>(reinterpret_cast<const char *>(recs) + (i * stride + first));
+    return make_uint4(0u, r.y, r.z, r.w);
+  }
+}
 
 constexpr int kSkmThreads = 1024, kSkmLogSlots = 13;
 
@@ -713,6 +701,7 @@
     if constexpr (LOOK) s_look = 0;
   }
   const int n_src = srcs.n;
+  const bool narrow = !TAGS && srcs.narrow != 0;
   unsigned long long *const marks_out = a.marks_raw ? a.marks_raw + (size_t)blockIdx.x * a.marks_cap : nullptr;
   int rp = 0;
   __syncthreads();
@@ -793,12 +782,12 @@
         const uint64_t lo = s_lo[q][bb], hi = s_lo[q][bb + 1];
         if (lo == hi) continue;
         const uint4 *__restrict__ recs = srcs.ptr[q];
-        uint4 nxt = q == 0 && pre_ok && pre_at == lo ? pre : (lo + tid < hi ? recs[lo + tid] : make_uint4(0u, 0u, 0u, 0u));
+        uint4 nxt = q == 0 && pre_ok && pre_at == lo ? pre : (lo + tid < hi ? skm_load_rec<TAGS>(recs, lo + tid, narrow) : make_uint4(0u, 0u, 0u, 0u));
         if (q == 0) pre_ok = false;
         for (uint64_t base = lo; base < hi; base += NT) {
           const uint4 r = nxt;
           const bool in = base + tid < hi;
-          if (base + NT + tid < hi) nxt = recs[base + NT + tid];
+          if (base + NT + tid < hi) nxt = skm_load_rec<TAGS>(recs, base + NT + tid, narrow);
           if (seen > a.max_fill) continue;
           const uint32_t len = in ? (r.z & 7u) + 1u : 0u;
           const uint8_t tag = TAGS ? (uint8_t)(r.x >> 28) : (uint8_t)0;
@@ -1038,7 +1027,7 @@
               }
           }
           if (nlo != nhi) {
-            pre = nlo + tid < nhi ? srcs.ptr[0][nlo + tid] : make_uint4(0u, 0u, 0u, 0u);
+            pre = nlo + tid < nhi ? skm_load_rec<TAGS>(srcs.ptr[0], nlo + tid, narrow) : make_uint4(0u, 0u, 0u, 0u);
             pre_at = nlo;
             pre_ok = true;
           }
@@ -1143,7 +1132,7 @@
               const uint4 *__restrict__ recs = srcs.ptr[q];
               for (uint64_t base = lo; base < hi; base += NT) {
                 const bool in = base + tid < hi;
-                const uint4 r = in ? recs[base + tid] : make_uint4(0u, 0u, 0u, 0u);
+                const uint4 r = in ? skm_load_rec<TAGS>(recs, base + tid, narrow) : make_uint4(0u, 0u, 0u, 0u);
                 const uint32_t len = in ? (r.z & 7u) + 1u : 0u;
                 const uint8_t tag = TAGS ? (uint8_t)(r.x >> 28) : (uint8_t)0;
                 uint32_t T;
@@ -1709,6 +1698,30 @@
   const bool rep = hp && !c->global_bases && c->n_parts <= 1 && c->opt<Opt::s1_skm_rep>() != 0;
   if (rep) hp = c->ws("skm_hp", (size_t)(kSkmRepAt + kSkmRepN * 9) * 8).as<unsigned long long>();
   const unsigned long long rep_slots = (unsigned long long)std::min<long long>(std::max<long long>(c->opt<Opt::s1_skm_rep_slots>(), 0), 64);
+  uint8_t *zero_map = nullptr;
+  if (pass == 0 && !for_count && !var && !c->global_bases && c->n_parts <= 1 && !c->accumulate && c->opt<Opt::s1_skm_zero_in_make>() != 0)
+    zero_map = c->ws("solid_bytes", s1_byte_map_bytes(s.n_bases)).as<uint8_t>();
+  bool zero_started = false;
+  auto zero_fork = [&]() -> hipEvent_t {
+    if (!zero_map || zero_started) return nullptr;
+    while (c->side_streams.size() < 1) {
+      hipStream_t ns;
+      MHX_HIP(hipStreamCreateWithFlags(&ns, hipStreamNonBlocking));
+      c->side_streams.push_back(ns);
+    }
+    while (c->side_events.size() < 2) {
+      hipEvent_t ne;
+      MHX_HIP(hipEventCreateWithFlags(&ne, hipEventDisableTiming));
+      c->side_events.push_back(ne);
+    }
+    hipStream_t ss = c->side_streams[0];
+    MHX_HIP(hipEventRecord(c->side_events[0], st));
+    MHX_HIP(hipStreamWaitEvent(ss, c->side_events[0], 0));
+    MHX_HIP(hipMemsetAsync(zero_map, 0, s.n_bases, ss));
+    MHX_HIP(hipEventRecord(c->side_events[1], ss));
+    zero_started = true;
+    return c->side_events[1];
+  };
   unsigned long long hp_init[48] = {0};
   hp_init[2] = hp_init[3] = ~0ull;
   unsigned long long h[4] = {0, 0, 0, 0};
@@ -1728,6 +1741,7 @@
       MHX_HIP(hipMemcpyAsync(hp + kSkmRepAt - 1, &rep_slots, 8, hipMemcpyHostToDevice, st));
       if (!for_count) MHX_HIP(hipMemsetAsync(hp + kSkmRepAt + kSkmRepN, 0xFF, (size_t)kSkmRepN * 8, st));
     }
+    const hipEvent_t zeroed = zero_fork();
     MHX_LAUNCH(c, for_count ? "count_skm_make" : "s1_skm_make", (double)s.n_bases / 4 + (double)n_win * 16 / 3.5, {
       if (rep && split_now) {
         if (var && for_count) MHX_MAKE_R(true, true, true, true);
@@ -1751,6 +1765,7 @@
         else MHX_MAKE(false, false, false);
       }
     });
+    if (zeroed) MHX_HIP(hipStreamWaitEvent(st, zeroed, 0));
     MHX_HIP(hipMemcpyAsync(h, cursor, 32, hipMemcpyDeviceToHost, st));
     MHX_HIP(hipMemcpyAsync(h_dh.data(), pre_hist, h_dh.size() * 8, hipMemcpyDeviceToHost, st));
     if (split_now) MHX_HIP(hipMemcpyAsync(h_fill.data(), split_cur, 256 * 8, hipMemcpyDeviceToHost, st));
@@ -1773,6 +1788,7 @@
   f->giants = nullptr;
   f->n_giant_items = f->giant_limit = f->giant_bins = f->giant_largest = 0;
   f->why = nullptr;
+  f->zeroed_bits = zero_map ? s.n_bases : 0;
   if ((uint32_t)h[1] != 0 || h[0] > cap) return false;
   const uint64_t n = h[0];
   const bool giant = !bins_whole && !c->global_bases && c->n_parts <= 1 && c->opt<Opt::s1_skm_giant>() != 0;
@@ -1819,10 +1835,15 @@
     prep.split_range_cap = range_cap;
     prep.hist_first = 1;
   }
+  const bool tags = (s.n_bases >> 32) != 0 || c->opt<Opt::s1_skm_tags>() != 0;
+  const bool narrow = !for_count && !tags && !c->global_bases && c->n_parts <= 1 && passes.size() >= 2 && n > 0 && c->opt<Opt::s1_skm_narrow>() != 0 &&
+                      sort_takes_narrow_last_pass(c, sort_passes, 1);
+  if (narrow) prep.last_words = 3;
   uint32_t *sorted = radix_sort(c, reinterpret_cast<uint32_t *>(buf_a), reinterpret_cast<uint32_t *>(buf_b), n, 4, 1, sort_passes, &prep);
   uint64_t *bounds = c->ws("s1_bucket_bounds", ((size_t)n_bins + 1) * 8 + 64).as<uint64_t>();
   MHX_LAUNCH(c, "s1_skm_bounds", (double)n_bins * 8 * 30,
-             hipLaunchKernelGGL(k_skm_bounds, dim3((n_bins + 1 + 255) / 256), dim3(256), 0, st, reinterpret_cast<const uint4 *>(sorted), n, n_bins, bounds, max_bin));
+             hipLaunchKernelGGL(k_skm_bounds, dim3((n_bins + 1 + 255) / 256), dim3(256), 0, st, sorted, narrow ? 3 : 4, n, n_bins, bounds, max_bin, (int)k,
+                                32u - (unsigned)bin_bits));
   const uint64_t limit = std::max<uint64_t>((uint64_t)c->opt<Opt::s1_skm_max_bin>(), 16 * (n / (bin_hi - bin_lo) + 1));
   constexpr uint32_t kListCap = (uint32_t)kSkmGiantMaxBins + 1;
   uint2 *giant_list = nullptr;
@@ -1837,6 +1858,7 @@
   MHX_HIP(hipStreamSynchronize(st));
   f->n_src = 1;
   f->src[0] = reinterpret_cast<const uint4 *>(sorted);
+  f->rec_words = narrow ? 3 : 4;
   f->src_bounds[0] = bounds;
   f->spare = sorted == reinterpret_cast<uint32_t *>(buf_a) ? reinterpret_cast<uint32_t *>(buf_b) : reinterpret_cast<uint32_t *>(buf_a);
   f->spare_bytes = cap_alloc * 16;
@@ -1899,7 +1921,9 @@
   }
   const uint64_t n_bits = c->global_bases ? c->global_bases : c->seqs.n_bases;
   const bool tags = (n_bits >> 32) != 0 || c->opt<Opt::s1_skm_tags>() != 0;
-  const long long deal = std::min<long long>(std::max<long long>(c->opt<Opt::s1_skm_deal>(), 0), 2);
+  srcs.narrow = f.rec_words == 3 ? 1 : 0;
+  if (srcs.narrow && (tags || f.n_src != 1)) throw Error("s1_skm_groups: 12-byte records carry no position tag and come from one source");
+  const long long deal =std::min<long long>(std::max<long long>(c->opt<Opt::s1_skm_deal>(), 0), 2);
 #define MHX_SKM_G(AGGV, TAGV, GV)                                                                                                \
   do {                                                                                                                           \
     if (deal == 2) hipLaunchKernelGGL((k_s1_skm<AGGV, TAGV, 2, GV>), dim3(grid), dim3(kSkmThreads), 0, st, srcs, a, ticket);      \
@@ -1914,7 +1938,7 @@
   const bool look = m >= 3;
   if (look && (marks_raw || giant)) throw Error("s1_skm_groups: min count 3 and 4 are served on one GPU, bins whole");
 #define MHX_SKM_LOOK(AGGV, TAGV) hipLaunchKernelGGL((k_s1_skm<AGGV, TAGV, 2, false, true>), dim3(grid), dim3(kSkmThreads), 0, st, srcs, a, ticket)
-  MHX_LAUNCH(c, "s1_skm_groups", (double)f.n_records * 16, {
+  MHX_LAUNCH(c, "s1_skm_groups", (double)f.n_records * (srcs.narrow ? 12 : 16), {
     if (look && agg && tags) MHX_SKM_LOOK(true, true);
     else if (look && agg) MHX_SKM_LOOK(true, false);
     else if (look && tags) MHX_SKM_LOOK(false, true);
@@ -2147,7 +2171,8 @@
 
 void s1_skm_bounds_of(mhx_ctx *c, const uint4 *recs, uint64_t n, uint32_t n_bins, uint64_t *bounds) {
   uint32_t *scratch = c->ws("skm_cursor", 64).as<uint32_t>() + 8;
-  hipLaunchKernelGGL(k_skm_bounds, dim3((n_bins + 1 + 255) / 256), dim3(256), 0, c->stream, recs, n, n_bins, bounds, scratch);
-}
-
-}
+  hipLaunchKernelGGL(k_skm_bounds, dim3((n_bins + 1 + 255) / 256), dim3(256), 0, c->stream, reinterpret_cast<const uint32_t *>(recs), 4, n, n_bins, bounds, scratch,
+                     0, 0u);
+}
+
+}
diff --git a/megahit_amd/csrc/skm_bins.h b/megahit_amd/csrc/skm_bins.h
--- /dev/null
+++ b/megahit_amd/csrc/skm_bins.h
@@ -0,0 +1,61 @@
+#pragma once
+#include <cstdint>
+
+#include "skm_deal.h"
+
+#if defined(__HIPCC__) || defined(__CUDACC__)
+#define MHX_SKM_UNROLL _Pragma("unroll")
+#else
+#define MHX_SKM_UNROLL
+#endif
+
+namespace mhx {
+
+constexpr int kSkmC = 8;
+constexpr int kSkmW = 10;
+constexpr int kSkmNM = kSkmC + kSkmW - 1;
+
+MHX_SKM_HD uint32_t skm_mix(uint32_t c) {
+  uint32_t h = c * 0x9E3779B1u;
+  return h ^ (h >> 15);
+}
+MHX_SKM_HD uint32_t skm_bin_of(uint32_t minh) {
+  return (minh ^ (minh >> 16)) * 0x7FEB352Du;
+}
+MHX_SKM_HD uint32_t skm_mmer_hash(uint64_t W, uint64_t R, int i, int M, uint32_t mmask) {
+  const uint32_t f = (uint32_t)(W >> (64 - 2 * (i + M))) & mmask;
+  const uint32_t rv = (uint32_t)(R >> (2 * i)) & mmask;
+  return skm_mix(f < rv ? f : rv);
+}
+MHX_SKM_HD void skm_block_bins(uint64_t W, uint64_t R, int k, unsigned bin_sh, uint32_t (&bins)[kSkmC]) {
+  const int M = k + 1 - (kSkmW - 1);
+  const uint32_t mmask = (1u << (2 * M)) - 1u;
+  uint32_t h[kSkmNM];
+  MHX_SKM_UNROLL
+  for (int i = 0; i < kSkmNM; ++i) h[i] = skm_mmer_hash(W, R, i, M, mmask);
+  uint32_t sfx[kSkmW];
+  sfx[kSkmW - 1] = h[kSkmW - 1];
+  MHX_SKM_UNROLL
+  for (int i = kSkmW - 2; i >= 0; --i) sfx[i] = h[i] < sfx[i + 1] ? h[i] : sfx[i + 1];
+  uint32_t pfx = 0xFFFFFFFFu;
+  bins[0] = skm_bin_of(sfx[0]) >> bin_sh;
+  MHX_SKM_UNROLL
+  for (int w = 1; w < kSkmC; ++w) {
+    pfx = pfx < h[kSkmW - 1 + w] ? pfx : h[kSkmW - 1 + w];
+    bins[w] = skm_bin_of(sfx[w] < pfx ? sfx[w] : pfx) >> bin_sh;
+  }
+}
+MHX_SKM_HD uint32_t skm_first_bin(uint64_t bases, int k, unsigned bin_sh) {
+  const int M = k + 1 - (kSkmW - 1);
+  const uint32_t mmask = (1u << (2 * M)) - 1u;
+  const uint64_t R = skm_rc32(bases);
+  uint32_t mn = 0xFFFFFFFFu;
+  MHX_SKM_UNROLL
+  for (int i = 0; i < kSkmW; ++i) {
+    const uint32_t h = skm_mmer_hash(bases, R, i, M, mmask);
+    mn = h < mn ? h : mn;
+  }
+  return skm_bin_of(mn) >> bin_sh;
+}
+
+}
diff --git a/megahit_amd/csrc/sort.hip b/megahit_amd/csrc/sort.hip
--- a/megahit_amd/csrc/sort.hip
+++ b/megahit_amd/csrc/sort.hip
@@ -303,9 +303,16 @@
   constexpr bool kHasUnitRuns = (S <= 3 && NI == 8 && (UT == 3 || UT == 2)) || (S == 4 && NI == 8 && UT == 2) || (S > 4 && NI == 4 && UT == 2);
   const bool unit_runs = kHasUnitRuns && c->opt<Opt::sort_unit_runs>() != 0;
   const bool rank_uniform = unit_runs && c->opt<Opt::sort_rank_uniform>() != 0;
+  constexpr bool kCanNarrow = S == 4 && NI == 8 && UT == 2;
+  const bool narrow_last = prep.last_words == 3;
+  if (prep.last_words != 0 && !(narrow_last && kCanNarrow && prep_fits && unit_runs && P > 0 &&
+                                digit_word_of(all[P - 1], passes[P - 1].bits + passes[P - 1].bits2, 1) == 0))
+    throw Error("radix sort: this call cannot leave the first word out of its last pass (sort_takes_narrow_last_pass)");
   for (int p = 0; p < P; ++p) {
     const int nb = passes[p].bits + passes[p].bits2;
     const int wi = digit_word_of(all[p], nb, 1);
+    const bool narrow = narrow_last && p == P - 1;
+    (void)narrow;
     if (p == 0 && gen) {
       static const std::string nm_gen = nm_scat + "_gen";
       MHX_LAUNCH(c, nm_gen.c_str(), bytes,
@@ -313,14 +320,16 @@
                                     tickets + kErrSlot, (unsigned long long)(p + 1), xcd_units, unit_runs ? 1 : 0, wi}));
     } else if (p == 0 && split) {
       if constexpr (kCanSplit) {
-#define MHX_US(RANKV, WIV)                                                                                                                        \
-  hipLaunchKernelGGL((k_radix_onesweep_u<S, NI, UT, SrcSplit<S>, RANKV, WIV>), dim3((unsigned)n_units_gen), dim3(kSortThreads), 0, st,            \
+#define MHX_US(RANKV, WIV, SOV)                                                                                                                   \
+  hipLaunchKernelGGL((k_radix_onesweep_u<S, NI, UT, SrcSplit<S>, RANKV, WIV, SOV>), dim3((unsigned)n_units_gen), dim3(kSortThreads), 0, st,       \
                      SrcSplit<S>{a, prep.split_fill, prep.split_ubase, prep.split_range_cap}, b, gen_slots, all[p], nb, starts + p * 256, status, tickets + p * 8, \
                      tickets + kErrSlot, (unsigned long long)(p + 1), xcd_units)
-        MHX_LAUNCH(c, nm_scat.c_str(), 2 * bytes, {
-          if (wi == 0 && rank_uniform && all[p].prev_mask) MHX_US(2, 0);
-          else if (wi == 0) MHX_US(0, 0);
-          else MHX_US(0, -1);
+        MHX_LAUNCH(c, nm_scat.c_str(), narrow ? bytes * 7 / 4 : 2 * bytes, {
+          if (narrow && rank_uniform && all[p].prev_mask) MHX_US(2, 0, 3);
+          else if (narrow) MHX_US(0, 0, 3);
+          else if (wi == 0 && rank_uniform && all[p].prev_mask) MHX_US(2, 0, S);
+          else if (wi == 0) MHX_US(0, 0, S);
+          else MHX_US(0, -1, S);
         });
 #undef MHX_US
       }
@@ -343,6 +352,20 @@
           }
         }
 #undef MHX_U2
+        if constexpr (kCanNarrow) {
+          if (narrow) {
+            MHX_LAUNCH(c, nm_scat.c_str(), bytes * 7 / 4, {
+              if (rank_uniform && all[p].prev_mask)
+                hipLaunchKernelGGL((k_radix_onesweep_u<S, NI, UT, SrcArray<S>, 2, 0, 3>), dim3((unsigned)n_units), dim3(kSortThreads), 0, st, SrcArray<S>{a}, b, n, all[p],
+                                   nb, starts + p * 256, status, tickets + p * 8, tickets + kErrSlot, (unsigned long long)(p + 1), xcd_units);
+              else
+                hipLaunchKernelGGL((k_radix_onesweep_u<S, NI, UT, SrcArray<S>, 0, 0, 3>), dim3((unsigned)n_units), dim3(kSortThreads), 0, st, SrcArray<S>{a}, b, n, all[p],
+                                   nb, starts + p * 256, status, tickets + p * 8, tickets + kErrSlot, (unsigned long long)(p + 1), xcd_units);
+            });
+            std::swap(a, b);
+            continue;
+          }
+        }
         MHX_LAUNCH(c, nm_scat.c_str(), 2 * bytes, {
           if (wi == 0 && rank_uniform && all[p].prev_mask) MHX_U(2, 0);
           else if (wi == 0) MHX_U(0, 0);
@@ -388,6 +411,7 @@
     }
   }
   refuse_unconsumed_generator(prep, "radix sort (classic passes)");
+  if (prep.last_words) throw Error("radix sort (classic passes): the caller takes narrower records from the last pass, which this sort path cannot write");
   const uint64_t n_chunks = div_ceil(n, SortCfg<S, NI>::kChunk);
   uint32_t *hist = c->ws("sort_hist", n_chunks * 256 * 4).as<uint32_t>();
   uint64_t *offs = c->ws("sort_offs", n_chunks * 256 * 8).as<uint64_t>();
@@ -626,6 +650,12 @@
   return !passes.empty() && passes.size() <= (size_t)kMaxChainedPasses && passes.size() <= (size_t)kMaxFusedPasses;
 }
 
+bool sort_takes_narrow_last_pass(const mhx_ctx *c, const std::vector<SortPass> &passes, int key_words) {
+  if (!sort_takes_split_first_pass(c, passes)) return false;
+  const SortPass &last = passes.back();
+  return digit_word_of(spec_of_pass(last, key_words), last.bits + last.bits2, 1) == 0;
+}
+
 uint32_t *radix_sort(mhx_ctx *c, uint32_t *a, uint32_t *b, uint64_t n, int stride, int key_words,
                      const std::vector<SortPass> &passes, SortPrep *prep_io) {
   SortPrep prep;
diff --git a/megahit_amd/csrc/sort_kernels.h b/megahit_amd/csrc/sort_kernels.h
--- a/megahit_amd/csrc/sort_kernels.h
+++ b/megahit_amd/csrc/sort_kernels.h
@@ -305,7 +305,7 @@
   return (ds.mask2 == 0 && ds.wi1 >= 0 && ds.wi1 <= max_word && (int)ds.bit1 + nbits <= 32) ? ds.wi1 : -1;
 }
 
-template <int S, int NI, int UT, class Src, int RANK, int WI>
+template <int S, int NI, int UT, class Src, int RANK, int WI, int SO = S>
 __global__ __launch_bounds__(kSortThreads) void k_radix_onesweep_u(Src src, uint32_t *__restrict__ out, uint64_t n, DigitSpec ds, int nbits,
                                                                    const unsigned long long *__restrict__ bin_start,
                                                                    unsigned long long *__restrict__ status, uint32_t *__restrict__ ticket,
@@ -458,7 +458,15 @@
         Rec<S> rr;
         load_rec<S>(stage + (size_t)li * S, rr);
         const unsigned d = rec_digit_w<S, WI>(rr, ds);
-        store_rec<S>(out + (uint64_t)(g_off[d] + (long long)(lo + li)) * S, rr);
+        if constexpr (SO == S) {
+          store_rec<S>(out + (uint64_t)(g_off[d] + (long long)(lo + li)) * S, rr);
+        } else {
+          static_assert(SO > 0 && SO < S, "the words a pass writes are the last SO of its records");
+          Rec<SO> ro;
+#pragma unroll
+          for (int i = 0; i < SO; ++i) ro.w[i] = rr.w[S - SO + i];
+          store_rec<SO>(out + (uint64_t)(g_off[d] + (long long)(lo + li)) * SO, ro);
+        }
       }
     }
     __syncthreads();
```

After: 57910 M edges/s (median of 6 runs). No clear change (+1.0%).
